# kelaendi/mused

Hardware: AMD Instinct MI355X
Metric: stream rows/sec, d=1024 l=128 window=10k synthetic (SWFD + kNN similarity + eigenstep + labels) (higher is better)
Workload: dtype f64; 1 GPU; synthetic d=1024 l=128 window=10000 k=50 (BASELINE config 2); stream=blob, W=10000, d=1024, l=128, k=50, modalities=1, swfd_levels=14, rccl_ranks=1, lanes_per_gpu=20, padded_window_slots=2

## Files before the change

mused_amd/csrc/eig.hip:

```cpp
#include <stdlib.h>

#include <vector>

#include "internal.h"
#include "wave_ops.h"

namespace mused {

std::recursive_mutex& capture_mutex() {
  static std::recursive_mutex m;
  return m;
}

struct OsjqCtl {
  unsigned head, tail;
  int finished, nmat;
  int all_done, error;
  int dirty;
  int pad;
};

enum class EigDirect {
  None,
  Trd,
  Trdx,
};
enum class EigJacobi {
  Queue,
  WaveGraph,
  RowGraph,
};
struct EigChoice {
  EigDirect direct;
  EigJacobi jacobi;
  int ldn;
  int rps;
  int need;
  bool cert_all;
  bool sort;
  bool adaptive;
};
struct EigEnv {
  bool trd;
  int queue;
  bool graph;
  unsigned long long queue_timeout;
};

struct EigPlan {
  int n = 0, batch = 0, sweeps = 0;
  EigChoice c{};
  double* G = nullptr;
  double* Gc = nullptr;
  double* lam = nullptr;
  const int* rep = nullptr;
  const int* jrep = nullptr;
  int* err_out = nullptr;
  double* trace = nullptr;
  unsigned long long* work = nullptr;
  int* notconv = nullptr;
  unsigned* q = nullptr;
  unsigned qcap = 0;
  OsjqCtl* qctl = nullptr;
  int* qdone = nullptr;
  int* qclean = nullptr;
  unsigned long long q_timeout = 0;
  double* trd_ws = nullptr;
  int* trd_done = nullptr;
  int *trdx_act = nullptr, *trdx_jrep = nullptr;
  int* trdx_nrej = nullptr;
  int* trdx_nrej_host = nullptr;
  hipEvent_t trdx_ev = nullptr;
  bool prof = false;
  int prof_n = 0;
  std::vector<hipEvent_t> ev0, ev1;
  std::vector<hipEvent_t> evm;
  hipGraph_t graph = nullptr;
  hipGraphExec_t exec = nullptr;
  hipStream_t cap_stream = nullptr;
  bool capturing = false;
};

constexpr int OSJ_CB = 32;
constexpr double OSJ_CONV_COS2_WAVE = 1e-10, OSJ_CONV_COS2_ROW = 1e-14;
__device__ __forceinline__ bool osj_pair_active(double pq2, double pp, double qq, double floor2, double cos2) {
  return (pq2 > cos2 * (pp * qq)) & (pp > floor2) & (qq > floor2);
}

__device__ __forceinline__ bool osj_finished(const int* __restrict__ notconv, int fr, int rps, int batch, int m) {
  if (!notconv || fr < rps) return false;
  int any = 0;
  for (int i = 1; i <= rps; ++i) any |= notconv[(long)(fr - i) * batch + m];
  return any == 0;
}

__host__ __device__ constexpr int osj_pair_p(int m2, int step, int k) {
  const int m = m2 - 1;
  const int a = (k == 0) ? m : (step + k) % m;
  const int b = (k == 0) ? (step % m) : ((step - k + m) % m);
  return a < b ? a : b;
}
__host__ __device__ constexpr int osj_pair_q(int m2, int step, int k) {
  const int m = m2 - 1;
  const int a = (k == 0) ? m : (step + k) % m;
  const int b = (k == 0) ? (step % m) : ((step - k + m) % m);
  return a < b ? b : a;
}

template <int N>
__device__ __forceinline__ double wave_treduce(double (&v)[N], int lane, int& idx) {
  static_assert(N == 4 || N == 8 || N == 16 || N == 32 || N == 64, "wave_treduce: N must be 4, 8, 16, 32 or 64");
  if constexpr (N == 4) {
    v[0] = swap32_add(v[0], v[2]);
    v[1] = swap32_add(v[1], v[3]);
    double t4 = swap16_add(v[0], v[1]);
    t4 = t4 + dpp_mov_f64<DPP_ROW_MIRROR>(t4);
    t4 = t4 + dpp_mov_f64<DPP_ROW_HALF_MIRROR>(t4);
    t4 = t4 + dpp_mov_f64<DPP_QUAD_XOR2>(t4);
    t4 = t4 + dpp_mov_f64<DPP_QUAD_XOR1>(t4);
    idx = ((lane >> 5) & 1) * 2 + ((lane >> 4) & 1);
    return t4;
  } else {
#pragma unroll
  for (int i = 0; i < N / 2; ++i) v[i] = swap32_add(v[i], v[i + N / 2]);
#pragma unroll
  for (int i = 0; i < N / 4; ++i) v[i] = swap16_add(v[i], v[i + N / 4]);
  {
    const bool hi = (lane & 8) != 0;
#pragma unroll
    for (int i = 0; i < N / 8; ++i) {
      const double keep = hi ? v[i + N / 8] : v[i];
      const double send = hi ? v[i] : v[i + N / 8];
      v[i] = keep + dpp_mov_f64<DPP_ROW_MIRROR>(send);
    }
  }
  int id = ((lane >> 5) & 1) * 4 + ((lane >> 4) & 1) * 2 + ((lane >> 3) & 1);
  double t;
  if constexpr (N == 8) {
    t = v[0] + dpp_mov_f64<DPP_ROW_HALF_MIRROR>(v[0]);
    t = t + dpp_mov_f64<DPP_QUAD_XOR2>(t);
    t = t + dpp_mov_f64<DPP_QUAD_XOR1>(t);
  } else {
    {
      const bool hi = (lane & 4) != 0;
#pragma unroll
      for (int i = 0; i < N / 16; ++i) {
        const double keep = hi ? v[i + N / 16] : v[i];
        const double send = hi ? v[i] : v[i + N / 16];
        v[i] = keep + dpp_mov_f64<DPP_ROW_HALF_MIRROR>(send);
      }
      id = id * 2 + ((lane >> 2) & 1);
    }
    if constexpr (N == 16) {
      t = v[0] + dpp_mov_f64<DPP_QUAD_XOR2>(v[0]);
      t = t + dpp_mov_f64<DPP_QUAD_XOR1>(t);
    } else {
      {
        const bool hi = (lane & 2) != 0;
#pragma unroll
        for (int i = 0; i < N / 32; ++i) {
          const double keep = hi ? v[i + N / 32] : v[i];
          const double send = hi ? v[i] : v[i + N / 32];
          v[i] = keep + dpp_mov_f64<DPP_QUAD_XOR2>(send);
        }
        id = id * 2 + ((lane >> 1) & 1);
      }
      if constexpr (N == 32) {
        t = v[0] + dpp_mov_f64<DPP_QUAD_XOR1>(v[0]);
      } else {
        const bool hi = (lane & 1) != 0;
        const double keep = hi ? v[1] : v[0];
        const double send = hi ? v[0] : v[1];
        t = keep + dpp_mov_f64<DPP_QUAD_XOR1>(send);
        id = id * 2 + (lane & 1);
      }
    }
  }
  idx = id;
  return t;
  }
}

__device__ __forceinline__ double osj_readlane(double v, int l) {
  const unsigned long long u = (unsigned long long)__double_as_longlong(v);
  const unsigned lo = __builtin_amdgcn_readlane((int)(unsigned)(u & 0xffffffffull), l);
  const unsigned hi = __builtin_amdgcn_readlane((int)(unsigned)(u >> 32), l);
  return __longlong_as_double((long long)(((unsigned long long)hi << 32) | lo));
}

__device__ __forceinline__ double osj_rcp(double y) {
  double r = __builtin_amdgcn_rcp(y);
  r = fma(r, fma(-y, r, 1.0), r);
  r = fma(r, fma(-y, r, 1.0), r);
  return r;
}
__device__ __forceinline__ double osj_rsqrt(double h) {
  double r = __builtin_amdgcn_rsq(h);
  r = r * fma(-0.5 * h, r * r, 1.5);
  r = r * fma(-0.5 * h, r * r, 1.5);
  return r;
}
__device__ __forceinline__ void osj_rotation(double pp, double qq, double pq, double& c, double& s, double& npp,
                                             double& nqq) {
  c = 1.0; s = 0.0; npp = pp; nqq = qq;
  if (pq * pq > 1e-30 * (pp * qq) && pq != 0.0) {
    const double zeta = (qq - pp) * osj_rcp(2.0 * pq);
    const double az = fabs(zeta);
    double t;
// ... 410 lines not shown
      for (int i = 0; i < RP; ++i) osj_st<ST_WT>(&M[(long)colg * ldn + lane + 64 * i], x[c * RP + i] * dd);
    }
  } else {
    const int ca = set_col(ida), cb = set_col(idb);
#pragma unroll
    for (int j = 0; j < SC; ++j) {
      const double da = sh.dsc[wave][j], db = sh.dsc[wave][SC + j];
#pragma unroll
      for (int i = 0; i < RP; ++i) {
        osj_st<ST_WT>(&M[(long)(ca + j) * ldn + lane + 64 * i], x[j * RP + i] * da);
        osj_st<ST_WT>(&M[(long)(cb + j) * ldn + lane + 64 * i], x[(SC + j) * RP + i] * db);
      }
    }
  }
  return active;
}

template <int RP, int SC, bool PREFIX>
__global__ __launch_bounds__(64 * (OSJ_CB / SC), SC == 8 ? 2 : 1) void osjw_kernel(double* __restrict__ Gc, int ldn, int nb,
                                                                                  int round,
                                                                                  int* __restrict__ notconv, int fr, int rps,
                                                                                  const double* __restrict__ trace,
                                                                                  int sortcols,
                                                                                  const int* __restrict__ rep) {
  if (rep && rep[blockIdx.y] != (int)blockIdx.y) return;
  if (osj_finished(notconv, fr, rps, gridDim.y, blockIdx.y)) return;
  double small2 = notconv ? 0.0 : -1.0;
  if (trace) {
    const double tr = trace[blockIdx.y];
    small2 = 1e-24 * tr * tr;
  }
  __shared__ OsjwShared<RP, SC> sh;
  double* M = Gc + (long)blockIdx.y * ldn * ldn;
#ifdef MUSED_OSJ_WT_STORES
  const int active = osjw_unit<RP, SC, PREFIX, false, true>(M, ldn, nb, round, blockIdx.x, small2, sortcols, sh, threadIdx.x);
#else
  const int active = osjw_unit<RP, SC, PREFIX, false>(M, ldn, nb, round, blockIdx.x, small2, sortcols, sh, threadIdx.x);
#endif
  if (notconv && __any(active) && (threadIdx.x & 63) == 0) atomicOr(&notconv[(long)fr * gridDim.y + blockIdx.y], 1);
}

constexpr unsigned OSJQ_EXIT = 0xffffffffu;

__global__ void osjq_init_kernel(OsjqCtl* __restrict__ ctl, unsigned* __restrict__ q, int* __restrict__ qdone,
                                 int* __restrict__ qclean, int batch, int upr, const int* __restrict__ rep,
                                 const int* __restrict__ skip) {
  const int m = blockIdx.x * blockDim.x + threadIdx.x;
  if (m == 0) {
    ctl->head = 0; ctl->finished = 0; ctl->all_done = 0; ctl->error = 0;
  }
  if (m >= batch) return;
  qdone[m] = 0;
  qclean[m] = 0;
  if (rep && rep[m] != m) return;
  if (skip && skip[m]) return;
  const unsigned pos = atomicAdd(&ctl->tail, (unsigned)upr);
  for (int i = 0; i < upr; ++i) q[pos + i] = 1u + (((unsigned)m * 256u + 0u) * 4u + (unsigned)i);
  atomicAdd(&ctl->nmat, 1);
  ctl->dirty = 1;
}

__global__ void osjq_reset_kernel(OsjqCtl* __restrict__ ctl) { ctl->tail = 0; ctl->nmat = 0; ctl->dirty = 0; }
template <int RP>
__global__ __launch_bounds__(256, 2) void osjq_kernel(double* __restrict__ Gc, int ldn, int nb, int batch, int max_sweeps,
                                                     int sort_from, int* __restrict__ notconv,
                                                     const double* __restrict__ trace, unsigned* __restrict__ q,
                                                     unsigned qcap, OsjqCtl* __restrict__ ctl, int* __restrict__ qdone,
                                                     int* __restrict__ qclean, unsigned long long timeout,
                                                     int* __restrict__ err_out) {
  __shared__ OsjwShared<RP, 8> sh;
  __shared__ unsigned s_item;
  const int rounds = nb - 1, upr = nb / 2;
  while (true) {
    if (threadIdx.x == 0) {
      unsigned item = OSJQ_EXIT;
      const bool over = __hip_atomic_load(&ctl->all_done, __ATOMIC_RELAXED, __HIP_MEMORY_SCOPE_AGENT) != 0;
      const unsigned t = over ? qcap : atomicAdd(&ctl->head, 1u);
      if (t < qcap) {
        const unsigned long long t0 = __builtin_amdgcn_s_memrealtime();
        while ((item = __hip_atomic_load(&q[t], __ATOMIC_RELAXED, __HIP_MEMORY_SCOPE_AGENT)) == 0u) {
          if (__hip_atomic_load(&ctl->all_done, __ATOMIC_RELAXED, __HIP_MEMORY_SCOPE_AGENT)) {
            item = OSJQ_EXIT;
            break;
          }
          __builtin_amdgcn_s_sleep(4);
          if (__builtin_amdgcn_s_memrealtime() - t0 > timeout) {
            __hip_atomic_store(&ctl->error, 1, __ATOMIC_RELAXED, __HIP_MEMORY_SCOPE_AGENT);
            __hip_atomic_store(&ctl->all_done, 1, __ATOMIC_RELAXED, __HIP_MEMORY_SCOPE_AGENT);
            if (err_out) atomicOr(err_out, 1);
            item = OSJQ_EXIT;
            break;
          }
        }
      }
      s_item = item;
    }
    __syncthreads();
    const unsigned item = (unsigned)__builtin_amdgcn_readfirstlane((int)s_item);
    __syncthreads();
    if (item == OSJQ_EXIT) return;
    const unsigned v = item - 1u;
    const int k = (int)(v & 3u), R = (int)((v >> 2) & 255u), m = (int)(v >> 10);
    const int sweep = R / rounds, r = R - sweep * rounds;
    double small2 = notconv ? 0.0 : -1.0;
    if (trace) {
      const double tr = trace[m];
      small2 = 1e-24 * tr * tr;
    }
    double* M = Gc + (long)m * ldn * ldn;
    const int so = sweep >= sort_from ? 1 : 0;
    int active;
    int tid = threadIdx.x;
    asm volatile("" : "+v"(tid));
    if (r == 0) active = osjw_unit<RP, 8, true, true>(M, ldn, nb, 0, k, small2, so, sh, tid);
    else active = osjw_unit<RP, 8, false, true>(M, ldn, nb, r, k, small2, so, sh, tid);
    if (notconv && __any(active) && (threadIdx.x & 63) == 0) atomicOr(&notconv[(long)R * batch + m], 1);
    asm volatile("s_waitcnt vmcnt(0)" ::: "memory");
    __syncthreads();
    if (threadIdx.x == 0) {
      const int old = atomicAdd(&qdone[m], 1);
      if (old == upr - 1) {
        __hip_atomic_store(&qdone[m], 0, __ATOMIC_RELAXED, __HIP_MEMORY_SCOPE_AGENT);
        bool fin = (r == rounds - 1) && (sweep + 1 >= max_sweeps);
        if (notconv && !fin) {
          const int flag = __hip_atomic_load(&notconv[(long)R * batch + m], __ATOMIC_RELAXED, __HIP_MEMORY_SCOPE_AGENT);
          const int clean = flag ? 0 : __hip_atomic_load(&qclean[m], __ATOMIC_RELAXED, __HIP_MEMORY_SCOPE_AGENT) + 1;
          __hip_atomic_store(&qclean[m], clean, __ATOMIC_RELAXED, __HIP_MEMORY_SCOPE_AGENT);
          fin = clean >= rounds;
        }
        if (fin) {
          const int f = atomicAdd(&ctl->finished, 1);
          if (f + 1 == ctl->nmat) __hip_atomic_store(&ctl->all_done, 1, __ATOMIC_RELAXED, __HIP_MEMORY_SCOPE_AGENT);
        } else {
          asm volatile("s_waitcnt vmcnt(0)" ::: "memory");
          const unsigned tt = atomicAdd(&ctl->tail, (unsigned)upr);
          for (int i = 0; i < upr; ++i)
            if (tt + i < qcap)
              __hip_atomic_store(&q[tt + i], 1u + (((unsigned)m * 256u + (unsigned)(R + 1)) * 4u + (unsigned)i),
                                 __ATOMIC_RELAXED, __HIP_MEMORY_SCOPE_AGENT);
        }
      }
    }
  }
}

__global__ void osjq_zero_kernel(unsigned* __restrict__ q, unsigned n, const OsjqCtl* __restrict__ ctl) {
  if (!ctl->dirty) return;
  const unsigned i = blockIdx.x * blockDim.x + threadIdx.x;
  if (i < n) q[i] = 0u;
}

__global__ __launch_bounds__(1024) void osjq_prep_direct_kernel(OsjqCtl* __restrict__ ctl, unsigned* __restrict__ q, unsigned qcap,
                                                               int* __restrict__ qdone, int* __restrict__ qclean, int batch,
                                                               int upr, const int* __restrict__ rep, const int* __restrict__ skip,
                                                               const double* __restrict__ Gc, int ldn, int nflag,
                                                               double* __restrict__ trace, int* __restrict__ notconv) {
  __shared__ int s_dirty;
  const int t = threadIdx.x;
  if (t == 0) s_dirty = ctl->dirty;
  __syncthreads();
  if (s_dirty)
    for (unsigned i = t; i < qcap; i += 1024) q[i] = 0u;
  __syncthreads();
  if (t == 0) {
    ctl->head = 0; ctl->tail = 0; ctl->finished = 0; ctl->nmat = 0; ctl->all_done = 0; ctl->error = 0; ctl->dirty = 0;
  }
  __syncthreads();
  for (int m = t; m < batch; m += 1024) {
    qdone[m] = 0;
    qclean[m] = 0;
    if (rep && rep[m] != m) continue;
    if (skip && skip[m]) continue;
    if (trace) {
      const double* M = Gc + (long)m * ldn * ldn;
      double sacc = 0.0;
      for (int i = 0; i < ldn; ++i) sacc += fabs(M[(long)i * ldn + i]);
      trace[m] = sacc;
      for (int f = 0; f < nflag; ++f) notconv[(long)f * batch + m] = 0;
    }
    const unsigned pos = atomicAdd(&ctl->tail, (unsigned)upr);
    for (int i = 0; i < upr; ++i) q[pos + i] = 1u + (((unsigned)m * 256u + 0u) * 4u + (unsigned)i);
    atomicAdd(&ctl->nmat, 1);
    ctl->dirty = 1;
  }
  __syncthreads();
  if (t == 0 && ctl->nmat == 0) ctl->all_done = 1;
}

template <int RP>
static void osjq_launch(EigPlan* p, hipStream_t st) {
  const int ldn = p->c.ldn, nb = ldn / OSJ_CB, upr = nb / 2;
  const bool behind_direct = p->c.direct == EigDirect::Trd;
  if (behind_direct) {
    hipLaunchKernelGGL(osjq_prep_direct_kernel, dim3(1), dim3(1024), 0, st, p->qctl, p->q, p->qcap, p->qdone, p->qclean, p->batch,
                       upr, p->rep, p->trd_done, p->Gc, ldn, p->notconv ? p->sweeps * p->c.rps : 0, p->notconv ? p->trace : nullptr,
                       p->notconv);
  } else {
    hipLaunchKernelGGL(osjq_zero_kernel, dim3(cdiv(p->qcap, 1024)), dim3(1024), 0, st, p->q, p->qcap, p->qctl);
    hipLaunchKernelGGL(osjq_reset_kernel, dim3(1), dim3(1), 0, st, p->qctl);
    hipLaunchKernelGGL(osjq_init_kernel, dim3(cdiv(p->batch, 256)), dim3(256), 0, st, p->qctl, p->q, p->qdone, p->qclean,
                       p->batch, upr, p->rep, (const int*)nullptr);
  }
  long units = (long)p->batch * upr;
  const long cap = behind_direct ? 64 : 512;
  const int grid = (int)(units < cap ? units : cap);
  hipLaunchKernelGGL((osjq_kernel<RP>), dim3(grid), dim3(256), 0, st, p->Gc, ldn, nb, p->batch, p->sweeps,
                     p->c.sort ? 0 : 1 << 30 , p->notconv, p->trace, p->q, p->qcap, p->qctl, p->qdone, p->qclean, p->q_timeout, p->err_out);
}

template <int RP>
static void osjw_launch_sweep(EigPlan* p, int sweep, hipStream_t st) {
  const int ldn = p->c.ldn, nb = ldn / OSJ_CB;
  const int so = p->c.sort ? 1 : 0;
  const int rps = p->c.rps;
  hipLaunchKernelGGL((osjw_kernel<RP, 8, true>), dim3(nb / 2, p->batch), dim3(256), 0, st, p->Gc, ldn, nb, 0,
                     p->notconv, sweep * rps, rps, p->trace, so, p->jrep);
  for (int round = 1; round < nb - 1; ++round)
    hipLaunchKernelGGL((osjw_kernel<RP, 8, false>), dim3(nb / 2, p->batch), dim3(256), 0, st, p->Gc, ldn, nb,
                       round, p->notconv, sweep * rps + round, rps, p->trace, so, p->jrep);
}

__global__ void osj_pack_kernel(const double* __restrict__ G, int n, int ldn, double* __restrict__ Gc) {
  const long gid = (long)blockIdx.x * blockDim.x + threadIdx.x;
  const long per = (long)ldn * ldn;
  if (gid >= per * gridDim.y) return;
  const int b = blockIdx.y;
  const long e = gid;
  if (e >= per) return;
  const int c = (int)(e / ldn), r = (int)(e - (long)c * ldn);
  Gc[b * per + e] = (c < n && r < n) ? G[(long)b * n * n + (long)c * n + r] : 0.0;
}

__global__ void osj_begin_kernel(const double* __restrict__ Gc, int ldn, int nflag, double* __restrict__ trace,
                                 int* __restrict__ notconv) {
  const int b = blockIdx.x, lane = threadIdx.x;
  const double* M = Gc + (long)b * ldn * ldn;
  double s = 0.0;
  for (int i = lane; i < ldn; i += 64) s += fabs(M[(long)i * ldn + i]);
  s = wave_sum(s);
  if (lane == 0) trace[b] = s;
  for (int f = lane; f < nflag; f += 64) notconv[(long)f * gridDim.x + b] = 0;
}

__global__ void osj_count_kernel(const int* __restrict__ notconv, int batch, int nround, int rps,
                                 unsigned long long* __restrict__ acc, const int* __restrict__ rep) {
  int c = 0;
  for (int b = threadIdx.x; b < batch; b += blockDim.x) {
    if (rep && rep[b] != b) continue;
    int clean = 0;
    for (int r = 0; r < nround; ++r) {
      if (r >= rps && clean >= rps) break;
      ++c;
      clean = notconv[(long)r * batch + b] ? 0 : clean + 1;
    }
  }
  c = (int)wave_sum((double)c);
  if ((threadIdx.x & 63) == 0) atomicAdd(acc, (unsigned long long)c);
}

__global__ void osj_norms_kernel(const double* __restrict__ Gc, int ldn, double* __restrict__ lam, const int* __restrict__ skip) {
  const int col = blockIdx.x * (blockDim.x >> 6) + (threadIdx.x >> 6);
  if (col >= ldn) return;
  const int b = blockIdx.y, lane = threadIdx.x & 63;
  if (skip && skip[b]) return;
  const double* c = Gc + ((long)b * ldn + col) * ldn;
  double s = 0.0;
  for (int r = lane; r < ldn; r += 64) s += c[r] * c[r];
  s = wave_sum(s);
  if (lane == 0) lam[(long)b * ldn + col] = sqrt(s);
}

__global__ void osj_extract_kernel(const double* __restrict__ Gc, const double* __restrict__ lam, int n, int ldn,
                                   double* __restrict__ evals, double* __restrict__ V) {
  const int b = blockIdx.y;
  const long gid = (long)blockIdx.x * blockDim.x + threadIdx.x;
  if (gid >= (long)n * n) return;
  const int j = (int)(gid / n), a = (int)(gid - (long)j * n);
  const double l = lam[(long)b * ldn + j];
  if (a == 0) evals[(long)b * n + j] = l;
  if (V) V[(long)b * n * n + (long)a * n + j] = (l > 0.0) ? Gc[((long)b * ldn + j) * ldn + a] / l : 0.0;
}

template <int NT>
static void osjw4_launch_sweep(EigPlan* p, int sweep, hipStream_t st) {
  constexpr int RP = NT / 64;
  const int ldn = p->c.ldn, nb = ldn / OSJ_CB;
  const int rps = p->c.rps;
  const int so = p->c.sort ? 1 : 0;
  hipLaunchKernelGGL((osj_round_kernel<OSJ_CB / 2, NT, 2>), dim3(nb, p->batch), dim3(NT), 0, st, p->Gc, p->n, ldn,
                     2 * nb, 0, p->notconv, sweep * rps, rps, p->trace, so, p->jrep);
  for (int round = 0; round < nb - 1; ++round)
    hipLaunchKernelGGL((osjw_kernel<RP, 4, false>), dim3(nb / 2, p->batch), dim3(512), 0, st, p->Gc, ldn, nb, round,
                       p->notconv, sweep * rps + 1 + round, rps, p->trace, so, p->jrep);
}

template <int NT>
static void osj_launch_sweep(EigPlan* p, int sweep, hipStream_t st) {
  const int ldn = p->c.ldn, nb = ldn / OSJ_CB;
  const int rps = p->c.rps;
  const int so = p->c.sort ? 1 : 0;
  hipLaunchKernelGGL((osj_round_kernel<OSJ_CB / 2, NT, 2>), dim3(nb, p->batch), dim3(NT), 0, st, p->Gc, p->n, ldn,
                     2 * nb, 0, p->notconv, sweep * rps, rps, p->trace, so, p->jrep);
  for (int round = 0; round < nb - 1; ++round)
    hipLaunchKernelGGL((osj_round_kernel<OSJ_CB, NT, 1>), dim3(nb / 2, p->batch), dim3(NT), 0, st, p->Gc, p->n, ldn,
                       nb, round, p->notconv, sweep * rps + 1 + round, rps, p->trace, so, p->jrep);
}

static int osj_enqueue_sweeps(EigPlan* p, hipStream_t st) {
  const int ldn = p->c.ldn;
  switch (p->c.jacobi) {
    case EigJacobi::Queue:
      switch (ldn) {
        case 64: osjq_launch<1>(p, st); break;
        case 128: osjq_launch<2>(p, st); break;
        case 192: osjq_launch<3>(p, st); break;
        default: osjq_launch<4>(p, st); break;
      }
      break;
    case EigJacobi::WaveGraph:
      for (int sw = 0; sw < p->sweeps; ++sw) {
        switch (ldn) {
          case 64: osjw_launch_sweep<1>(p, sw, st); break;
          case 128: osjw_launch_sweep<2>(p, sw, st); break;
          case 192: osjw_launch_sweep<3>(p, sw, st); break;
          case 256: osjw_launch_sweep<4>(p, sw, st); break;
          case 320: osjw4_launch_sweep<320>(p, sw, st); break;
          case 384: osjw4_launch_sweep<384>(p, sw, st); break;
          case 448: osjw4_launch_sweep<448>(p, sw, st); break;
          default: osjw4_launch_sweep<512>(p, sw, st); break;
        }
      }
      break;
    case EigJacobi::RowGraph:
      for (int sw = 0; sw < p->sweeps; ++sw) {
        switch (ldn) {
          case 640: osj_launch_sweep<640>(p, sw, st); break;
          case 768: osj_launch_sweep<768>(p, sw, st); break;
          case 896: osj_launch_sweep<896>(p, sw, st); break;
          default: osj_launch_sweep<1024>(p, sw, st); break;
        }
      }
      break;
  }
  MUSED_LAUNCH_CHECK();
  return MUSED_OK;
}

static int osj_padded_order(int n) {
  if (n <= 512) return ((n + 63) / 64) * 64;
  return ((n + 127) / 128) * 128;
}

static EigEnv eig_read_env() {
  EigEnv e;
  const char* te = getenv("MUSED_EIG_TRD");
  e.trd = !(te && te[0] == '0');
  const char* qe = getenv("MUSED_EIG_QUEUE");
  e.queue = qe ? (qe[0] == '1' ? 1 : 0) : -1;
  const char* ng = getenv("MUSED_NO_GRAPH");
  e.graph = !(ng && ng[0] == '1');
  const char* tq = getenv("MUSED_EIG_QUEUE_TIMEOUT_TICKS");
  e.queue_timeout = tq ? strtoull(tq, nullptr, 10) : 300000000ull;
  return e;
}

static EigChoice eig_choose(int n, int batch, int sweeps, int flags, int need, const EigEnv& env) {
  EigChoice c;
  c.ldn = osj_padded_order(n);
  const int nb = c.ldn / OSJ_CB;
  c.sort = !(flags & EIG_PLAN_NO_SORT);
  c.adaptive = !(flags & EIG_PLAN_FIXED_SWEEPS);
  c.need = (flags & (EIG_PLAN_TOP_NEED | EIG_PLAN_TOP_FD)) ? need : ((flags & EIG_PLAN_TOP_HALF) ? n / 2 : 0);
  c.cert_all = (flags & EIG_PLAN_TOP_NEED) != 0;
  const bool queue_fits = c.ldn <= 256 && sweeps * (nb - 1) <= 255 && batch <= (1 << 21);
  c.direct = EigDirect::None;
  if (env.trd && c.need > 0) {
    if (queue_fits && trd_supports(n, c.ldn, c.need))
      c.direct = EigDirect::Trd;
    else if (trdx_supports(c.ldn, c.need))
      c.direct = EigDirect::Trdx;
  }
  const bool want_queue =
      c.direct == EigDirect::Trd || (env.queue >= 0 ? env.queue == 1 : (long)batch * (nb / 2) <= 224);
  c.jacobi = (queue_fits && want_queue) ? EigJacobi::Queue : (c.ldn <= 512 ? EigJacobi::WaveGraph : EigJacobi::RowGraph);
  c.rps = c.ldn <= 256 ? nb - 1 : nb;
  return c;
}

static int eig_plan_create_impl(EigPlan* p, const EigEnv& env, bool own_graph) {
  const EigChoice& c = p->c;
  const size_t batch = (size_t)p->batch, ldn = (size_t)c.ldn;
  if (p->n != c.ldn) MUSED_CHECK_HIP(hipMalloc(&p->G, sizeof(double) * batch * p->n * p->n));
  MUSED_CHECK_HIP(hipMalloc(&p->Gc, sizeof(double) * batch * ldn * ldn));
  MUSED_CHECK_HIP(hipMalloc(&p->lam, sizeof(double) * batch * ldn));
  if (c.jacobi == EigJacobi::Queue) {
    const int nb = c.ldn / OSJ_CB;
    p->qcap = (unsigned)((long)p->batch * (nb / 2) * (nb - 1) * p->sweeps);
    p->q_timeout = env.queue_timeout;
    MUSED_CHECK_HIP(hipMalloc(&p->q, sizeof(unsigned) * (size_t)p->qcap));
    MUSED_CHECK_HIP(hipMalloc(&p->qctl, sizeof(OsjqCtl)));
    MUSED_CHECK_HIP(hipMalloc(&p->qdone, sizeof(int) * batch));
    MUSED_CHECK_HIP(hipMalloc(&p->qclean, sizeof(int) * batch));
    MUSED_CHECK_HIP(hipMemset(p->qctl, 0, sizeof(OsjqCtl)));
    MUSED_CHECK_HIP(hipMemset(p->q, 0, sizeof(unsigned) * (size_t)p->qcap));
  }
  int rc;
  switch (c.direct) {
    case EigDirect::None: break;
    case EigDirect::Trd:
      if ((rc = trd_prepare())) return rc;
      MUSED_CHECK_HIP(hipMalloc(&p->trd_ws, sizeof(double) * trd_workspace_doubles(p->batch)));
      MUSED_CHECK_HIP(hipMalloc(&p->trd_done, sizeof(int) * batch));
      break;
    case EigDirect::Trdx:
      if ((rc = trdx_prepare(c.ldn))) return rc;
      MUSED_CHECK_HIP(hipMalloc(&p->trd_ws, sizeof(double) * trdx_workspace_doubles(c.ldn, p->batch)));
      MUSED_CHECK_HIP(hipMalloc(&p->trd_done, sizeof(int) * batch));
      MUSED_CHECK_HIP(hipMalloc(&p->trdx_act, sizeof(int) * batch));
      MUSED_CHECK_HIP(hipMalloc(&p->trdx_jrep, sizeof(int) * batch));
      MUSED_CHECK_HIP(hipMalloc(&p->trdx_nrej, sizeof(int)));
      MUSED_CHECK_HIP(hipHostMalloc((void**)&p->trdx_nrej_host, sizeof(int), hipHostMallocDefault));
      MUSED_CHECK_HIP(hipEventCreateWithFlags(&p->trdx_ev, hipEventDisableTiming));
      p->jrep = p->trdx_jrep;
      break;
  }
  if (c.adaptive) {
    MUSED_CHECK_HIP(hipMalloc(&p->trace, sizeof(double) * (batch + 1) + sizeof(int) * batch * p->sweeps * c.rps));
    p->work = (unsigned long long*)(p->trace + batch);
    p->notconv = (int*)(p->trace + batch + 1);
    MUSED_CHECK_HIP(hipMemset(p->work, 0, 8));
  }
  if (own_graph && env.graph) {
    MUSED_CHECK_HIP(hipStreamCreateWithFlags(&p->cap_stream, hipStreamNonBlocking));
    MUSED_CHECK_HIP(hipStreamBeginCapture(p->cap_stream, hipStreamCaptureModeThreadLocal));
    p->capturing = true;
    if ((rc = osj_enqueue_sweeps(p, p->cap_stream))) return rc;
    p->capturing = false;
    MUSED_CHECK_HIP(hipStreamEndCapture(p->cap_stream, &p->graph));
    MUSED_CHECK_HIP(hipGraphInstantiate(&p->exec, p->graph, nullptr, nullptr, 0));
    (void)hipStreamDestroy(p->cap_stream);
    p->cap_stream = nullptr;
  }
  return MUSED_OK;
}

int eig_plan_create(int n, int batch, int sweeps, bool own_graph, EigPlan** out, const int* rep, int flags, int* err_out,
                    int need) {
  MUSED_REQUIRE(n >= 2 && n % 2 == 0 && n <= 1024 && batch >= 1 && sweeps >= 1,
                "eig_plan_create: the order must be even and <= 1024 (n=%d)", n);
  CaptureLock resource_guard(capture_mutex());
  const EigEnv env = eig_read_env();
  EigPlan* p = new EigPlan();
  p->n = n; p->batch = batch; p->sweeps = sweeps;
  p->rep = p->jrep = rep;
  p->err_out = err_out;
  p->c = eig_choose(n, batch, sweeps, flags, need, env);
  const int rc = eig_plan_create_impl(p, env, own_graph);
  if (rc) {
    eig_plan_destroy(p);
    return rc;
  }
  *out = p;
  return MUSED_OK;
}

void eig_plan_destroy(EigPlan* p) {
  if (!p) return;
  CaptureLock resource_guard(capture_mutex());
  if (p->capturing) {
    hipGraph_t g = nullptr;
    (void)hipStreamEndCapture(p->cap_stream, &g);
    if (g) (void)hipGraphDestroy(g);
  }
  if (p->exec) (void)hipGraphExecDestroy(p->exec);
  if (p->graph) (void)hipGraphDestroy(p->graph);
  if (p->cap_stream) (void)hipStreamDestroy(p->cap_stream);
  void* bufs[] = {p->G,      p->Gc,       p->lam,      p->trace,     p->q,        p->qctl, p->qdone,
                  p->qclean, p->trd_ws,   p->trd_done, p->trdx_act,  p->trdx_jrep, p->trdx_nrej};
  for (void* b : bufs)
    if (b) (void)hipFree(b);
  if (p->trdx_nrej_host) (void)hipHostFree(p->trdx_nrej_host);
  if (p->trdx_ev) (void)hipEventDestroy(p->trdx_ev);
  for (auto* v : {&p->ev0, &p->ev1, &p->evm})
    for (hipEvent_t e : *v) (void)hipEventDestroy(e);
  delete p;
}

int eig_plan_profile(EigPlan* p, bool on) {
  if (!p) return MUSED_OK;
  if (on && p->ev0.empty()) {
    for (auto* v : {&p->ev1, &p->evm, &p->ev0}) {
      if (v == &p->evm && p->c.direct == EigDirect::None) continue;
      while (v->size() < 2048) {
        hipEvent_t e;
        MUSED_CHECK_HIP(hipEventCreate(&e));
        v->push_back(e);
      }
    }
  }
  p->prof = on;
  if (on) {
    p->prof_n = 0;
    if (p->work) MUSED_CHECK_HIP(hipMemset(p->work, 0, 8));
  }
  return MUSED_OK;
}

int eig_plan_profile_read(EigPlan* p, double* total_ms, long* launches, double* bytes_per_launch) {
  *total_ms = 0.0; *launches = 0; *bytes_per_launch = 0.0;
  if (!p || p->ev0.empty()) return MUSED_OK;
  for (int i = 0; i < p->prof_n; ++i) {
    MUSED_CHECK_HIP(hipEventSynchronize(p->ev1[i]));
    float ms = 0.f;
    MUSED_CHECK_HIP(hipEventElapsedTime(&ms, p->ev0[i], p->ev1[i]));
    *total_ms += ms;
  }
  *launches = (long)p->prof_n * p->sweeps * p->c.rps;
  double frac = 1.0;
  if (p->work && p->prof_n > 0) {
    unsigned long long w = 0;
    CaptureLock guard(capture_mutex());
    MUSED_CHECK_HIP(hipMemcpy(&w, p->work, 8, hipMemcpyDeviceToHost));
    frac = (double)w / ((double)p->prof_n * p->sweeps * p->c.rps * p->batch);
  }
  *bytes_per_launch = 16.0 * (double)p->batch * p->c.ldn * p->c.ldn * frac;
  return MUSED_OK;
}

int eig_plan_profile_read_direct(EigPlan* p, double* total_ms, long* launches, double* matrices_solved, double* tridiag_ms) {
  *total_ms = 0.0; *launches = 0; *matrices_solved = 0.0;
  if (tridiag_ms) *tridiag_ms = 0.0;
  if (!p || p->c.direct == EigDirect::None || p->ev0.empty()) return MUSED_OK;
  for (int i = 0; i < p->prof_n; ++i) {
    MUSED_CHECK_HIP(hipEventSynchronize(p->ev1[i]));
    float ms = 0.f;
    MUSED_CHECK_HIP(hipEventElapsedTime(&ms, p->ev0[i], p->ev1[i]));
    *total_ms += ms;
    if (tridiag_ms) {
      MUSED_CHECK_HIP(hipEventElapsedTime(&ms, p->ev0[i], p->evm[i]));
      *tridiag_ms += ms;
    }
  }
  *launches = p->prof_n;
  if (p->work) {
    unsigned long long w = 0;
    CaptureLock guard(capture_mutex());
    MUSED_CHECK_HIP(hipMemcpy(&w, p->work, 8, hipMemcpyDeviceToHost));
    *matrices_solved = (double)w;
  }
  return MUSED_OK;
}

EigColumns eig_plan_columns(EigPlan* p) { return {p->Gc, p->lam, p->c.ldn}; }

bool eig_plan_direct_solver(EigPlan* p) { return p && p->c.direct != EigDirect::None; }

double* eig_plan_input(EigPlan* p) { return p->G ? p->G : p->Gc; }

static int eig_run_direct(EigPlan* p, hipStream_t st, bool rec) {
  unsigned long long* work = rec ? p->work : nullptr;
  hipEvent_t after_a = rec ? p->evm[p->prof_n] : nullptr;
  int rc;
  if (p->c.direct == EigDirect::Trd) {
    rc = trd_solve(p->Gc, p->n, p->c.ldn, p->c.need, p->c.cert_all, p->batch, p->rep, p->trd_done, p->trd_ws, st, nullptr, work,
                   after_a, p->lam);
  } else {
    MUSED_CHECK_HIP(hipMemsetAsync(p->trdx_nrej, 0, sizeof(int), st));
    rc = trdx_solve(p->Gc, p->c.ldn, p->c.need, p->c.cert_all, p->batch, p->rep, p->trd_done, p->trdx_act, p->trdx_jrep,
                    p->trdx_nrej, p->trd_ws, st, work, after_a, nullptr, p->lam);
  }
  if (rc) return rc;
  if (rec) {
    MUSED_CHECK_HIP(hipEventRecord(p->ev1[p->prof_n], st));
    ++p->prof_n;
  }
  return MUSED_OK;
}

static int eig_jacobi_needed(EigPlan* p, hipStream_t st, bool* needed) {
  *needed = true;
  if (p->c.direct != EigDirect::Trdx) return MUSED_OK;
  hipStreamCaptureStatus cs = hipStreamCaptureStatusNone;
  (void)hipStreamIsCapturing(st, &cs);
  if (cs != hipStreamCaptureStatusNone) return MUSED_OK;
  MUSED_CHECK_HIP(hipMemcpyAsync(p->trdx_nrej_host, p->trdx_nrej, sizeof(int), hipMemcpyDeviceToHost, st));
  MUSED_CHECK_HIP(hipEventRecord(p->trdx_ev, st));
  MUSED_CHECK_HIP(hipEventSynchronize(p->trdx_ev));
  *needed = *p->trdx_nrej_host != 0;
  return MUSED_OK;
}

int eig_plan_run_inplace(EigPlan* p, double* evals, double* V, hipStream_t st, bool allow_graph) {
  const EigChoice& c = p->c;
  const bool direct = c.direct != EigDirect::None;
  int rc;
  if (p->G) {
    const long per = (long)c.ldn * c.ldn;
    hipLaunchKernelGGL(osj_pack_kernel, dim3(cdiv(per, 256), p->batch), dim3(256), 0, st, p->G, p->n, c.ldn, p->Gc);
  }
  if (p->notconv && c.direct != EigDirect::Trd)
    hipLaunchKernelGGL(osj_begin_kernel, dim3(p->batch), dim3(64), 0, st, p->Gc, c.ldn, p->sweeps * c.rps, p->trace, p->notconv);
  const bool rec = p->prof && p->prof_n < (int)p->ev0.size();
  if (rec) MUSED_CHECK_HIP(hipEventRecord(p->ev0[p->prof_n], st));
  if (direct && (rc = eig_run_direct(p, st, rec))) return rc;
  bool jacobi = true;
  if ((rc = eig_jacobi_needed(p, st, &jacobi))) return rc;
  if (jacobi) {
    if (p->exec && allow_graph)
      MUSED_CHECK_HIP(hipGraphLaunch(p->exec, st));
    else if ((rc = osj_enqueue_sweeps(p, st)))
      return rc;
  }
  if (rec && !direct) {
    MUSED_CHECK_HIP(hipEventRecord(p->ev1[p->prof_n], st));
    ++p->prof_n;
    if (p->notconv)
      hipLaunchKernelGGL(osj_count_kernel, dim3(1), dim3(256), 0, st, p->notconv, p->batch, p->sweeps * c.rps, c.rps, p->work,
                         p->rep);
  }
  hipLaunchKernelGGL(osj_norms_kernel, dim3(cdiv(c.ldn, 4), p->batch), dim3(256), 0, st, p->Gc, c.ldn, p->lam,
                     (const int*)p->trd_done);
  if (evals)
    hipLaunchKernelGGL(osj_extract_kernel, dim3(cdiv((long)p->n * p->n, 256), p->batch), dim3(256), 0, st, p->Gc, p->lam, p->n,
                       c.ldn, evals, V);
  MUSED_LAUNCH_CHECK();
  return MUSED_OK;
}

int eig_plan_run(EigPlan* p, const double* G, double* evals, double* V, hipStream_t st) {
  const size_t bytes = sizeof(double) * (size_t)p->batch * p->n * p->n;
  MUSED_CHECK_HIP(hipMemcpyAsync(eig_plan_input(p), G, bytes, hipMemcpyDeviceToDevice, st));
  return eig_plan_run_inplace(p, evals, V, st, true);
}

static int eig_time(EigPlan* p, hipEvent_t& e0, hipEvent_t& e1, const double* G, int reps, double* evals, double* V,
                    double* out_ms, int* out_err, hipStream_t st) {
  MUSED_CHECK_HIP(hipEventCreate(&e0));
  MUSED_CHECK_HIP(hipEventCreate(&e1));
  int rc = eig_plan_run(p, G, evals, V, st);
  MUSED_CHECK_HIP(hipStreamSynchronize(st));
  MUSED_CHECK_HIP(hipEventRecord(e0, st));
  for (int i = 0; i < reps && !rc; ++i) rc = eig_plan_run(p, G, evals, V, st);
  MUSED_CHECK_HIP(hipEventRecord(e1, st));
  MUSED_CHECK_HIP(hipEventSynchronize(e1));
  float ms = 0.f;
  MUSED_CHECK_HIP(hipEventElapsedTime(&ms, e0, e1));
  *out_ms = ms / (reps > 0 ? reps : 1);
  if (out_err) {
    *out_err = 0;
    if (p->c.jacobi == EigJacobi::Queue) {
      OsjqCtl c;
      MUSED_CHECK_HIP(hipMemcpy(&c, p->qctl, sizeof(c), hipMemcpyDeviceToHost));
      *out_err = c.error ? -1 : (int)c.tail;
    }
  }
  return rc;
}

}

using namespace mused;

extern "C" {

int mused_debug_eig_choice(int n, int batch, int sweeps, int flags, int need, int* out) {
  MUSED_REQUIRE(out && n >= 2 && n % 2 == 0 && n <= 1024 && batch >= 1 && sweeps >= 1,
                "mused_debug_eig_choice: the order must be even and <= 1024 (n=%d)", n);
  const EigChoice c = eig_choose(n, batch, sweeps, flags, need, eig_read_env());
  const int v[8] = {(int)c.direct, (int)c.jacobi, c.ldn, c.rps, c.need, c.cert_all, c.sort, c.adaptive};
  memcpy(out, v, sizeof(v));
  return MUSED_OK;
}

int mused_debug_eig_time(const double* G, int n, int batch, int sweeps, int reps, double* evals, double* V, double* out_ms,
                         int* out_err, void* stream) {
  EigPlan* p = nullptr;
  int rc = eig_plan_create(n, batch, sweeps, true, &p);
  if (rc) return rc;
  hipEvent_t e0 = nullptr, e1 = nullptr;
  rc = eig_time(p, e0, e1, G, reps, evals, V, out_ms, out_err, (hipStream_t)stream);
  if (e0) (void)hipEventDestroy(e0);
  if (e1) (void)hipEventDestroy(e1);
  eig_plan_destroy(p);
  return rc;
}

int mused_syevj_batched(const double* G, int n, int batch, int sweeps, double* evals, double* V, void* stream) {
  MUSED_REQUIRE(G && evals && V, "mused_syevj_batched: null pointer");
  EigPlan* p = nullptr;
  int rc = eig_plan_create(n, batch, sweeps, true, &p);
  if (rc) return rc;
  rc = eig_plan_run(p, G, evals, V, (hipStream_t)stream);
  hipError_t e = hipStreamSynchronize((hipStream_t)stream);
  eig_plan_destroy(p);
  if (rc) return rc;
  MUSED_CHECK_HIP(e);
  return MUSED_OK;
}

}
```

mused_amd/csrc/gemm_f64.h:

```cpp
#pragma once
#include <mutex>
#include "common.h"

namespace mused {

typedef double v4f64 __attribute__((ext_vector_type(4)));

constexpr int GEMM_BM = 128;
constexpr int GEMM_BN = 128;
constexpr int GEMM_BK = 16;
constexpr int GEMM_LD = 144;
constexpr int GEMM_THREADS = 256;
constexpr int GEMM_LDS_BYTES = 2  * 2  * GEMM_BK * GEMM_LD * 8;

struct GemmArgs {
  const void* A;
  const void* B;
  long lda, ldb;
  long strideA, strideB;
  int M, N, K;
  int kchunk;
  int splitk;
  int bsplit;
  int tiles_m, tiles_n;
  const int* rep;
  int sym;
};

template <typename TIn, bool VEC>
__device__ __forceinline__ void stage_load_kc(const TIn* __restrict__ src, long ld, int r0, int nrows, int k0,
                                              int kend, TIn (&r)[8]) {
  const int m = threadIdx.x & 127;
  const int kh = threadIdx.x >> 7;
  const int row = r0 + m;
  const int k = k0 + kh * 8;
  if (row < nrows) {
    const TIn* p = src + (long)row * ld + k;
    if (VEC && k + 8 <= kend) {
      if (sizeof(TIn) == 4) {
        const float4 a = *reinterpret_cast<const float4*>(p);
        const float4 b = *reinterpret_cast<const float4*>(p + 4);
        r[0] = a.x; r[1] = a.y; r[2] = a.z; r[3] = a.w;
        r[4] = b.x; r[5] = b.y; r[6] = b.z; r[7] = b.w;
      } else {
        const double2* q = reinterpret_cast<const double2*>(p);
#pragma unroll
        for (int j = 0; j < 4; ++j) {
          const double2 v = q[j];
          r[2 * j] = v.x;
          r[2 * j + 1] = v.y;
        }
      }
    } else {
#pragma unroll
      for (int j = 0; j < 8; ++j) r[j] = (k + j < kend) ? p[j] : (TIn)0;
    }
  } else {
#pragma unroll
    for (int j = 0; j < 8; ++j) r[j] = (TIn)0;
  }
}

template <typename TIn>
__device__ __forceinline__ void stage_store_kc(double* __restrict__ lds, const TIn (&r)[8]) {
  const int m = threadIdx.x & 127;
  const int kh = threadIdx.x >> 7;
#pragma unroll
  for (int j = 0; j < 8; ++j) lds[(kh * 8 + j) * GEMM_LD + m] = (double)r[j];
}

template <typename TIn, bool VEC>
__device__ __forceinline__ void stage_load_mc(const TIn* __restrict__ src, long ld, int c0, int ncols, int k0,
                                              int kend, TIn (&r)[8]) {
  const int kk = threadIdx.x >> 4;
  const int c = c0 + (threadIdx.x & 15) * 8;
  const int k = k0 + kk;
  if (k < kend) {
    const TIn* p = src + (long)k * ld + c;
    if (VEC && c + 8 <= ncols) {
      if (sizeof(TIn) == 4) {
        const float4 a = *reinterpret_cast<const float4*>(p);
        const float4 b = *reinterpret_cast<const float4*>(p + 4);
        r[0] = a.x; r[1] = a.y; r[2] = a.z; r[3] = a.w;
        r[4] = b.x; r[5] = b.y; r[6] = b.z; r[7] = b.w;
      } else {
        const double2* q = reinterpret_cast<const double2*>(p);
#pragma unroll
        for (int j = 0; j < 4; ++j) {
          const double2 v = q[j];
          r[2 * j] = v.x;
          r[2 * j + 1] = v.y;
        }
      }
    } else {
#pragma unroll
      for (int j = 0; j < 8; ++j) r[j] = (c + j < ncols) ? p[j] : (TIn)0;
    }
  } else {
#pragma unroll
    for (int j = 0; j < 8; ++j) r[j] = (TIn)0;
  }
}

template <typename TIn>
__device__ __forceinline__ void stage_store_mc(double* __restrict__ lds, const TIn (&r)[8]) {
  const int kk = threadIdx.x >> 4;
  const int c = (threadIdx.x & 15) * 8;
  double* p = lds + kk * GEMM_LD + c;
#pragma unroll
  for (int j = 0; j < 8; ++j) p[j] = (double)r[j];
}

template <typename TIn>
__device__ __forceinline__ void stage_load8(const TIn* __restrict__ p, TIn (&r)[8]) {
  if (sizeof(TIn) == 4) {
    const float4 a = *reinterpret_cast<const float4*>(p);
    const float4 b = *reinterpret_cast<const float4*>(p + 4);
    r[0] = a.x; r[1] = a.y; r[2] = a.z; r[3] = a.w;
    r[4] = b.x; r[5] = b.y; r[6] = b.z; r[7] = b.w;
  } else {
    const double2* q = reinterpret_cast<const double2*>(p);
#pragma unroll
    for (int j = 0; j < 4; ++j) {
      const double2 v = q[j];
      r[2 * j] = v.x;
      r[2 * j + 1] = v.y;
    }
  }
}
template <typename TIn>
__device__ __forceinline__ void stage_load_kc_full(const TIn* __restrict__ src, long ld, int r0, int k0, TIn (&r)[8]) {
  stage_load8(src + (long)(r0 + (threadIdx.x & 127)) * ld + k0 + (threadIdx.x >> 7) * 8, r);
}
template <typename TIn>
__device__ __forceinline__ void stage_load_mc_full(const TIn* __restrict__ src, long ld, int c0, int k0, TIn (&r)[8]) {
  stage_load8(src + (long)(k0 + (threadIdx.x >> 4)) * ld + c0 + (threadIdx.x & 15) * 8, r);
}

__device__ __forceinline__ int xcd_remap(int pid, int nwg) {
  const int q = nwg >> 3, r = nwg & 7, xcd = pid & 7;
  const int base = (xcd < r) ? xcd * (q + 1) : r * (q + 1) + (xcd - r) * q;
  return base + (pid >> 3);
}

template <typename TA, typename TB, bool A_KC, bool B_KC, bool VEC>
__device__ __forceinline__ void gemm_tile_mainloop(const GemmArgs& g, const TA* __restrict__ A, const TB* __restrict__ B,
                                                   int m0, int n0, int k_lo, int k_hi, double* smem,
                                                   v4f64 (&acc)[4][4]) {
  double* As = smem;
  double* Bs = smem + 2 * GEMM_BK * GEMM_LD;
  const int lane = threadIdx.x & 63;
  const int wave = threadIdx.x >> 6;
  const int wr = wave >> 1, wc = wave & 1;
  const int kq = lane >> 4, li = lane & 15;
#pragma unroll
  for (int i = 0; i < 4; ++i)
#pragma unroll
    for (int j = 0; j < 4; ++j) acc[i][j] = (v4f64){0.0, 0.0, 0.0, 0.0};

  TA ra[8];
  TB rb[8];
  const int nkt = (k_hi - k_lo + GEMM_BK - 1) / GEMM_BK;

  const bool full_mn = VEC && m0 + GEMM_BM <= g.M && n0 + GEMM_BN <= g.N;
  auto load_tile = [&](int kt) {
    const int k0 = k_lo + kt * GEMM_BK;
    if (full_mn && k0 + GEMM_BK <= k_hi) {
      if (A_KC) stage_load_kc_full<TA>(A, g.lda, m0, k0, ra); else stage_load_mc_full<TA>(A, g.lda, m0, k0, ra);
      if (B_KC) stage_load_kc_full<TB>(B, g.ldb, n0, k0, rb); else stage_load_mc_full<TB>(B, g.ldb, n0, k0, rb);
      return;
    }
    if (A_KC) stage_load_kc<TA, VEC>(A, g.lda, m0, g.M, k0, k_hi, ra);
    else      stage_load_mc<TA, VEC>(A, g.lda, m0, g.M, k0, k_hi, ra);
    if (B_KC) stage_load_kc<TB, VEC>(B, g.ldb, n0, g.N, k0, k_hi, rb);
    else      stage_load_mc<TB, VEC>(B, g.ldb, n0, g.N, k0, k_hi, rb);
  };
  auto store_tile = [&](int buf) {
    double* a = As + buf * GEMM_BK * GEMM_LD;
    double* b = Bs + buf * GEMM_BK * GEMM_LD;
    if (A_KC) stage_store_kc(a, ra); else stage_store_mc(a, ra);
    if (B_KC) stage_store_kc(b, rb); else stage_store_mc(b, rb);
  };

  if (nkt > 0) {
    load_tile(0);
    store_tile(0);
  }
  __syncthreads();

  int cur = 0;
  for (int kt = 0; kt < nkt; ++kt) {
    const bool more = (kt + 1 < nkt);
    if (more) load_tile(kt + 1);
    const double* a = As + cur * GEMM_BK * GEMM_LD + wr * 64 + li;
    const double* b = Bs + cur * GEMM_BK * GEMM_LD + wc * 64 + li;
#pragma unroll
    for (int kk = 0; kk < GEMM_BK / 4; ++kk) {
      double fa[4], fb[4];
#pragma unroll
      for (int i = 0; i < 4; ++i) fa[i] = a[(kk * 4 + kq) * GEMM_LD + i * 16];
#pragma unroll
      for (int j = 0; j < 4; ++j) fb[j] = b[(kk * 4 + kq) * GEMM_LD + j * 16];
#pragma unroll
      for (int i = 0; i < 4; ++i)
#pragma unroll
        for (int j = 0; j < 4; ++j)
          acc[i][j] = __builtin_amdgcn_mfma_f64_16x16x4f64(fa[i], fb[j], acc[i][j], 0, 0, 0);
    }
    if (more) store_tile(cur ^ 1);
    __syncthreads();
    cur ^= 1;
  }
}

template <typename TA, typename TB, bool A_KC, bool B_KC, bool VEC, typename Epi>
__global__ __launch_bounds__(GEMM_THREADS, 2) void gemm_f64_kernel(GemmArgs g, Epi epi) {
  extern __shared__ __attribute__((aligned(16))) double smem[];

  const int z = blockIdx.z;
  const int zb = g.bsplit ? z / g.bsplit : z;
  if (g.rep && g.rep[zb] != zb) return;
  int tm, tn;
  if (g.sym) {
    const int t = g.tiles_n, nwg = t * (t + 1) / 2;
    const int e = xcd_remap(blockIdx.x, nwg);
    int r = (int)((2.0 * t + 1.0 - sqrt((2.0 * t + 1.0) * (2.0 * t + 1.0) - 8.0 * e)) * 0.5);
    r = r < 0 ? 0 : (r > t - 1 ? t - 1 : r);
    while (r > 0 && r * t - r * (r - 1) / 2 > e) --r;
    while (r + 1 < t && (r + 1) * t - (r + 1) * r / 2 <= e) ++r;
    tm = r;
    tn = r + (e - (r * t - r * (r - 1) / 2));
  } else {
    const int nwg = g.tiles_m * g.tiles_n;
    const int wg = xcd_remap(blockIdx.x, nwg);
    constexpr int GROUP_M = 8;
    const int per_group = GROUP_M * g.tiles_n;
    const int group_id = wg / per_group;
    const int first_m = group_id * GROUP_M;
    const int group_size = min(g.tiles_m - first_m, GROUP_M);
    tm = first_m + (wg % group_size);
    tn = (wg % per_group) / group_size;
  }
  const int m0 = tm * GEMM_BM, n0 = tn * GEMM_BN;
  const bool mirror = g.sym && tm != tn;

  int k_lo = 0, k_hi = g.K;
  const TA* A = reinterpret_cast<const TA*>(g.A);
  const TB* B = reinterpret_cast<const TB*>(g.B);
  if (g.splitk) {
    k_lo = z * g.kchunk;
    k_hi = min(g.K, k_lo + g.kchunk);
  } else {
    A += (long)zb * g.strideA;
    B += (long)zb * g.strideB;
    if (g.bsplit) {
      k_lo = (z - zb * g.bsplit) * g.kchunk;
      k_hi = min(g.K, k_lo + g.kchunk);
    }
  }

  const int lane = threadIdx.x & 63;
  const int wave = threadIdx.x >> 6;
  const int wr = wave >> 1, wc = wave & 1;
  const int kq = lane >> 4, li = lane & 15;

  v4f64 acc[4][4];
  gemm_tile_mainloop<TA, TB, A_KC, B_KC, VEC>(g, A, B, m0, n0, k_lo, k_hi, smem, acc);

#pragma unroll
  for (int i = 0; i < 4; ++i) {
#pragma unroll
    for (int j = 0; j < 4; ++j) {
      const int col = n0 + wc * 64 + j * 16 + li;
#pragma unroll
      for (int r = 0; r < 4; ++r) {
        const int row = m0 + wr * 64 + i * 16 + kq + 4 * r;
        if (row < g.M && col < g.N) epi(z, row, col, acc[i][j][r]);
      }
    }
  }
  if (mirror) {
    __syncthreads();
    double* patch = smem + wave * (32 * 65);
#pragma unroll
    for (int half = 0; half < 2; ++half) {
#pragma unroll
      for (int i = 0; i < 4; ++i)
#pragma unroll
        for (int jj = 0; jj < 2; ++jj) {
          const int j = half * 2 + jj;
          const int col = n0 + wc * 64 + j * 16 + li;
#pragma unroll
          for (int r = 0; r < 4; ++r) {
            const int rl = i * 16 + kq + 4 * r;
            const int rg = m0 + wr * 64 + rl;
            patch[(jj * 16 + li) * 65 + rl] = (rg < g.M && col < g.N) ? epi.value(col, rg, acc[i][j][r]) : 0.0;
          }
        }
      const int rowm = m0 + wr * 64 + lane;
#pragma unroll 8
      for (int c = 0; c < 32; ++c) {
        const int colm = n0 + wc * 64 + half * 32 + c;
        if (colm < g.N && rowm < g.M) epi.put(z, colm, rowm, patch[c * 65 + lane]);
      }
    }
  }
}

struct EpiStore {
  double* C;
  long ldc;
  long strideC;
  double alpha;
  __device__ __forceinline__ void operator()(int z, int row, int col, double v) const {
    C[(long)z * strideC + (long)row * ldc + col] = alpha * v;
  }
  __device__ __forceinline__ double value(int, int, double v) const { return alpha * v; }
  __device__ __forceinline__ void put(int z, int row, int col, double val) const {
    C[(long)z * strideC + (long)row * ldc + col] = val;
  }
};

template <typename TA, typename TB, bool A_KC, bool B_KC, bool VEC, typename Epi>
int gemm_f64_prepare_t() {
  static std::once_flag once;
  static hipError_t err = hipSuccess;
  std::call_once(once, [] {
    auto k = gemm_f64_kernel<TA, TB, A_KC, B_KC, VEC, Epi>;
    err = hipFuncSetAttribute(reinterpret_cast<const void*>(k), hipFuncAttributeMaxDynamicSharedMemorySize,
                              GEMM_LDS_BYTES);
  });
  MUSED_CHECK_HIP(err);
  return MUSED_OK;
}

template <typename TA, typename TB, bool A_KC, bool B_KC, typename Epi>
int gemm_f64_launch_t(GemmArgs g, int batch, Epi epi, bool vec, hipStream_t stream) {
  g.tiles_m = cdiv(g.M, GEMM_BM);
  g.tiles_n = cdiv(g.N, GEMM_BN);
  if (g.M <= 0 || g.N <= 0 || batch <= 0) return MUSED_OK;
  dim3 grid(g.sym ? g.tiles_n * (g.tiles_n + 1) / 2 : g.tiles_m * g.tiles_n, 1, batch);
  int rc;
  if (vec) {
    if ((rc = gemm_f64_prepare_t<TA, TB, A_KC, B_KC, true, Epi>())) return rc;
    hipLaunchKernelGGL((gemm_f64_kernel<TA, TB, A_KC, B_KC, true, Epi>), grid, dim3(GEMM_THREADS), GEMM_LDS_BYTES,
                       stream, g, epi);
  } else {
    if ((rc = gemm_f64_prepare_t<TA, TB, A_KC, B_KC, false, Epi>())) return rc;
    hipLaunchKernelGGL((gemm_f64_kernel<TA, TB, A_KC, B_KC, false, Epi>), grid, dim3(GEMM_THREADS), GEMM_LDS_BYTES,
                       stream, g, epi);
  }
  MUSED_LAUNCH_CHECK();
  return MUSED_OK;
}

template <typename T>
static inline bool vec_ok(const void* p, long ld, long stride) {
  const long e = 16 / (long)sizeof(T);
  return ((uintptr_t)p % 16 == 0) && (ld % e == 0) && (stride % e == 0);
}

}
```

mused_amd/csrc/gemm_f64.hip:

```cpp
#include <stdarg.h>

#include "gemm_f64.h"
#include "internal.h"

namespace mused {

static thread_local char g_err[512] = "";

void set_error(const char* fmt, ...) {
  va_list ap;
  va_start(ap, fmt);
  vsnprintf(g_err, sizeof(g_err), fmt, ap);
  va_end(ap);
}

const char* last_error() { return g_err; }

int gemm_f64_prepare_all() {
  int rc = 0;
#define PREP(a, b, v) rc |= gemm_f64_prepare_t<double, double, a, b, v, EpiStore>()
  PREP(true, true, true); PREP(true, true, false); PREP(true, false, true); PREP(true, false, false);
  PREP(false, true, true); PREP(false, true, false); PREP(false, false, true); PREP(false, false, false);
#undef PREP
  return rc ? MUSED_ERR_HIP : MUSED_OK;
}

int gemm_f64(bool a_kc, bool b_kc, const double* A, long lda, long strideA, const double* B, long ldb,
             long strideB, double* C, long ldc, long strideC, int M, int N, int K, int batch, double alpha,
             hipStream_t stream, const int* rep) {
  GemmArgs g;
  memset(&g, 0, sizeof(g));
  g.A = A; g.B = B; g.lda = lda; g.ldb = ldb; g.strideA = strideA; g.strideB = strideB;
  g.M = M; g.N = N; g.K = K; g.splitk = 0; g.kchunk = 0;
  g.rep = rep;
  g.sym = (A == B && a_kc == b_kc && lda == ldb && strideA == strideB && M == N) ? 1 : 0;
  EpiStore epi{C, ldc, strideC, alpha};
  const bool vec = vec_ok<double>(A, lda, strideA) && vec_ok<double>(B, ldb, strideB);
  if (a_kc && b_kc) return gemm_f64_launch_t<double, double, true, true>(g, batch, epi, vec, stream);
  if (a_kc && !b_kc) return gemm_f64_launch_t<double, double, true, false>(g, batch, epi, vec, stream);
  if (!a_kc && b_kc) return gemm_f64_launch_t<double, double, false, true>(g, batch, epi, vec, stream);
  return gemm_f64_launch_t<double, double, false, false>(g, batch, epi, vec, stream);
}

int gemm_f64_splitk(bool a_kc, bool b_kc, const double* A, long lda, const double* B, long ldb, double* partial,
                    int M, int N, int K, int kchunk, int nsplit, hipStream_t stream) {
  MUSED_REQUIRE(kchunk > 0 && kchunk % GEMM_BK == 0 && nsplit >= 1 && (long)kchunk * nsplit >= K,
                "gemm_f64_splitk: bad kchunk %d x %d for K=%d", kchunk, nsplit, K);
  GemmArgs g;
  memset(&g, 0, sizeof(g));
  g.A = A; g.B = B; g.lda = lda; g.ldb = ldb;
  g.M = M; g.N = N; g.K = K; g.splitk = 1; g.kchunk = kchunk;
  EpiStore epi{partial, (long)N, (long)M * N, 1.0};
  const bool vec = vec_ok<double>(A, lda, 0) && vec_ok<double>(B, ldb, 0);
  if (a_kc && b_kc) return gemm_f64_launch_t<double, double, true, true>(g, nsplit, epi, vec, stream);
  if (a_kc && !b_kc) return gemm_f64_launch_t<double, double, true, false>(g, nsplit, epi, vec, stream);
  if (!a_kc && b_kc) return gemm_f64_launch_t<double, double, false, true>(g, nsplit, epi, vec, stream);
  return gemm_f64_launch_t<double, double, false, false>(g, nsplit, epi, vec, stream);
}

__global__ void splitk_reduce_kernel(const double* __restrict__ partial, int nsplit, long count,
                                     double* __restrict__ out) {
  const long i = (long)blockIdx.x * blockDim.x + threadIdx.x;
  if (i >= count) return;
  double s = 0.0;
  for (int z = 0; z < nsplit; ++z) s += partial[(long)z * count + i];
  out[i] = s;
}

int gemm_f64_batched_splitk(bool a_kc, bool b_kc, const double* A, long lda, long strideA, const double* B, long ldb, long strideB,
                            double* partial, int M, int N, int K, int batch, int kchunk, int nsplit, hipStream_t stream,
                            const int* rep) {
  MUSED_REQUIRE(kchunk > 0 && kchunk % GEMM_BK == 0 && nsplit >= 1 && (long)kchunk * nsplit >= K,
                "gemm_f64_batched_splitk: bad kchunk %d x %d for K=%d", kchunk, nsplit, K);
  GemmArgs g;
  memset(&g, 0, sizeof(g));
  g.A = A; g.B = B; g.lda = lda; g.ldb = ldb; g.strideA = strideA; g.strideB = strideB;
  g.M = M; g.N = N; g.K = K; g.splitk = 0; g.kchunk = kchunk; g.bsplit = nsplit;
  g.rep = rep;
  g.sym = (A == B && a_kc == b_kc && lda == ldb && strideA == strideB && M == N) ? 1 : 0;
  EpiStore epi{partial, (long)N, (long)M * N, 1.0};
  const bool vec = vec_ok<double>(A, lda, strideA) && vec_ok<double>(B, ldb, strideB);
  if (a_kc && b_kc) return gemm_f64_launch_t<double, double, true, true>(g, batch * nsplit, epi, vec, stream);
  if (a_kc && !b_kc) return gemm_f64_launch_t<double, double, true, false>(g, batch * nsplit, epi, vec, stream);
  if (!a_kc && b_kc) return gemm_f64_launch_t<double, double, false, true>(g, batch * nsplit, epi, vec, stream);
  return gemm_f64_launch_t<double, double, false, false>(g, batch * nsplit, epi, vec, stream);
}

__global__ void batched_splitk_reduce_kernel(const double* __restrict__ partial, int nsplit, long count, double* __restrict__ out,
                                             const int* __restrict__ rep) {
  const int z = blockIdx.y;
  if (rep && rep[z] != z) return;
  const long i = (long)blockIdx.x * blockDim.x + threadIdx.x;
  if (i >= count) return;
  const double* p = partial + (long)z * nsplit * count + i;
  double s = 0.0;
  for (int sp = 0; sp < nsplit; ++sp) s += p[(long)sp * count];
  out[(long)z * count + i] = s;
}

int gemm_batched_splitk_reduce(const double* partial, int nsplit, long count, double* out, int batch, const int* rep,
                               hipStream_t stream) {
  hipLaunchKernelGGL(batched_splitk_reduce_kernel, dim3(cdiv(count, 256), batch), dim3(256), 0, stream, partial, nsplit, count, out,
                     rep);
  MUSED_LAUNCH_CHECK();
  return MUSED_OK;
}

int gemm_splitk_reduce(const double* partial, int nsplit, long count, double* out, hipStream_t stream) {
  hipLaunchKernelGGL(splitk_reduce_kernel, dim3(cdiv(count, 256)), dim3(256), 0, stream, partial, nsplit, count,
                     out);
  MUSED_LAUNCH_CHECK();
  return MUSED_OK;
}

}

extern "C" {

const char* mused_last_error(void) { return mused::last_error(); }

int mused_version(void) { return 100; }

int mused_memcpy_d2d(void* dst, const void* src, long bytes, void* stream) {
  MUSED_REQUIRE(dst && src && bytes >= 0, "mused_memcpy_d2d: bad arguments");
  MUSED_CHECK_HIP(hipMemcpyAsync(dst, src, (size_t)bytes, hipMemcpyDeviceToDevice, (hipStream_t)stream));
  return MUSED_OK;
}

int mused_gemm_f64(int a_kc, int b_kc, const double* A, long lda, const double* B, long ldb, double* C, long ldc,
                   int M, int N, int K, double alpha, void* stream) {
  return mused::gemm_f64(a_kc != 0, b_kc != 0, A, lda, 0, B, ldb, 0, C, ldc, 0, M, N, K, 1, alpha,
                         (hipStream_t)stream);
}

int mused_gemm_f64_batched(int a_kc, int b_kc, const double* A, long lda, long strideA, const double* B, long ldb,
                           long strideB, double* C, long ldc, long strideC, int M, int N, int K, int batch,
                           double alpha, void* stream) {
  return mused::gemm_f64(a_kc != 0, b_kc != 0, A, lda, strideA, B, ldb, strideB, C, ldc, strideC, M, N, K, batch,
                         alpha, (hipStream_t)stream);
}

int mused_gemm_f64_batched_rep(int a_kc, int b_kc, const double* A, long lda, long strideA, const double* B, long ldb,
                               long strideB, double* C, long ldc, long strideC, int M, int N, int K, int batch,
                               double alpha, const int* rep, void* stream) {
  return mused::gemm_f64(a_kc != 0, b_kc != 0, A, lda, strideA, B, ldb, strideB, C, ldc, strideC, M, N, K, batch,
                         alpha, (hipStream_t)stream, rep);
}

int mused_gemm_f64_splitk(int a_kc, int b_kc, const double* A, long lda, const double* B, long ldb, double* partial,
                          double* C, int M, int N, int K, int kchunk, int nsplit, void* stream) {
  MUSED_REQUIRE(A && B && partial && C && M >= 0 && N >= 0 && K >= 0, "mused_gemm_f64_splitk: bad arguments");
  int rc = mused::gemm_f64_splitk(a_kc != 0, b_kc != 0, A, lda, B, ldb, partial, M, N, K, kchunk, nsplit,
                                  (hipStream_t)stream);
  if (rc != MUSED_OK || M == 0 || N == 0) return rc;
  return mused::gemm_splitk_reduce(partial, nsplit, (long)M * N, C, (hipStream_t)stream);
}

int mused_gemm_f64_batched_splitk(int a_kc, int b_kc, const double* A, long lda, long strideA, const double* B, long ldb,
                                  long strideB, double* partial, double* C, int M, int N, int K, int batch, int kchunk,
                                  int nsplit, const int* rep, void* stream) {
  MUSED_REQUIRE(A && B && partial && C && M >= 0 && N >= 0 && K >= 0 && batch >= 1,
                "mused_gemm_f64_batched_splitk: bad arguments");
  int rc = mused::gemm_f64_batched_splitk(a_kc != 0, b_kc != 0, A, lda, strideA, B, ldb, strideB, partial, M, N, K, batch,
                                          kchunk, nsplit, (hipStream_t)stream, rep);
  if (rc != MUSED_OK || M == 0 || N == 0) return rc;
  return mused::gemm_batched_splitk_reduce(partial, nsplit, (long)M * N, C, batch, rep, (hipStream_t)stream);
}

}
```

mused_amd/csrc/internal.h:

```cpp
#pragma once
#include "common.h"

#include <mutex>

namespace mused {

int select_from_records(const double* rec, int n, int kind, int k, int* out_idx, unsigned long long* out_mask,
                        int mask_words, hipStream_t stream);
int select_from_tag_sets(const int* rowptr, const int* tags, const int* postptr, const int* postrow, int n, int k,
                         int* out_idx, unsigned long long* out_mask, int mask_words, hipStream_t stream);
int select_max_fused_rows(bool tag_sets);
int select_window_records(const double* rec, const int* vrank, int s, int e, int kind, int k, unsigned long long* out_mask,
                          int mask_words, hipStream_t stream);
int select_window_tag_sets(const int* rowptr, const int* tags, const int* postptr, const int* postrow, const int* vrank, int s,
                           int e, int k, unsigned long long* out_mask, int mask_words, hipStream_t stream);

std::recursive_mutex& capture_mutex();
using CaptureLock = std::lock_guard<std::recursive_mutex>;


int gemm_f64(bool a_kc, bool b_kc, const double* A, long lda, long strideA, const double* B, long ldb,
             long strideB, double* C, long ldc, long strideC, int M, int N, int K, int batch, double alpha,
             hipStream_t stream, const int* rep = nullptr);

int gemm_f64_batched_splitk(bool a_kc, bool b_kc, const double* A, long lda, long strideA, const double* B, long ldb, long strideB,
                            double* partial, int M, int N, int K, int batch, int kchunk, int nsplit, hipStream_t stream,
                            const int* rep = nullptr);
int gemm_batched_splitk_reduce(const double* partial, int nsplit, long count, double* out, int batch, const int* rep,
                               hipStream_t stream);
int gemm_f64_prepare_all();

int gemm_f64_splitk(bool a_kc, bool b_kc, const double* A, long lda, const double* B, long ldb, double* partial,
                    int M, int N, int K, int kchunk, int nsplit, hipStream_t stream);
int gemm_splitk_reduce(const double* partial, int nsplit, long count, double* out, hipStream_t stream);

int lu_permute_l(double* Y, int n, int r, long ld, int* pivstep, double* prow, long ws_f64_len, hipStream_t st);
int qr_economic(double* Y, int n, int r, long ldy, double* Q, long ldq, double* tau, double* wpart, hipStream_t st,
                const int* run_if = nullptr);
int spmm_binary(const int* rowptr, const int* colidx, int n, const double* Q, long ldq, int r, double* Y, long ldy,
                hipStream_t stream);

int adj_csr_from_mask(const unsigned long long* mask, int n, int words, int* deg, int* rowptr, int* colidx,
                      int* stats, long cap, int* overflow, hipStream_t st);
int zero_ints(int* p, long n, hipStream_t st);
int adj_transpose(const unsigned long long* mask, int n, int words, unsigned long long* out, hipStream_t st);

struct EigPlan;
constexpr int EIG_PLAN_FIXED_SWEEPS = 1;
constexpr int EIG_PLAN_NO_SORT = 2;
constexpr int EIG_PLAN_TOP_HALF = 4;
constexpr int EIG_PLAN_TOP_NEED = 8;
constexpr int EIG_PLAN_TOP_FD = 16;
int eig_plan_create(int n, int batch, int sweeps, bool own_graph, EigPlan** out, const int* rep = nullptr, int flags = 0,
                    int* err_out = nullptr, int need = 0);
void eig_plan_destroy(EigPlan* p);
double* eig_plan_input(EigPlan* p);
int eig_plan_run_inplace(EigPlan* p, double* evals, double* V, hipStream_t stream, bool allow_graph);
int eig_plan_run(EigPlan* p, const double* G, double* evals, double* V, hipStream_t stream);
struct EigColumns {
  const double *cols, *lam;
  int ld;
};
EigColumns eig_plan_columns(EigPlan* p);
bool eig_plan_direct_solver(EigPlan* p);
int eig_plan_profile(EigPlan* p, bool on);
int eig_plan_profile_read(EigPlan* p, double* total_ms, long* launches, double* bytes_per_launch);
int eig_plan_profile_read_direct(EigPlan* p, double* total_ms, long* launches, double* matrices_solved,
                                 double* tridiag_ms = nullptr);

size_t trd_workspace_doubles(int batch);
int trd_prepare();
bool trd_supports(int n, int ldn, int need);
long trd_tail_ws_per();
long trd_tail_off_hs();
long trd_tail_off_tg();
int trd_tail_launch(const double* G, const int* rep, double* ws, int batch, hipStream_t st);
int trd_solve(double* Gc, int n, int ldn, int need, bool cert_all, int batch, const int* rep, int* done, double* ws,
              hipStream_t st, long long* dbg_clk = nullptr, unsigned long long* work = nullptr, hipEvent_t after_a = nullptr,
              double* lam_out = nullptr);

bool trdx_supports(int ldn, int need);
size_t trdx_workspace_doubles(int ldn, int batch);
int trdx_prepare(int ldn);
int trdx_solve(double* Gc, int ldn, int need, bool cert_all, int batch, const int* rep, int* done, int* act, int* jrep,
               int* nrej, double* ws, hipStream_t st, unsigned long long* work = nullptr, hipEvent_t after_a = nullptr,
               long long* prof = nullptr,
               double* lam_out = nullptr);

}
```

mused_amd/csrc/swfd.hip:

```cpp
#include <vector>

#include "internal.h"

namespace mused {

struct Swfd {
  int N, d, ell, L, S, cap, n2, n4, n3;
  int lanes;
  double R;
  long i;
  int pend;
  long restart_mark;
  int skip_dead;
  bool twin;
  int sweeps;
  double* buf;
  double* queue;
  long long* qt;
  int* meta;
  int* rep;
  long long* dropped;
  double* theta;
  double *T, *Wc;
  int gram_split;
  double* gpart;
  int* plan;
  int* keep_src;
  long long* now_dev;
  int* status;
  int* status_host;
  EigPlan* eig;
  double *stack, *Wq, *Bout, *sig_out, *qinfo;
  int* qsel;
  EigPlan* eigq;
  EigPlan* eigq3;
  int pre_chunk;
  double *pre_in, *pre_out, *pre_gram;
  EigPlan* eigp;
};

static inline int sk_index(const Swfd* h, int lane, int level, int kind) { return lane * 2 * h->L + kind * h->L + level; }

struct BitWord { unsigned long long w; };
template <typename T>
__device__ __forceinline__ double row_elem(const T* row, int c) { return (double)row[c]; }
template <>
__device__ __forceinline__ double row_elem<BitWord>(const BitWord* row, int c) {
  return (double)((row[c >> 6].w >> (c & 63)) & 1ull);
}

template <typename T>
__global__ void swfd_append_kernel(const T* __restrict__ X, long ldx, long lane_stride, int per_lane, int m, int d,
                                   int n2, int pend, const int* __restrict__ meta, double* __restrict__ buf) {
  const int r = blockIdx.x, s = blockIdx.y;
  X += (long)(s / per_lane) * lane_stride;
  const int row = meta[s * 4 + 0] + pend + r;
  if (row >= n2) return;
  double* dst = buf + ((long)s * n2 + row) * d;
  const T* src = X + (long)r * ldx;
  for (int c = threadIdx.x; c < d; c += blockDim.x) dst[c] = row_elem<T>(src, c);
}

__global__ void swfd_restart_kernel(double* __restrict__ buf, double* __restrict__ queue, long long* __restrict__ qt,
                                    int* __restrict__ meta, long long* __restrict__ dropped, int L, long buf_elems,
                                    long queue_elems, int cap) {
  const int lane = blockIdx.y / L, j = blockIdx.y - lane * L;
  const int sm = lane * 2 * L + j, sa = sm + L;
  const long gid = (long)blockIdx.x * blockDim.x + threadIdx.x;
  if (gid < buf_elems) {
    buf[sm * buf_elems + gid] = buf[sa * buf_elems + gid];
    buf[sa * buf_elems + gid] = 0.0;
  }
  if (gid < queue_elems) queue[sm * queue_elems + gid] = queue[sa * queue_elems + gid];
  if (gid < cap) qt[sm * cap + gid] = qt[sa * cap + gid];
  if (gid == 0) {
    for (int k = 0; k < 4; ++k) {
      meta[sm * 4 + k] = meta[sa * 4 + k];
      meta[sa * 4 + k] = 0;
    }
    dropped[sm] = dropped[sa];
    dropped[sa] = 0;
  }
}

__global__ void swfd_set_now_kernel(long long* now, long long v) { *now = v; }

__global__ void swfd_rep_kernel(const int* __restrict__ meta, int L, int nchains, int* __restrict__ rep, int twin,
                                const long long* __restrict__ dropped, long long epoch_start, int skip_dead,
                                long long* __restrict__ now_dev, long long now) {
  const int c = blockIdx.x * blockDim.x + threadIdx.x;
  if (c == 0) *now_dev = now;
  if (c >= nchains) return;
  const int base = ((twin && (c & 1)) ? c - 1 : c) * L;
  if (twin && (c & 1)) {
    int r = base + L - 1;
    rep[c * L + L - 1] = r;
    for (int j = L - 2; j >= 0; --j) {
      if (meta[(base + j) * 4 + 3] != 0) r = base + j;
      rep[c * L + j] = r;
    }
    return;
  }
  int r = base + L - 1;
  rep[r] = r;
  for (int j = L - 2; j >= 0; --j) {
    if (meta[(base + j) * 4 + 3] != 0) r = base + j;
    rep[base + j] = r;
  }
  if (skip_dead && !twin && (c & 1) == 0)
    for (int j = 0; j < L - 1; ++j)
      if (dropped[base + j] > epoch_start) rep[base + j] = -1;
}

__global__ __launch_bounds__(1024) void swfd_decide_kernel(const double* __restrict__ evals,
                                                          const double* __restrict__ U, int ldu, int n2,
                                                          int ell, int cap,
                                                          int N, const long long* __restrict__ now_p,
                                                          const double* __restrict__ theta, int* __restrict__ meta,
                                                          long long* __restrict__ qt, long long* __restrict__ dropped,
                                                          int* __restrict__ plan, int* __restrict__ keep_src,
                                                          double* __restrict__ Wc, const int* __restrict__ rep) {
  __shared__ double lam[1024];
  __shared__ int order[1024];
  __shared__ double scale[512];
  const int s = blockIdx.x, t = threadIdx.x;
  const long long now = *now_p;
  const int sr = rep ? rep[s] : s;
  if (sr < 0) return;
  const double* ev = evals + (long)sr * ldu;
  const double* Us = U + (long)sr * ldu * ldu;
  if (t < n2) lam[t] = ev[t];
  __syncthreads();
  if (t < n2) {
    const double mine = lam[t];
    int rank = 0;
    for (int j = 0; j < n2; ++j) {
      const double o = lam[j];
      rank += (o > mine) || (o == mine && j < t);
    }
    order[rank] = t;
  }
  __syncthreads();
  __shared__ int s_part[16];
  __shared__ int s_wcnt[3][4];
  const int head0 = meta[s * 4 + 1], cnt0 = meta[s * 4 + 2];
  long long* q = qt + (long)s * cap;
  const int wv = t >> 6, ln = t & 63;
  int expired = 0;
  for (int k = t; k < cnt0; k += 1024) expired += (q[(head0 + k) % cap] + N <= now) ? 1 : 0;
#pragma unroll
  for (int o = 32; o > 0; o >>= 1) expired += __shfl_xor(expired, o);
  if (ln == 0) s_part[wv] = expired;
  __syncthreads();
  int nexp = 0;
#pragma unroll
  for (int ww = 0; ww < 16; ++ww) nexp += s_part[ww];
  const int head1 = (head0 + nexp) % cap, cnt1 = cnt0 - nexp;
  const double l0 = lam[order[0]];
  const double delta = lam[order[ell - 1]] > 0.0 ? lam[order[ell - 1]] : 0.0;
  const double tol = 1e-10 * (l0 > 0.0 ? l0 : 0.0);
  const double th = theta[s];
  int kind = 0, near = 0;
  double sc = 0.0;
  if (t < ell) {
    const double l = lam[order[t]];
    double s2 = l - delta;
    s2 = s2 > 0.0 ? s2 : 0.0;
    if (s2 > tol) {
      sc = sqrt(s2 / l) / l;
      kind = (s2 >= th) ? 2 : 1;
      near = (kind == 2 && s2 < 2.0 * th) ? 1 : 0;
    }
    scale[t] = sc;
  }
  const unsigned long long mk = __ballot(kind == 1), md = __ballot(kind == 2), mn = __ballot(near != 0);
  const unsigned long long below = (ln == 0) ? 0ull : (~0ull >> (64 - ln));
  if (ln == 0 && wv < 4) {
    s_wcnt[0][wv] = __popcll(mk);
    s_wcnt[1][wv] = __popcll(md);
    s_wcnt[2][wv] = __popcll(mn);
  }
  __syncthreads();
  int kpos = __popcll(mk & below), dpos = __popcll(md & below);
  int nk = 0, nd = 0, nnear = 0;
#pragma unroll
  for (int ww = 0; ww < 4; ++ww) {
    if (ww < wv) {
      kpos += s_wcnt[0][ww];
      dpos += s_wcnt[1][ww];
    }
    nk += s_wcnt[0][ww];
    nd += s_wcnt[1][ww];
    nnear += s_wcnt[2][ww];
  }
  const int nevict = (cnt1 + nd > cap) ? (cnt1 + nd - cap) : 0;
  if (t == 0) {
    long long drop = dropped[s];
    if (nevict > 0) {
      const long long ts = q[(head1 + nevict - 1) % cap];
      drop = ts > drop ? ts : drop;
    }
    dropped[s] = drop;
  }
  __syncthreads();
  if (t < ell) {
    int pos = 0;
    if (kind == 1) {
      pos = kpos;
      keep_src[s * ell + kpos] = t;
    } else if (kind == 2) {
      pos = (head1 + cnt1 + dpos) % cap;
      q[pos] = now;
    }
    plan[(s * ell + t) * 2 + 0] = kind;
    plan[(s * ell + t) * 2 + 1] = pos;
  }
  if (t == 0) {
    meta[s * 4 + 0] = nk;
    meta[s * 4 + 1] = (head1 + nevict) % cap;
    meta[s * 4 + 2] = cnt1 + nd - nevict;
    meta[s * 4 + 3] += nnear;
  }
  __syncthreads();
  if (sr != s) return;
  double* W = Wc + (long)s * ell * n2;
  for (int e = t; e < ell * n2; e += 1024) {
    const int i = e / n2, a = e - i * n2;
    const double sc = scale[i];
    W[e] = (sc != 0.0) ? sc * Us[(long)order[i] * ldu + a] : 0.0;
  }
}

__global__ void swfd_scatter_kernel(const double* __restrict__ T, const int* __restrict__ plan,
                                    const int* __restrict__ keep_src, const int* __restrict__ meta,
                                    double* __restrict__ buf, double* __restrict__ queue, int n2, int ell, int cap,
                                    int d, const int* __restrict__ rep) {
  const int rho = blockIdx.x, s = blockIdx.y;
  if (rep && rep[s] < 0) return;
  const double* Ts = T + (long)(rep ? rep[s] : s) * ell * d;
  if (rho < ell && plan[(s * ell + rho) * 2] == 2) {
    const int slot = plan[(s * ell + rho) * 2 + 1];
    double* dst = queue + ((long)s * cap + slot) * d;
    const double* src = Ts + (long)rho * d;
    for (int c = threadIdx.x; c < d; c += blockDim.x) dst[c] = src[c];
  }
  const int nk = meta[s * 4 + 0];
  double* dst = buf + ((long)s * n2 + rho) * d;
  if (rho < nk) {
    const double* src = Ts + (long)keep_src[s * ell + rho] * d;
    for (int c = threadIdx.x; c < d; c += blockDim.x) dst[c] = src[c];
  } else {
    for (int c = threadIdx.x; c < d; c += blockDim.x) dst[c] = 0.0;
  }
}

static int swfd_rotate_all(Swfd* h, hipStream_t st) {
  const int S = h->S, n2 = h->n2, d = h->d, ell = h->ell;
  int rc;
  if (h->rep)
    hipLaunchKernelGGL(swfd_rep_kernel, dim3(cdiv(2 * h->lanes, 64)), dim3(64), 0, st, h->meta, h->L, 2 * h->lanes, h->rep,
                       h->twin ? 1 : 0, h->dropped, (long long)(((h->i - 1) / h->N) * h->N), h->skip_dead, h->now_dev,
                       (long long)h->i);
  else
    hipLaunchKernelGGL(swfd_set_now_kernel, dim3(1), dim3(1), 0, st, h->now_dev, (long long)h->i);
  if (h->gram_split > 1) {
    const int kchunk = ((d + h->gram_split - 1) / h->gram_split + 15) / 16 * 16;
    if ((rc = gemm_f64_batched_splitk(true, true, h->buf, d, (long)n2 * d, h->buf, d, (long)n2 * d, h->gpart, n2, n2, d, S, kchunk,
                                      h->gram_split, st, h->rep)))
      return rc;
    if ((rc = gemm_batched_splitk_reduce(h->gpart, h->gram_split, (long)n2 * n2, eig_plan_input(h->eig), S, h->rep, st))) return rc;
  } else if ((rc = gemm_f64(true, true, h->buf, d, (long)n2 * d, h->buf, d, (long)n2 * d, eig_plan_input(h->eig), n2,
                            (long)n2 * n2, n2, n2, d, S, 1.0, st, h->rep)))
    return rc;
  if ((rc = eig_plan_run_inplace(h->eig, nullptr, nullptr, st, true))) return rc;
  const EigColumns e = eig_plan_columns(h->eig);
  hipLaunchKernelGGL(swfd_decide_kernel, dim3(S), dim3(1024), 0, st, e.lam, e.cols, e.ld, n2, ell, h->cap, h->N, h->now_dev,
                     h->theta, h->meta, h->qt, h->dropped, h->plan, h->keep_src, h->Wc, h->rep);
  if ((rc = gemm_f64(true, false, h->Wc, n2, (long)ell * n2, h->buf, d, (long)n2 * d, h->T, d, (long)ell * d, ell, d,
                     n2, S, 1.0, st, h->rep)))
    return rc;
  hipLaunchKernelGGL(swfd_scatter_kernel, dim3(n2, S), dim3(256), 0, st, h->T, h->plan, h->keep_src, h->meta, h->buf,
                     h->queue, n2, ell, h->cap, d, h->rep);
  MUSED_LAUNCH_CHECK();
  h->pend = 0;
  return MUSED_OK;
}

static int swfd_restart(Swfd* h, hipStream_t st) {
  const long be = (long)h->n2 * h->d, qe = (long)h->cap * h->d;
  const long m = be > qe ? be : qe;
  hipLaunchKernelGGL(swfd_restart_kernel, dim3(cdiv(m, 256), h->L * h->lanes), dim3(256), 0, st, h->buf, h->queue, h->qt,
                     h->meta, h->dropped, h->L, be, qe, h->cap);
  MUSED_LAUNCH_CHECK();
  return MUSED_OK;
}

constexpr int SWFD_PRE_MAX = 96;
struct PreBlocks {
  int row0[SWFD_PRE_MAX];
  int rows[SWFD_PRE_MAX];
};

template <typename T>
__global__ void swfd_pre_load_kernel(const T* __restrict__ X, long ldx, long lane_stride, int lanes, int ell, int d,
                                     PreBlocks pb, double* __restrict__ out) {
  const int row = blockIdx.x, z = blockIdx.y;
  const int blk = z / lanes, lane = z - blk * lanes;
  double* dst = out + ((long)z * ell + row) * d;
  if (row < pb.rows[blk]) {
    const T* src = X + (long)lane * lane_stride + (long)(pb.row0[blk] + row) * ldx;
    for (int c = threadIdx.x; c < d; c += blockDim.x) dst[c] = row_elem<T>(src, c);
  } else {
    for (int c = threadIdx.x; c < d; c += blockDim.x) dst[c] = 0.0;
  }
}

__global__ void swfd_pre_pack_kernel(const double* __restrict__ gram, int ell, double* __restrict__ Gc) {
  const int n2 = 2 * ell;
  const long z = blockIdx.y;
  const long e = (long)blockIdx.x * blockDim.x + threadIdx.x;
  if (e >= (long)n2 * n2) return;
  const int col = (int)(e / n2), row = (int)(e - (long)col * n2);
  double v = 0.0;
  if (col < ell) v = (row < ell) ? gram[z * ell * ell + (long)col * ell + row] : ((row - ell == col) ? 1.0 : 0.0);
  Gc[z * n2 * n2 + e] = v;
}

template <typename T>
static int swfd_prerotate(Swfd* h, const T* X, long ldx, long lane_stride, const PreBlocks& pb, int nblk, hipStream_t st) {
  const int ell = h->ell, d = h->d, B = h->lanes, n2 = h->n2;
  int rc;
  const int Z = nblk * B;
  hipLaunchKernelGGL(swfd_pre_load_kernel<T>, dim3(ell, Z), dim3(256), 0, st, X, ldx, lane_stride, B, ell, d, pb,
                     h->pre_in);
  if ((rc = gemm_f64(true, true, h->pre_in, d, (long)ell * d, h->pre_in, d, (long)ell * d, h->pre_gram, ell,
                     (long)ell * ell, ell, ell, d, Z, 1.0, st)))
    return rc;
  hipLaunchKernelGGL(swfd_pre_pack_kernel, dim3(cdiv((long)n2 * n2, 256), Z), dim3(256), 0, st, h->pre_gram, ell,
                     eig_plan_input(h->eigp));
  if ((rc = eig_plan_run_inplace(h->eigp, nullptr, nullptr, st, true))) return rc;
  const double* cols = eig_plan_columns(h->eigp).cols;
  const int ld = eig_plan_columns(h->eigp).ld;
  if ((rc = gemm_f64(true, false, cols + ell, ld, (long)ld * ld, h->pre_in, d, (long)ell * d, h->pre_out, d, (long)ell * d,
                     ell, d, ell, Z, 1.0, st)))
    return rc;
  MUSED_LAUNCH_CHECK();
  return MUSED_OK;
}

template <typename T>
static int swfd_append_t(Swfd* h, const T* X, long ldx, long lane_stride, long m, hipStream_t st) {
  long r = 0;
  int rc;
  PreBlocks pb;
  int pre_n = 0, pre_next = 0;
  while (r < m) {
    if (h->i > 0 && h->i % h->N == 0 && h->restart_mark != h->i) {
      if ((rc = swfd_restart(h, st))) return rc;
      h->restart_mark = h->i;
      h->twin = false;
    }
    const long in_epoch = h->i % h->N;
    long until = h->ell - (in_epoch % h->ell);
    if (h->N - in_epoch < until) until = h->N - in_epoch;
    const long take = (m - r) < until ? (m - r) : until;
    bool from_pre = false;
    if (h->pre_chunk > 0 && h->pend == 0 && take == until) {
      if (pre_next >= pre_n) {
        pre_n = pre_next = 0;
        long rr = r, ii = h->i;
        while (pre_n < h->pre_chunk && rr < m) {
          const long ie = ii % h->N;
          long u = h->ell - (ie % h->ell);
          if (h->N - ie < u) u = h->N - ie;
          if (m - rr < u) break;
          pb.row0[pre_n] = (int)rr;
          pb.rows[pre_n] = (int)u;
          ++pre_n;
          rr += u;
          ii += u;
        }
        if ((rc = swfd_prerotate<T>(h, X, ldx, lane_stride, pb, pre_n, st))) return rc;
      }
      from_pre = true;
    }
    if (from_pre) {
      const double* src = h->pre_out + (long)pre_next * h->lanes * h->ell * h->d;
      hipLaunchKernelGGL(swfd_append_kernel<double>, dim3((int)take, h->S), dim3(256), 0, st, src, (long)h->d,
                         (long)h->ell * h->d, 2 * h->L, (int)take, h->d, h->n2, h->pend, h->meta, h->buf);
      ++pre_next;
    } else {
      hipLaunchKernelGGL(swfd_append_kernel<T>, dim3((int)take, h->S), dim3(256), 0, st, X + r * ldx, ldx, lane_stride,
                         2 * h->L, (int)take, h->d, h->n2, h->pend, h->meta, h->buf);
    }
    MUSED_LAUNCH_CHECK();
    h->pend += (int)take;
    h->i += take;
    r += take;
    if (take == until) {
      if ((rc = swfd_rotate_all(h, st))) return rc;
    }
  }
  return MUSED_OK;
}

__global__ void swfd_select_kernel(const int* __restrict__ meta, const long long* __restrict__ qt,
                                   const long long* __restrict__ dropped, int L, int cap, int N, long long now,
                                   int* __restrict__ qsel_all) {
  if (threadIdx.x != 0) return;
  const int lane = blockIdx.x;
  const int base = lane * 2 * L;
  int* qsel = qsel_all + (long)lane * (4 + cap);
  int lvl = L - 1;
  for (int j = 0; j < L; ++j) {
    const long long dr = dropped[base + j];
    if (dr == 0 || dr + N <= now) { lvl = j; break; }
  }
  const int sk = base + lvl;
  const int head = meta[sk * 4 + 1], cnt = meta[sk * 4 + 2];
  int ns = 0;
  for (int q = 0; q < cnt; ++q) {
    const int slot = (head + q) % cap;
    if (qt[(long)sk * cap + slot] + N > now) qsel[4 + ns++] = slot;
  }
  qsel[0] = lvl;
  qsel[1] = ns;
  qsel[2] = meta[sk * 4 + 0];
  qsel[3] = sk;
}

__global__ void swfd_stack_kernel(const int* __restrict__ qsel_all, const double* __restrict__ buf,
                                  const double* __restrict__ queue, int n2, int n4, int cap, int d, int pend,
// ... 12 lines not shown
                                                                const double* __restrict__ U_all, int ldu, int n4, int ell,
                                                                int cap, const int* __restrict__ qsel_all,
                                                                double* __restrict__ Wq_all,
                                                                double* __restrict__ qinfo_all) {
  __shared__ double lam[1024];
  __shared__ int order[1024];
  __shared__ double scale[512];
  const int t = threadIdx.x, lane = blockIdx.x;
  const double* evals = evals_all + (long)lane * ldu;
  const double* U = U_all + (long)lane * ldu * ldu;
  const int* qsel = qsel_all + (long)lane * (4 + cap);
  double* Wq = Wq_all + (long)lane * ell * n4;
  double* qinfo = qinfo_all + (long)lane * 2;
  if (t < n4) lam[t] = evals[t];
  __syncthreads();
  if (t < n4) {
    const double mine = lam[t];
    int rank = 0;
    for (int j = 0; j < n4; ++j) {
      const double o = lam[j];
      rank += (o > mine) || (o == mine && j < t);
    }
    order[rank] = t;
  }
  __syncthreads();
  const double l0 = lam[order[0]];
  const double delta = lam[order[ell - 1]] > 0.0 ? lam[order[ell - 1]] : 0.0;
  const double tol = 1e-10 * (l0 > 0.0 ? l0 : 0.0);
  if (t < ell) {
    const double l = lam[order[t]];
    double s2 = l - delta;
    s2 = s2 > 0.0 ? s2 : 0.0;
    scale[t] = (s2 > tol) ? sqrt(s2 / l) / l : 0.0;
  }
  if (t == 0) {
    qinfo[0] = (double)qsel[0];
    qinfo[1] = delta;
  }
  __syncthreads();
  for (int e = t; e < ell * n4; e += 1024) {
    const int i = e / n4, a = e - i * n4;
    const double sc = scale[i];
    Wq[e] = (sc != 0.0) ? sc * U[(long)order[i] * ldu + a] : 0.0;
  }
}

__global__ __launch_bounds__(256) void swfd_finish_rows_kernel(double* __restrict__ B, int d, double* __restrict__ sig) {
  __shared__ double sv[4];
  __shared__ int si[4];
  __shared__ double ss[4];
  __shared__ double s_sign;
  const long rowid = (long)blockIdx.y * gridDim.x + blockIdx.x;
  double* row = B + rowid * d;
  double best = -1.0, sq = 0.0;
  int bi = 0x7fffffff;
  for (int c = threadIdx.x; c < d; c += 256) {
    const double v = row[c];
    const double a = fabs(v);
    sq += v * v;
    if (a > best || (a == best && c < bi)) { best = a; bi = c; }
  }
#pragma unroll
  for (int o = 32; o > 0; o >>= 1) {
    const double ob = __shfl_xor(best, o);
    const int oi = __shfl_xor(bi, o);
    sq += __shfl_xor(sq, o);
    if (ob > best || (ob == best && oi < bi)) { best = ob; bi = oi; }
  }
  if ((threadIdx.x & 63) == 0) { sv[threadIdx.x >> 6] = best; si[threadIdx.x >> 6] = bi; ss[threadIdx.x >> 6] = sq; }
  __syncthreads();
  if (threadIdx.x == 0) {
    for (int w = 1; w < 4; ++w)
      if (sv[w] > best || (sv[w] == best && si[w] < bi)) { best = sv[w]; bi = si[w]; }
    s_sign = (row[bi] < 0.0) ? -1.0 : 1.0;
    sig[rowid] = sqrt(ss[0] + ss[1] + ss[2] + ss[3]);
  }
  __syncthreads();
  if (s_sign < 0.0)
    for (int c = threadIdx.x; c < d; c += 256) row[c] = -row[c];
}

static int swfd_query(Swfd* h, double* outB, double* outSigma, double* outInfo, hipStream_t st) {
  const bool small = (h->pend == 0) && h->eigq3;
  EigPlan* const eq = small ? h->eigq3 : h->eigq;
  const int n4 = small ? h->n3 : h->n4, d = h->d, ell = h->ell, B = h->lanes;
  int rc;
  hipLaunchKernelGGL(swfd_select_kernel, dim3(B), dim3(64), 0, st, h->meta, h->qt, h->dropped, h->L, h->cap, h->N,
                     (long long)h->i, h->qsel);
  hipLaunchKernelGGL(swfd_stack_kernel, dim3(n4, B), dim3(256), 0, st, h->qsel, h->buf, h->queue, h->n2, n4, h->cap, d,
                     h->pend, h->stack);
  if ((rc = gemm_f64(true, true, h->stack, d, (long)n4 * d, h->stack, d, (long)n4 * d, eig_plan_input(eq), n4,
                     (long)n4 * n4, n4, n4, d, B, 1.0, st)))
    return rc;
  if ((rc = eig_plan_run_inplace(eq, nullptr, nullptr, st, true))) return rc;
  const EigColumns e = eig_plan_columns(eq);
  hipLaunchKernelGGL(swfd_decide_query_kernel, dim3(B), dim3(1024), 0, st, e.lam, e.cols, e.ld, n4, ell, h->cap, h->qsel, h->Wq,
                     h->qinfo);
  if ((rc = gemm_f64(true, false, h->Wq, n4, (long)ell * n4, h->stack, d, (long)n4 * d, h->Bout, d, (long)ell * d, ell,
                     d, n4, B, 1.0, st)))
    return rc;
  hipLaunchKernelGGL(swfd_finish_rows_kernel, dim3(ell, B), dim3(256), 0, st, h->Bout, d, h->sig_out);
  MUSED_LAUNCH_CHECK();
  MUSED_CHECK_HIP(hipMemcpyAsync(outB, h->Bout, sizeof(double) * (size_t)B * ell * d, hipMemcpyDeviceToDevice, st));
  if (outSigma)
    MUSED_CHECK_HIP(hipMemcpyAsync(outSigma, h->sig_out, sizeof(double) * (size_t)B * ell, hipMemcpyDeviceToDevice, st));
  if (outInfo) MUSED_CHECK_HIP(hipMemcpyAsync(outInfo, h->qinfo, sizeof(double) * 2 * B, hipMemcpyDeviceToDevice, st));
  return MUSED_OK;
}

static size_t swfd_half_bytes(const Swfd* h) {
  const size_t L = h->L;
  return L * ((size_t)h->n2 * h->d * 8 + (size_t)h->cap * h->d * 8 + (size_t)h->cap * 8 + 4 * 4 + 8);
}

}

using namespace mused;

extern "C" {

int mused_swfd_create_lanes(long N, double R, int d, int ell, int sweeps, int lanes, void** out);
int mused_swfd_destroy(void* handle);

int mused_swfd_create(long N, double R, int d, int ell, int sweeps, void** out) {
  return mused_swfd_create_lanes(N, R, d, ell, sweeps, 1, out);
}

static int swfd_create_impl(Swfd* h, long N, double R, int d, int ell, int sweeps, int lanes);

int mused_swfd_create_lanes(long N, double R, int d, int ell, int sweeps, int lanes, void** out) {
  MUSED_REQUIRE(out && N >= 1 && d >= 1 && ell >= 1 && ell <= 256, "mused_swfd_create: need N, d >= 1 and 1 <= sketch_dim <= 256");
  MUSED_REQUIRE(lanes >= 1 && lanes <= 64, "mused_swfd_create_lanes: 1 <= lanes <= 64");
  MUSED_REQUIRE(N < (1l << 31), "mused_swfd_create: N too large");
  CaptureLock resource_guard(capture_mutex());
  Swfd* h = new Swfd();
  memset(h, 0, sizeof(*h));
  const int rc = swfd_create_impl(h, N, R, d, ell, sweeps, lanes);
  if (rc) {
    (void)mused_swfd_destroy(h);
    return rc;
  }
  *out = h;
  return MUSED_OK;
}

static int swfd_create_impl(Swfd* h, long N, double R, int d, int ell, int sweeps, int lanes) {
  h->N = (int)N; h->R = R; h->d = d; h->ell = ell;
  double r1 = R > 1.0 ? R : 1.0;
  int lg = 0;
  while ((double)(1ull << lg) < r1 && lg < 62) ++lg;
  h->L = lg + 1;
  h->lanes = lanes;
  h->S = 2 * h->L * lanes;
  h->cap = 2 * ell;
  h->n2 = 2 * ell;
  h->n4 = 4 * ell;
  h->n3 = (3 * ell + 1) & ~1;
  h->sweeps = sweeps > 0 ? sweeps : 24;
  h->restart_mark = -1;
  h->twin = true;
  const size_t S = h->S, n2 = h->n2, n4 = h->n4, cap = h->cap, dd = d, l = ell;
#define ALLOC(p, bytes) MUSED_CHECK_HIP(hipMalloc((void**)&(p), (bytes)))
#define ZALLOC(p, bytes) do { ALLOC(p, bytes); MUSED_CHECK_HIP(hipMemset((p), 0, (bytes))); } while (0)
  ZALLOC(h->buf, 8 * S * n2 * dd);
  ZALLOC(h->queue, 8 * S * cap * dd);
  ZALLOC(h->qt, 8 * S * cap);
  ZALLOC(h->meta, 4 * S * 4);
  {
    const char* dd = getenv("MUSED_SWFD_DEDUPE");
    if (!(dd && dd[0] == '0')) ALLOC(h->rep, 4 * S);
    const char* sd = getenv("MUSED_SWFD_SKIP_DEAD");
    h->skip_dead = (sd && sd[0] == '0') ? 0 : 1;
  }
  ZALLOC(h->dropped, 8 * S);
  ZALLOC(h->status, 4);
  MUSED_CHECK_HIP(hipHostMalloc((void**)&h->status_host, sizeof(int), hipHostMallocDefault));
  ALLOC(h->theta, 8 * S);
  ALLOC(h->T, 8 * S * l * dd); ALLOC(h->Wc, 8 * S * l * n2);
  ALLOC(h->plan, 4 * S * l * 2); ALLOC(h->keep_src, 4 * S * l); ALLOC(h->now_dev, 8);
  {
    const char* gs = getenv("MUSED_SWFD_GRAM_SPLIT");
    h->gram_split = gs ? atoi(gs) : (d >= 8192 ? 8 : 1);
    if (h->gram_split < 1 || h->gram_split > 16) h->gram_split = 1;
    if (h->gram_split > 1) ALLOC(h->gpart, 8 * S * (size_t)h->gram_split * n2 * n2);
  }
  const size_t Bn = lanes;
  ALLOC(h->stack, 8 * Bn * n4 * dd);
  ALLOC(h->Wq, 8 * Bn * l * n4); ALLOC(h->Bout, 8 * Bn * l * dd); ALLOC(h->sig_out, 8 * Bn * l);
  ALLOC(h->qinfo, 8 * 2 * Bn); ALLOC(h->qsel, 4 * Bn * (4 + cap));
#undef ZALLOC
#undef ALLOC
  std::vector<double> th(S);
  for (int lane = 0; lane < lanes; ++lane)
    for (int kind = 0; kind < 2; ++kind)
      for (int j = 0; j < h->L; ++j) th[sk_index(h, lane, j, kind)] = ldexp((double)h->N / ell, j);
  MUSED_CHECK_HIP(hipMemcpy(h->theta, th.data(), 8 * S, hipMemcpyHostToDevice));
  int rc;
  if ((rc = gemm_f64_prepare_all())) return rc;
  if ((rc = eig_plan_create(h->n2, h->S, h->sweeps, true, &h->eig, h->rep, EIG_PLAN_TOP_HALF, h->status))) return rc;
  if ((rc = eig_plan_create(h->n4, lanes, h->sweeps + 2, true, &h->eigq, nullptr, EIG_PLAN_TOP_FD, h->status, ell))) return rc;
  if (h->n3 < h->n4 &&
      (rc = eig_plan_create(h->n3, lanes, h->sweeps + 2, true, &h->eigq3, nullptr, EIG_PLAN_TOP_FD, h->status, ell)))
    return rc;
  {
    const char* pr = getenv("MUSED_SWFD_PREROT");
    const bool want_pre = pr ? (pr[0] != '0') : !eig_plan_direct_solver(h->eig);
    if (want_pre) {
      const size_t per_block = (size_t)lanes * ell * dd * 8;
      size_t c = ((size_t)256 << 20) / per_block;
      c = c < 1 ? 1 : (c > (size_t)SWFD_PRE_MAX ? (size_t)SWFD_PRE_MAX : c);
      h->pre_chunk = (int)c;
      MUSED_CHECK_HIP(hipMalloc((void**)&h->pre_in, c * per_block));
      MUSED_CHECK_HIP(hipMalloc((void**)&h->pre_out, c * per_block));
      MUSED_CHECK_HIP(hipMalloc((void**)&h->pre_gram, 8 * c * lanes * l * l));
      const char* ps = getenv("MUSED_SWFD_PREROT_SWEEPS");
      const int psw = ps ? atoi(ps) : 5;
      if ((rc = eig_plan_create(h->n2, (int)c * lanes, psw > 0 ? psw : 5, true, &h->eigp, nullptr,
                                EIG_PLAN_FIXED_SWEEPS | EIG_PLAN_NO_SORT, h->status)))
        return rc;
    }
  }
  return MUSED_OK;
}

int mused_swfd_destroy(void* handle) {
  Swfd* h = (Swfd*)handle;
  if (!h) return MUSED_OK;
  CaptureLock resource_guard(capture_mutex());
  eig_plan_destroy(h->eig);
  eig_plan_destroy(h->eigq);
  if (h->eigq3) eig_plan_destroy(h->eigq3);
  if (h->eigp) eig_plan_destroy(h->eigp);
  void* bufs[] = {h->buf, h->queue, h->qt, h->meta, h->dropped, h->theta, h->T, h->Wc, h->plan,
                  h->keep_src, h->now_dev, h->stack, h->Wq, h->Bout, h->sig_out, h->qinfo, h->qsel,
                  h->rep, h->pre_in, h->pre_out, h->pre_gram, h->status, h->gpart};
  for (void* b : bufs) (void)hipFree(b);
  if (h->status_host) (void)hipHostFree(h->status_host);
  delete h;
  return MUSED_OK;
}

int mused_swfd_levels(void* handle) { return handle ? ((Swfd*)handle)->L : -1; }

int mused_swfd_profile(void* handle, int on) {
  Swfd* h = (Swfd*)handle;
  MUSED_REQUIRE(h, "mused_swfd_profile: null handle");
  return eig_plan_profile(h->eig, on != 0);
}

int mused_swfd_profile_read(void* handle, double* total_ms, long* launches, double* bytes_per_launch) {
  Swfd* h = (Swfd*)handle;
  MUSED_REQUIRE(h && total_ms && launches && bytes_per_launch, "mused_swfd_profile_read: null pointer");
  return eig_plan_profile_read(h->eig, total_ms, launches, bytes_per_launch);
}

extern "C" int mused_swfd_profile_read_direct(void* handle, double* total_ms, long* launches, double* matrices_solved,
                                              int* direct, double* tridiag_ms) {
  Swfd* h = (Swfd*)handle;
  MUSED_REQUIRE(h && total_ms && launches && matrices_solved && direct, "mused_swfd_profile_read_direct: null pointer");
  *direct = eig_plan_direct_solver(h->eig) ? 1 : 0;
  return eig_plan_profile_read_direct(h->eig, total_ms, launches, matrices_solved, tridiag_ms);
}

int mused_swfd_append_lanes(void* handle, const void* rows, int dtype, long n_rows, long ld, long lane_stride,
                            void* stream);

int mused_swfd_append(void* handle, const void* rows, int dtype, long n_rows, long ld, void* stream) {
  Swfd* h = (Swfd*)handle;
  MUSED_REQUIRE(h && h->lanes == 1, "mused_swfd_append: this handle has %d lanes, use mused_swfd_append_lanes", h ? h->lanes : 0);
  return mused_swfd_append_lanes(handle, rows, dtype, n_rows, ld, 0, stream);
}

int mused_swfd_append_lanes(void* handle, const void* rows, int dtype, long n_rows, long ld, long lane_stride,
                            void* stream) {
  Swfd* h = (Swfd*)handle;
  MUSED_REQUIRE(h && (rows || n_rows == 0) && n_rows >= 0, "mused_swfd_append: bad arguments");
  hipStream_t st = (hipStream_t)stream;
  if (dtype == MUSED_BITS) {
    MUSED_REQUIRE(ld >= (h->d + 63) / 64, "mused_swfd_append: bit rows need a pitch of at least ceil(d / 64) words");
    return swfd_append_t<BitWord>(h, (const BitWord*)rows, ld, lane_stride, n_rows, st);
  }
  MUSED_REQUIRE(ld >= h->d, "mused_swfd_append: row pitch smaller than d");
  if (dtype == MUSED_F32) return swfd_append_t<float>(h, (const float*)rows, ld, lane_stride, n_rows, st);
  if (dtype == MUSED_F64) return swfd_append_t<double>(h, (const double*)rows, ld, lane_stride, n_rows, st);
  if (dtype == MUSED_I64) return swfd_append_t<long long>(h, (const long long*)rows, ld, lane_stride, n_rows, st);
  set_error("mused_swfd_append: unsupported dtype %d", dtype);
  return MUSED_ERR_UNSUPPORTED;
}

int mused_swfd_lanes(void* handle) { return handle ? ((Swfd*)handle)->lanes : -1; }

int mused_swfd_debug_state(void* handle, int* rep_out, int* meta_out) {
  Swfd* h = (Swfd*)handle;
  if (!h) return MUSED_ERR_ARG;
  MUSED_CHECK_HIP(hipDeviceSynchronize());
  if (h->rep && rep_out) MUSED_CHECK_HIP(hipMemcpy(rep_out, h->rep, 4 * (size_t)h->S, hipMemcpyDeviceToHost));
  if (meta_out) MUSED_CHECK_HIP(hipMemcpy(meta_out, h->meta, 16 * (size_t)h->S, hipMemcpyDeviceToHost));
  return h->rep ? 1 : 0;
}

int mused_swfd_query(void* handle, double* out_sketch, double* out_sigma, double* out_info, void* stream) {
  Swfd* h = (Swfd*)handle;
  MUSED_REQUIRE(h && out_sketch, "mused_swfd_query: null pointer");
  return swfd_query(h, out_sketch, out_sigma, out_info, (hipStream_t)stream);
}

int mused_swfd_status(void* handle, int* status_out, void* stream) {
  Swfd* h = (Swfd*)handle;
  MUSED_REQUIRE(h && status_out, "mused_swfd_status: null pointer");
  MUSED_CHECK_HIP(hipMemcpyAsync(h->status_host, h->status, sizeof(int), hipMemcpyDeviceToHost, (hipStream_t)stream));
  MUSED_CHECK_HIP(hipStreamSynchronize((hipStream_t)stream));
  *status_out = *h->status_host;
  return MUSED_OK;
}

int mused_swfd_counters(void* handle, long* rows_seen, int* pending) {
  Swfd* h = (Swfd*)handle;
  MUSED_REQUIRE(h && rows_seen && pending, "mused_swfd_counters: null pointer");
  *rows_seen = h->i;
  *pending = h->pend;
  return MUSED_OK;
}

long mused_swfd_half_bytes(void* handle) { return handle ? (long)swfd_half_bytes((Swfd*)handle) : -1; }

static int half_copy(Swfd* h, int kind, char* blob, bool to_blob, hipStream_t st) {
  const size_t L = h->L;
  const size_t o = (size_t)kind * L;
  struct Part { char* dev; size_t bytes; };
  Part parts[5] = {
      {(char*)(h->buf + o * h->n2 * h->d), L * h->n2 * h->d * 8},
      {(char*)(h->queue + o * h->cap * h->d), L * (size_t)h->cap * h->d * 8},
      {(char*)(h->qt + o * h->cap), L * (size_t)h->cap * 8},
      {(char*)(h->meta + o * 4), L * 16},
      {(char*)(h->dropped + o), L * 8},
  };
  size_t off = 0;
  for (const Part& p : parts) {
    if (to_blob) MUSED_CHECK_HIP(hipMemcpyAsync(blob + off, p.dev, p.bytes, hipMemcpyDeviceToDevice, st));
    else MUSED_CHECK_HIP(hipMemcpyAsync(p.dev, blob + off, p.bytes, hipMemcpyDeviceToDevice, st));
    off += p.bytes;
  }
  return MUSED_OK;
}

int mused_swfd_export_half(void* handle, int kind, void* dst, void* stream) {
  Swfd* h = (Swfd*)handle;
  MUSED_REQUIRE(h && dst && (kind == 0 || kind == 1), "mused_swfd_export_half: bad arguments");
  MUSED_REQUIRE(h->lanes == 1, "mused_swfd_export_half: single-lane handles only");
  return half_copy(h, kind, (char*)dst, true, (hipStream_t)stream);
}

int mused_swfd_import_half(void* handle, int kind, const void* src, void* stream) {
  Swfd* h = (Swfd*)handle;
  MUSED_REQUIRE(h && src && (kind == 0 || kind == 1), "mused_swfd_import_half: bad arguments");
  MUSED_REQUIRE(h->lanes == 1, "mused_swfd_import_half: single-lane handles only");
  h->twin = false;
  return half_copy(h, kind, (char*)src, false, (hipStream_t)stream);
}

int mused_swfd_begin_epoch(void* handle, long rows_seen, const void* main_half, void* stream) {
  Swfd* h = (Swfd*)handle;
  MUSED_REQUIRE(h && rows_seen >= 0 && rows_seen % h->N == 0, "mused_swfd_begin_epoch: rows_seen must be a multiple of N");
  hipStream_t st = (hipStream_t)stream;
  const size_t S = h->S, L = h->L;
  MUSED_CHECK_HIP(hipMemsetAsync(h->buf, 0, 8 * S * (size_t)h->n2 * h->d, st));
  MUSED_CHECK_HIP(hipMemsetAsync(h->meta, 0, 4 * S * 4, st));
  MUSED_CHECK_HIP(hipMemsetAsync(h->dropped, 0, 8 * S, st));
  MUSED_CHECK_HIP(hipMemsetAsync(h->qt, 0, 8 * S * h->cap, st));
  (void)L;
  if (main_half) {
    MUSED_REQUIRE(h->lanes == 1, "mused_swfd_begin_epoch: a state blob can only be imported into a single-lane handle");
    int rc = half_copy(h, 0, (char*)main_half, false, st);
    if (rc) return rc;
  }
  h->i = rows_seen;
  h->pend = 0;
  h->restart_mark = rows_seen;
  h->twin = (main_half == nullptr);
  return MUSED_OK;
}

}

extern "C" int mused_fd_rotate(double* buf, int ell, int d, double* sigma_out, int sweeps, void* stream) {
  MUSED_REQUIRE(buf && sigma_out && ell >= 1 && d >= 1, "mused_fd_rotate: bad arguments");
  void* hv = nullptr;
  int rc = mused_swfd_create(1l << 30, 1.0, d, ell, sweeps, &hv);
  if (rc) return rc;
  mused::Swfd* h = (mused::Swfd*)hv;
  hipStream_t st = (hipStream_t)stream;
  const size_t bytes = sizeof(double) * (size_t)2 * ell * d;
  hipError_t e = hipMemcpyAsync(h->buf, buf, bytes, hipMemcpyDeviceToDevice, st);
  h->i = 2 * ell;
  if (e == hipSuccess) rc = mused::swfd_rotate_all(h, st);
  if (e == hipSuccess && !rc) e = hipMemcpyAsync(buf, h->buf, bytes, hipMemcpyDeviceToDevice, st);
  if (e == hipSuccess && !rc) {
    hipLaunchKernelGGL(mused::swfd_finish_rows_kernel, dim3(ell), dim3(256), 0, st, buf, d, sigma_out);
    e = hipStreamSynchronize(st);
  }
  mused_swfd_destroy(hv);
  if (rc) return rc;
  MUSED_CHECK_HIP(e);
  return MUSED_OK;
}
```

mused_amd/csrc/trd.hip:

```cpp
#include <stdlib.h>

#include "trd_common.h"

namespace mused {

constexpr int TN = 256, TM = 128, TNT = 512;
constexpr int L_D = 0, L_E = 256, L_LAM = 1024, L_ZS = 1152, L_TAU = 1280, L_MISC = 1536, L_S = 1728;
constexpr int A_XS = 0 , A_VS = 256, A_WS = 512, A_RP = 768 , A_CP = 1792 , A_RED = 2304 , A_SQ = 2312 ;

__host__ __device__ constexpr int tidx(int a, int b) { return a * (a + 1) / 2 + b; }

#ifdef TRD_STEP_PROFILE
#define TRD_TICK(i) do { const long long now_ = clock64(); prof[i] += now_ - last_; last_ = now_; } while (0)
#else
#define TRD_TICK(i) do { } while (0)
#endif
template <int K>
__device__ __forceinline__ void trd_step(double (&A)[2][36], const int k, double* __restrict__ sm, const int t, const int p,
                                         const int q, const int wp, const int wq, double* __restrict__ Hs, long long* prof) {
  const int kk = k & 31, l = t & 63;
#ifdef TRD_STEP_PROFILE
  long long last_ = clock64();
#endif
  double* S = sm + L_S;
// ... 33 lines not shown
    tau = (beta - x0) * trd_rcp(beta);
    scale = trd_rcp(x0 - beta);
  }
  if (t < TN) {
    const double v = (tau != 0.0) ? (t > k + 1 ? xs[t] * scale : (t == k + 1 ? 1.0 : 0.0)) : 0.0;
    vs[t] = v;
    Hs[(long)k * TN + t] = v;
    if (t == 0) {
      sm[L_E + k] = beta;
      sm[L_TAU + k] = tau;
    }
  }
  lds_barrier();
  TRD_TICK(1);
  if (tau == 0.0) return;
  {
    double r[16];
#pragma unroll
    for (int e = 0; e < 16; ++e) r[e] = 0.0;
#pragma unroll
    for (int b = K; b < 8; ++b) {
      const double vj = vs[q + 32 * b];
#pragma unroll
      for (int a = b; a < 8; ++a) {
        r[2 * a] = fma(A[0][tidx(a, b)], vj, r[2 * a]);
        r[2 * a + 1] = fma(A[1][tidx(a, b)], vj, r[2 * a + 1]);
      }
    }
    double c[8];
#pragma unroll
    for (int b = 0; b < 8; ++b) c[b] = 0.0;
    double dpart = 0.0;
#pragma unroll
    for (int u = 0; u < 2; ++u)
#pragma unroll
      for (int a = K; a < 8; ++a) {
        const double vi = vs[p + 16 * u + 32 * a];
        dpart = fma(vi, r[2 * a + u], dpart);
#pragma unroll
        for (int b = K; b <= a; ++b) c[b] = fma(A[u][tidx(a, b)], vi, c[b]);
      }
    const bool h5 = (l & 32) != 0, h4 = (l & 16) != 0, h3 = (l & 8) != 0;
    const bool h2 = (l & 4) != 0, h1 = (l & 2) != 0, h0 = (l & 1) != 0;
    double* rp = S + A_RP + wq * 256;
    double* cpw = S + A_CP + wp * 256;
    if constexpr (K < 4) {
#pragma unroll
      for (int e = 0; e < 8; ++e) r[e] = swap32_add(r[e], r[e + 8]);
#pragma unroll
      for (int e = 0; e < 4; ++e) r[e] = swap16_add(r[e], r[e + 4]);
#pragma unroll
      for (int e = 0; e < 2; ++e) {
        const double keep = h3 ? r[e + 2] : r[e], send = h3 ? r[e] : r[e + 2];
        r[e] = keep + dpp_mov_f64<DPP_ROW_ROR8>(send);
      }
      const int e0 = (h5 ? 8 : 0) + (h4 ? 4 : 0) + (h3 ? 2 : 0);
      rp[p + 16 * e0] = r[0];
      rp[p + 16 * (e0 + 1)] = r[1];
#pragma unroll
      for (int b = 0; b < 4; ++b) {
        const double keep = h2 ? c[b + 4] : c[b], send = h2 ? c[b] : c[b + 4];
        c[b] = keep + dpp_mov_f64<DPP_ROW_HALF_MIRROR>(send);
      }
#pragma unroll
      for (int b = 0; b < 2; ++b) {
        const double keep = h0 ? c[b + 2] : c[b], send = h0 ? c[b] : c[b + 2];
        c[b] = keep + dpp_mov_f64<DPP_QUAD_XOR1>(send);
      }
      {
        const double keep = h1 ? c[1] : c[0], send = h1 ? c[0] : c[1];
        c[0] = keep + dpp_mov_f64<DPP_QUAD_XOR2>(send);
      }
      const int b0 = (h2 ? 4 : 0) + (h0 ? 2 : 0) + (h1 ? 1 : 0);
      cpw[q + 32 * b0] = c[0];
    } else {
#pragma unroll
      for (int e = 0; e < 4; ++e) r[e] = swap32_add(r[8 + e], r[12 + e]);
#pragma unroll
      for (int e = 0; e < 2; ++e) r[e] = swap16_add(r[e], r[e + 2]);
      {
        const double keep = h3 ? r[1] : r[0], send = h3 ? r[0] : r[1];
        r[0] = keep + dpp_mov_f64<DPP_ROW_ROR8>(send);
      }
      rp[p + 16 * (8 + (h5 ? 4 : 0) + (h4 ? 2 : 0) + (h3 ? 1 : 0))] = r[0];
#pragma unroll
      for (int b = 0; b < 2; ++b) {
        const double keep = h2 ? c[6 + b] : c[4 + b], send = h2 ? c[4 + b] : c[6 + b];
        c[b] = keep + dpp_mov_f64<DPP_ROW_HALF_MIRROR>(send);
      }
      {
        const double keep = h0 ? c[1] : c[0], send = h0 ? c[0] : c[1];
        c[0] = keep + dpp_mov_f64<DPP_QUAD_XOR1>(send);
      }
      c[0] = c[0] + dpp_mov_f64<DPP_QUAD_XOR2>(c[0]);
      if (!h1) cpw[q + 32 * (4 + (h2 ? 2 : 0) + (h0 ? 1 : 0))] = c[0];
    }
    dpart = wave_allsum(dpart);
    if (l == 0) S[A_RED + (t >> 6)] = dpart;
  }
  TRD_TICK(2);
  lds_barrier();
  TRD_TICK(3);
  if (t < TN) {
    const double* rp = S + A_RP;
    const double* cp = S + A_CP;
    const double* red = S + A_RED;
    const double y = ((rp[t] + rp[256 + t]) + (rp[512 + t] + rp[768 + t])) + (cp[t] + cp[256 + t]);
    const double dot = 2.0 * (((red[0] + red[1]) + (red[2] + red[3])) + ((red[4] + red[5]) + (red[6] + red[7])));
    const double alpha = -0.5 * tau * tau * dot;
    ws[t] = t > k ? fma(tau, y, alpha * vs[t]) : 0.0;
  }
  lds_barrier();
  TRD_TICK(4);
#pragma unroll
  for (int u = 0; u < 2; ++u) {
    double vi[8], wi[8];
#pragma unroll
    for (int a = K; a < 8; ++a) {
      vi[a] = vs[p + 16 * u + 32 * a];
      wi[a] = ws[p + 16 * u + 32 * a];
    }
#pragma unroll
    for (int b = K; b < 8; ++b) {
      const double vj = vs[q + 32 * b], wj = ws[q + 32 * b];
      const double vjh = 0.5 * vj, wjh = 0.5 * wj;
#pragma unroll
      for (int a = b; a < 8; ++a)
        A[u][tidx(a, b)] = fma(-vi[a], (a == b) ? wjh : wj, fma(-wi[a], (a == b) ? vjh : vj, A[u][tidx(a, b)]));
    }
  }
  TRD_TICK(5);
}

struct L256 {
  static constexpr int TNX = TN, TMX = TM;
  static constexpr long W_HS = 0;
  static constexpr long W_ZG = W_HS + (long)TN * TN;
  static constexpr long W_TG = W_ZG + (long)TN * TM;
  static constexpr long W_LG = W_TG + 3 * TN;
  static constexpr long W_MI = W_LG + 3 * TM;
  static constexpr long W_TM = W_MI + 16;
  static constexpr long W_PER = W_TM + 16 * 256;
};
constexpr long W_HS = L256::W_HS, W_ZG = L256::W_ZG, W_TG = L256::W_TG, W_LG = L256::W_LG, W_MI = L256::W_MI, W_TM = L256::W_TM,
               W_PER = L256::W_PER;

struct TrdDebug {
  long long* clk;
  unsigned long long* work;
};

template <bool EMB>
__global__ __launch_bounds__(TNT, 1) void trd_a_kernel(const double* __restrict__ Gc, const int* __restrict__ rep,
                                                       double* __restrict__ ws, TrdDebug dbg, const TrdShape sh) {
  extern __shared__ __attribute__((aligned(16))) double sm[];
  const int bm = blockIdx.x;
  if (rep && rep[bm] != bm) return;
  const int t = threadIdx.x, w = t >> 6, l = t & 63;
  const int wp = w >> 2, wq = w & 3, lp = l & 7, lq = l >> 3;
  const int p = wp * 8 + lp, q = wq * 8 + lq;
  const int off = EMB ? sh.off : 0, ldn = EMB ? sh.ldn : TN;
  const double* G = Gc + (long)bm * ldn * ldn;
  double* wsm = ws + (long)bm * W_PER;
  double* Hs = wsm + W_HS;
  double* S = sm + L_S;
  double A[2][36];
  const double* Gsrc = G;
  if constexpr (EMB) {
    for (int e = t; e < TN * TN; e += TNT) {
      const int j = e >> 8, i = e & 255;
      Hs[e] = (j >= off && i >= off) ? G[(long)(j - off) * ldn + (i - off)] : 0.0;
    }
    __syncthreads();
    Gsrc = Hs;
  }
#pragma unroll
  for (int u = 0; u < 2; ++u)
#pragma unroll
    for (int a = 0; a < 8; ++a)
#pragma unroll
      for (int b = 0; b <= a; ++b) {
        const int i = p + 16 * u + 32 * a, j = q + 32 * b;
        A[u][tidx(a, b)] = Gsrc[(long)j * TN + i] * (a == b ? 0.5 : 1.0);
      }
  for (int i = t; i < 768; i += TNT) S[A_XS + i] = 0.0;
  if (EMB) {
    __syncthreads();
    if (t < off) {
      sm[L_D + t] = 0.0;
      sm[L_E + t] = 0.0;
      sm[L_TAU + t] = 0.0;
    }
    for (int i = t; i < (off & 15) * TN; i += TNT) Hs[(long)(off & ~15) * TN + i] = 0.0;
  }
  __syncthreads();
  long long prof[6] = {0, 0, 0, 0, 0, 0};
#define TRD_RUN(KV)                                                                           \
  for (int k_ = (EMB && off > 32 * (KV)) ? off : 32 * (KV); k_ < 32 * (KV) + 32 && k_ <= TN - 2; ++k_) \
    trd_step<KV>(A, k_, sm, t, p, q, wp, wq, Hs, prof);
  TRD_RUN(0) TRD_RUN(1) TRD_RUN(2) TRD_RUN(3) TRD_RUN(4) TRD_RUN(5) TRD_RUN(6) TRD_RUN(7)
#undef TRD_RUN
#ifdef TRD_STEP_PROFILE
  if (dbg.clk && t == 0)
    for (int i = 0; i < 6; ++i) dbg.clk[(long)bm * 16 + 8 + i] = prof[i];
#endif
  (void)prof;
  if (p == 15 && q == 31) sm[L_D + TN - 1] = 2.0 * A[1][tidx(7, 7)];
  if (t == 0) { sm[L_E + TN - 1] = 0.0; sm[L_TAU + TN - 1] = 0.0; }
  __syncthreads();
  if (t < TN) {
    wsm[W_TG + t] = sm[L_D + t];
    wsm[W_TG + TN + t] = sm[L_E + t];
    wsm[W_TG + 2 * TN + t] = sm[L_TAU + t];
  }
}

__global__ __launch_bounds__(64) void trd_t_kernel(const int* __restrict__ rep, double* __restrict__ ws, const TrdShape sh) {
  __shared__ double Gs[16][17];
  __shared__ double Ts[16][17];
  const int bm = blockIdx.x >> 4, kb = blockIdx.x & 15;
  if (rep && rep[bm] != bm) return;
  if (16 * kb + 15 < sh.off) return;
  double* wsm = ws + (long)bm * W_PER;
  const double* Hs = wsm + W_HS;
  const int l = threadIdx.x, kq = l >> 4, li = l & 15;
  const int kr = 16 * kb + li;
  const double* vrow = Hs + (long)(kr <= TN - 3 ? kr : 0) * TN;
  const bool okr = kr <= TN - 3;
  v4f64 Ga = {0.0, 0.0, 0.0, 0.0}, Gb = {0.0, 0.0, 0.0, 0.0};
  const int s_lo = (16 * kb) >> 2;
  for (int s4 = s_lo; s4 < TN / 4; s4 += 2) {
    const double a0 = okr ? vrow[4 * s4 + kq] : 0.0;
    const double a1 = okr ? vrow[4 * s4 + 4 + kq] : 0.0;
    Ga = __builtin_amdgcn_mfma_f64_16x16x4f64(a0, a0, Ga, 0, 0, 0);
    Gb = __builtin_amdgcn_mfma_f64_16x16x4f64(a1, a1, Gb, 0, 0, 0);
  }
  Ga += Gb;
#pragma unroll
  for (int r = 0; r < 4; ++r) {
    Gs[kq + 4 * r][li] = Ga[r];
    Ts[kq + 4 * r][li] = 0.0;
  }
  __syncthreads();
  if (l < 16) {
    for (int c = 0; c < 16; ++c) {
      const int kc = 16 * kb + c;
      const double tau = kc <= TN - 3 ? wsm[W_TG + 2 * TN + kc] : 0.0;
      double v = 0.0;
      if (l == c) v = tau;
      else if (l < c) {
        double acc = 0.0;
        for (int b2 = l; b2 < c; ++b2) acc = fma(Ts[l][b2], Gs[b2][c], acc);
        v = -tau * acc;
      }
      Ts[l][c] = v;
    }
  }
  __syncthreads();
#pragma unroll
  for (int r = 0; r < 4; ++r) wsm[W_TM + kb * 256 + (kq + 4 * r) * 16 + li] = Ts[kq + 4 * r][li];
}

constexpr int DM_VA = 0;
constexpr int DM_VB = 4096;
constexpr int DM_TM = DM_VB + 16 * 272;
constexpr int DM_TOTAL = DM_TM + 256;
__global__ __launch_bounds__(TNT, 1) void trd_d_kernel(double* __restrict__ Gc, const int* __restrict__ rep,
                                                       int* __restrict__ done, double* __restrict__ ws, TrdDebug dbg,
                                                       const TrdShape sh, double* __restrict__ lam_out) {
  extern __shared__ __attribute__((aligned(16))) double sm[];
  const int bm = blockIdx.x;
  if (rep && rep[bm] != bm) {
    if (threadIdx.x == 0) done[bm] = 1;
    return;
  }
  const int t = threadIdx.x, w = t >> 6, l = t & 63;
  const int kq = l >> 4, li = l & 15;
  const int off = sh.off, ldn = sh.ldn, n = sh.n;
  double* G = Gc + (long)bm * ldn * ldn;
  double* wsm = ws + (long)bm * W_PER;
  const double* Hs = wsm + W_HS;
  const double* Zg = wsm + W_ZG;
  double* S = sm + L_S;
  int* badflag = reinterpret_cast<int*>(sm + L_MISC + 8);
  if (t < TM) {
    sm[L_LAM + t] = wsm[W_LG + t];
    sm[L_ZS + t] = wsm[W_LG + TM + t];
    sm[L_D + t] = wsm[W_LG + 2 * TM + t];
  }
  if (t == 0) *badflag = reinterpret_cast<const int*>(wsm + W_MI + 2)[0];
  __syncthreads();
  const double lam0 = sm[L_LAM], lamcut = sm[L_LAM + sh.need - 1];
  auto significant = [&](int c) -> bool { return c < sh.nvec && trd_significant(sm[L_LAM + c], c, lam0, lamcut, sh); };
  if (t < 64) {
    double rmax = fmax(significant(t) ? sm[L_D + t] : 0.0, significant(t + 64) ? sm[L_D + t + 64] : 0.0);
#pragma unroll
    for (int o = 32; o > 0; o >>= 1) rmax = fmax(rmax, __shfl_xor(rmax, o));
    if (t == 0) sm[L_MISC + 10] = rmax;
  }
  const int col = 16 * w + li;
  const bool wact = 16 * w < sh.nvec;
  v4f64 Zt[16];
  {
    const double zs = wact ? sm[L_ZS + col] : 0.0;
#pragma unroll
    for (int T = 0; T < 16; ++T)
#pragma unroll
      for (int r = 0; r < 4; ++r) Zt[T][r] = wact ? Zg[(long)(16 * T + kq + 4 * r) * TM + col] * zs : 0.0;
  }
  const int kb_lo = off >> 4;
  auto fetch = [&](int kb, double (&nx)[8], double& tx) {
#pragma unroll
    for (int m = 0; m < 8; ++m) {
      const int idx = t + TNT * m, kr = 16 * kb + (idx >> 8);
      nx[m] = (kb >= kb_lo && kr <= TN - 3) ? Hs[(long)kr * TN + (idx & 255)] : 0.0;
    }
    tx = (kb >= kb_lo && t < 256) ? wsm[W_TM + kb * 256 + t] : 0.0;
  };
  auto store = [&](double* __restrict__ buf, const double (&nx)[8], double tx) {
#pragma unroll
    for (int m = 0; m < 8; ++m) {
      const int idx = t + TNT * m, rr = idx >> 8, row = idx & 255;
      buf[DM_VA + row * 16 + rr] = nx[m];
      buf[DM_VB + rr * 272 + row] = nx[m];
    }
    if (t < 256) buf[DM_TM + t] = tx;
  };
  double nx[8], tx;
  const int kb_top = (TN - 3) >> 4;
  fetch(kb_top, nx, tx);
  {
    double* bnd = S;
    if (li < 4) {
#pragma unroll
      for (int T = 0; T < 16; ++T)
#pragma unroll
        for (int r = 0; r < 4; ++r) bnd[w * 1024 + li * 256 + 16 * T + kq + 4 * r] = Zt[T][r];
    }
    __syncthreads();
    const double* xb = bnd + (w < 7 ? w + 1 : w) * 1024 + (li & 3) * 256;
    double dot[4] = {0.0, 0.0, 0.0, 0.0};
#pragma unroll
    for (int T = 0; T < 16; ++T) {
      if (16 * T + 15 >= off) {
#pragma unroll
        for (int r = 0; r < 4; ++r) {
          const int row = 16 * T + kq + 4 * r;
          const double z = row >= off ? Zt[T][r] : 0.0;
          const double x = row >= off ? xb[row] : 0.0;
#pragma unroll
          for (int dl = 1; dl <= 4; ++dl) {
            const double y = li < dl ? x : z;
            dot[dl - 1] = fma(z, __shfl(y, (l & 48) | ((li + dl) & 15)), dot[dl - 1]);
          }
        }
      }
    }
#pragma unroll
    for (int dl = 1; dl <= 4; ++dl) {
      double dv = dot[dl - 1];
      dv += __shfl_xor(dv, 16);
      dv += __shfl_xor(dv, 32);
      const int c2 = col + dl;
      if (kq == 0 && c2 < TM && significant(col) && significant(c2) && !(fabs(dv) <= TRD_COS_MAX)) atomicOr(badflag, 2);
    }
    const int c = t >> 2;
    if ((t & 3) == 0 && c + 5 < TM && significant(c) && significant(c + 5)) {
      const double width = fmax(1e-7 * lam0, TRD_GAP_PER_RES * sm[L_MISC + 10] * wsm[W_MI]);
      if ((sm[L_LAM + c] - sm[L_LAM + c + 5]) <= width) atomicOr(badflag, 4);
    }
  }
  __syncthreads();
  if (*badflag) {
    if (t == 0) done[bm] = 0;
    return;
  }
  store(S, nx, tx);
  __syncthreads();
  int cur = 0;
  for (int kb = kb_top; kb >= kb_lo; --kb) {
    fetch(kb - 1, nx, tx);
    const double* vA = S + cur * DM_TOTAL + DM_VA;
    const double* vB = S + cur * DM_TOTAL + DM_VB;
    const double* tm = S + cur * DM_TOTAL + DM_TM;
    const int Tlo = wact ? (16 * kb + 1) >> 4 : 16;
    v4f64 Sa = {0.0, 0.0, 0.0, 0.0}, Sb = {0.0, 0.0, 0.0, 0.0};
#pragma unroll
    for (int T = 0; T < 16; ++T) {
      if (T >= Tlo) {
#pragma unroll
        for (int r = 0; r < 4; ++r) {
          const double a = vA[(16 * T + 4 * r + kq) * 16 + li];
          if (T & 1) Sb = __builtin_amdgcn_mfma_f64_16x16x4f64(a, Zt[T][r], Sb, 0, 0, 0);
          else Sa = __builtin_amdgcn_mfma_f64_16x16x4f64(a, Zt[T][r], Sa, 0, 0, 0);
        }
      }
    }
    v4f64 Sw = Sa + Sb;
    v4f64 Cw = {0.0, 0.0, 0.0, 0.0};
#pragma unroll
    for (int s4 = 0; s4 < 4; ++s4) Cw = __builtin_amdgcn_mfma_f64_16x16x4f64(tm[li * 16 + 4 * s4 + kq], Sw[s4], Cw, 0, 0, 0);
    Cw = -Cw;
#pragma unroll
    for (int T = 0; T < 16; ++T) {
      if (T >= Tlo) {
#pragma unroll
        for (int s4 = 0; s4 < 4; ++s4)
          Zt[T] = __builtin_amdgcn_mfma_f64_16x16x4f64(vB[(4 * s4 + kq) * 272 + 16 * T + li], Cw[s4], Zt[T], 0, 0, 0);
      }
    }
    store(S + (cur ^ 1) * DM_TOTAL, nx, tx);
    __syncthreads();
    cur ^= 1;
  }
  {
    const int ncol = n < sh.nvec ? n : sh.nvec;
    const bool cval = col < ncol;
    const double lc = cval ? sm[L_LAM + col] : 0.0;
    const double f = lc > 0.0 ? lc : 0.0;
    double* tr = S + w * (16 * 132 + 64);
#pragma unroll
    for (int h = 0; h < 2; ++h) {
#pragma unroll
      for (int T = 0; T < 8; ++T)
#pragma unroll
        for (int r = 0; r < 4; ++r) tr[li * 132 + 16 * T + kq + 4 * r] = cval ? f * Zt[8 * h + T][r] : 0.0;
      __syncthreads();
      for (int c = 0; c < 16; ++c) {
        const int cc = 16 * w + c;
        if (cc < ldn) {
#pragma unroll
          for (int g = 0; g < 2; ++g) {
            const int i = 128 * h + 64 * g + l - off;
            if (i >= 0) G[(long)cc * ldn + i] = tr[c * 132 + 64 * g + l];
          }
        }
      }
      __syncthreads();
    }
    if (ldn > TM) {
      double* Z0 = G + (long)TM * ldn;
      const int nz = (ldn - TM) * ldn;
      if ((ldn & 1) == 0 && (reinterpret_cast<unsigned long long>(Z0) & 15ull) == 0ull) {
        double2* Z2 = reinterpret_cast<double2*>(Z0);
        for (int idx = t; idx < nz / 2; idx += TNT) Z2[idx] = make_double2(0.0, 0.0);
      } else {
        for (int idx = t; idx < nz; idx += TNT) Z0[idx] = 0.0;
      }
    }
    if (lam_out && t < ldn) {
      const double lv = t < ncol ? sm[L_LAM + t] : 0.0;
      lam_out[(long)bm * ldn + t] = (lv > 0.0 && lv * lv > 0.0) ? lv : 0.0;
    }
    const int npad = ldn - n;
    for (int idx = t; idx < npad * (ldn < TM ? ldn : TM); idx += TNT) {
      const int c = idx / npad;
      G[(long)c * ldn + n + (idx - c * npad)] = 0.0;
    }
  }
  if (t == 0) {
    done[bm] = 1;
    if (dbg.work) atomicAdd(dbg.work, 1ull);
  }
}

}

namespace mused {

size_t trd_workspace_doubles(int batch) { return (size_t)batch * (size_t)W_PER; }

constexpr int L_A_TOTAL = L_S + 2314;
constexpr int L_DM_TOTAL = L_S + 2 * DM_TOTAL;
constexpr int C_LDS = trd_c_lds_doubles<L256, 32>();

int trd_prepare() {
  static std::once_flag once;
  static hipError_t rc = hipSuccess;
  std::call_once(once, [] {
    rc = hipFuncSetAttribute((const void*)trd_d_kernel, hipFuncAttributeMaxDynamicSharedMemorySize, (int)(sizeof(double) * L_DM_TOTAL));
    if (rc == hipSuccess)
      rc = hipFuncSetAttribute((const void*)trd_c_kernel<L256, 32>, hipFuncAttributeMaxDynamicSharedMemorySize, (int)(sizeof(double) * C_LDS));
  });
  MUSED_CHECK_HIP(rc);
  return MUSED_OK;
}

long trd_tail_ws_per() { return W_PER; }
long trd_tail_off_hs() { return W_HS; }
long trd_tail_off_tg() { return W_TG; }
int trd_tail_launch(const double* G, const int* rep, double* ws, int batch, hipStream_t st) {
  TrdDebug dbg{nullptr, nullptr};
  TrdShape sh;
  sh.n = TN; sh.ldn = TN; sh.off = 0; sh.nvec = TM; sh.need = TM; sh.cert_all = 0;
  hipLaunchKernelGGL(trd_a_kernel<false>, dim3(batch), dim3(TNT), sizeof(double) * L_A_TOTAL, st, G, rep, ws, dbg, sh);
  MUSED_LAUNCH_CHECK();
  return MUSED_OK;
}

bool trd_supports(int n, int ldn, int need) { return n >= 2 && n <= TN && ldn >= n && ldn <= TN && need >= 1 && need <= TM && need <= n; }

int trd_solve(double* Gc, int n, int ldn, int need, bool cert_all, int batch, const int* rep, int* done, double* ws,
              hipStream_t st, long long* dbg_clk, unsigned long long* work, hipEvent_t after_a, double* lam_out) {
  MUSED_REQUIRE(trd_supports(n, ldn, need), "trd_solve: unsupported shape (n=%d, ld=%d, need=%d)", n, ldn, need);
  TrdDebug dbg{dbg_clk, work};
  TrdShape sh;
  sh.n = n; sh.ldn = ldn; sh.off = TN - n;
  sh.nvec = ((need + 31) / 32) * 32;
  sh.need = need;
  sh.cert_all = cert_all ? 1 : 0;
  const int nch = sh.nvec / 32;
  if (n == TN && ldn == TN) hipLaunchKernelGGL(trd_a_kernel<false>, dim3(batch), dim3(TNT), sizeof(double) * L_A_TOTAL, st, Gc, rep, ws, dbg, sh);
  else hipLaunchKernelGGL(trd_a_kernel<true>, dim3(batch), dim3(TNT), sizeof(double) * L_A_TOTAL, st, Gc, rep, ws, dbg, sh);
  if (after_a) MUSED_CHECK_HIP(hipEventRecord(after_a, st));
  if (batch <= 64) hipLaunchKernelGGL((trd_b_kernel<128, L256>), dim3(nch * batch), dim3(128), 0, st, rep, ws, sh);
  else hipLaunchKernelGGL((trd_b_kernel<512, L256>), dim3(batch), dim3(512), 0, st, rep, ws, sh);
  hipLaunchKernelGGL((trd_c_kernel<L256, 32>), dim3(nch * batch), dim3(128), sizeof(double) * C_LDS, st, rep, ws, sh);
  hipLaunchKernelGGL(trd_t_kernel, dim3(16 * batch), dim3(64), 0, st, rep, ws, sh);
  hipLaunchKernelGGL(trd_d_kernel, dim3(batch), dim3(TNT), sizeof(double) * L_DM_TOTAL, st, Gc, rep, done, ws, dbg, sh, lam_out);
  MUSED_LAUNCH_CHECK();
  return MUSED_OK;
}

__global__ void trd_export_kernel(const double* __restrict__ ws, double* __restrict__ d, double* __restrict__ e,
                                  double* __restrict__ lam, double* __restrict__ res) {
  const int bm = blockIdx.x, t = threadIdx.x;
  const double* wsm = ws + (long)bm * W_PER;
  if (d) d[(long)bm * TN + t] = wsm[W_TG + t];
  if (e) e[(long)bm * TN + t] = wsm[W_TG + TN + t];
  if (t < TM) {
    if (lam) lam[(long)bm * TM + t] = wsm[W_LG + t];
    if (res) res[(long)bm * TM + t] = wsm[W_LG + 2 * TM + t];
  }
}

}

using namespace mused;

extern "C" int mused_debug_trd_n(double* G, int n, int need, int cert_all, int batch, double* out_d, double* out_e,
                                 double* out_lam, double* out_res, int* out_done, void* stream) {
  MUSED_REQUIRE(G && batch >= 1 && out_done, "mused_debug_trd: bad arguments");
  int rc = trd_prepare();
  if (rc) return rc;
  hipStream_t st = (hipStream_t)stream;
  double* ws = nullptr;
  MUSED_CHECK_HIP(hipMalloc((void**)&ws, sizeof(double) * trd_workspace_doubles(batch)));
  rc = trd_solve(G, n, n, need, cert_all != 0, batch, nullptr, out_done, ws, st);
  if (!rc) hipLaunchKernelGGL(trd_export_kernel, dim3(batch), dim3(TN), 0, st, ws, out_d, out_e, out_lam, out_res);
  hipError_t e = hipStreamSynchronize(st);
  (void)hipFree(ws);
  if (rc) return rc;
  MUSED_CHECK_HIP(e);
  return MUSED_OK;
}

extern "C" int mused_debug_trd(double* G, int batch, double* out_d, double* out_e, double* out_lam, double* out_res,
                               int* out_done, void* stream) {
  return mused_debug_trd_n(G, TN, TM, 0, batch, out_d, out_e, out_lam, out_res, out_done, stream);
}

extern "C" int mused_debug_trd_time_n(const double* G, int n, int need, int batch, int reps, double* out_ms, int* out_done,
                                      long long* out_clk, void* stream) {
  MUSED_REQUIRE(G && batch >= 1 && reps >= 1 && out_ms, "mused_debug_trd_time: bad arguments");
  hipStream_t st = (hipStream_t)stream;
  int rc = trd_prepare();
  if (rc) return rc;
  double *ws = nullptr, *work = nullptr;
  int* done = nullptr;
  const size_t bytes = sizeof(double) * (size_t)batch * n * n;
  MUSED_CHECK_HIP(hipMalloc((void**)&ws, sizeof(double) * trd_workspace_doubles(batch)));
  MUSED_CHECK_HIP(hipMalloc((void**)&work, bytes));
  MUSED_CHECK_HIP(hipMalloc((void**)&done, sizeof(int) * (size_t)batch));
  hipEvent_t e0, e1;
  MUSED_CHECK_HIP(hipEventCreate(&e0));
  MUSED_CHECK_HIP(hipEventCreate(&e1));
  double total = 0.0;
  for (int i = 0; i <= reps && !rc; ++i) {
    MUSED_CHECK_HIP(hipMemcpyAsync(work, G, bytes, hipMemcpyDeviceToDevice, st));
    MUSED_CHECK_HIP(hipEventRecord(e0, st));
    rc = trd_solve(work, n, n, need, false, batch, nullptr, done, ws, st, out_clk);
    MUSED_CHECK_HIP(hipEventRecord(e1, st));
    MUSED_CHECK_HIP(hipEventSynchronize(e1));
    float ms = 0.f;
    MUSED_CHECK_HIP(hipEventElapsedTime(&ms, e0, e1));
    if (i > 0) total += ms;
  }
  *out_ms = total / reps;
  if (out_done) MUSED_CHECK_HIP(hipMemcpy(out_done, done, sizeof(int) * (size_t)batch, hipMemcpyDeviceToHost));
  (void)hipEventDestroy(e0);
  (void)hipEventDestroy(e1);
  (void)hipFree(ws); (void)hipFree(work); (void)hipFree(done);
  return rc;
}

extern "C" int mused_debug_trd_time(const double* G, int batch, int reps, double* out_ms, int* out_done, long long* out_clk,
                                    void* stream) {
  return mused_debug_trd_time_n(G, TN, TM, batch, reps, out_ms, out_done, out_clk, stream);
}
```

mused_amd/csrc/trd_common.h:

```cpp
#pragma once
#include <math.h>

#include <type_traits>

#include "internal.h"
#include "wave_ops.h"

namespace mused {

typedef double v4f64 __attribute__((ext_vector_type(4)));

constexpr double TRD_RES_MAX = 1e-13, TRD_COS_MAX = 1e-8, TRD_GAP_PER_RES = 2e8, TRD_COS_REORTH = 1e-10;

__device__ __forceinline__ void lds_barrier() { asm volatile("s_waitcnt lgkmcnt(0)\n\ts_barrier" ::: "memory"); }

__device__ __forceinline__ double trd_rcp(double y) {
  double r = __builtin_amdgcn_rcp(y);
  r = fma(fma(-y, r, 1.0), r, r);
  r = fma(fma(-y, r, 1.0), r, r);
  return r;
}

struct TrdShape {
  int n, ldn, off;
  int nvec;
  int need;
  int cert_all;
};

__device__ __forceinline__ bool trd_significant(double lc, int c, double lam0, double lamcut, const TrdShape& sh) {
  if (c >= sh.need || !(lc > 0.0)) return false;
  const double l0 = lam0 > 0.0 ? lam0 : 0.0;
  return sh.cert_all ? (lc > 1e-24 * l0) : ((lc - lamcut) > 1e-10 * l0);
}


template <int TNX>
__device__ __forceinline__ int trd_sturm(const double2* __restrict__ dd2, double x) {
  static_assert(TNX % 8 == 0 && TNX >= 24, "trd_sturm: the order must be a multiple of 8");
  double p0 = 1.0, p1 = dd2[0].x - x;
  unsigned bits = (unsigned)__double2hiint(p1) >> 31;
  int cnt = (int)bits;
  auto row = [&](const double2 de) {
    const double p2 = fma(de.x - x, p1, -(de.y * p0));
    bits = __builtin_amdgcn_alignbit(bits, (unsigned)__double2hiint(p2), 31);
    p0 = p1;
    p1 = p2;
  };
  auto rescale = [&]() {
    const unsigned e1 = __builtin_amdgcn_ubfe((unsigned)__double2hiint(p1), 20, 11), e0 = __builtin_amdgcn_ubfe((unsigned)__double2hiint(p0), 20, 11);
    const double f = __hiloint2double((int)((2046u - max(e1, e0)) << 20), 0);
    p1 *= f;
    p0 *= f;
  };
  auto flush = [&](unsigned mask) {
    cnt += __builtin_popcount((bits ^ (bits >> 1)) & mask);
    bits &= 1u;
  };
  constexpr int NBLK = TNX / 8 - 1, NLOOP = NBLK - 1;
  constexpr int PENDING = (NLOOP % 3) * 8 + 15;
  double2 cur[8];
#pragma unroll
  for (int j = 0; j < 8; ++j) cur[j] = dd2[1 + j];
#pragma unroll 3
  for (int b = 0; b < NLOOP; ++b) {
    double2 nxt[8];
#pragma unroll
    for (int j = 0; j < 8; ++j) nxt[j] = dd2[9 + 8 * b + j];
#pragma unroll
    for (int j = 0; j < 8; ++j) row(cur[j]);
    rescale();
#pragma unroll
    for (int j = 0; j < 8; ++j) cur[j] = nxt[j];
    if (b % 3 == 2) flush(0x00ffffffu);
  }
  {
    double2 nxt[8];
#pragma unroll
    for (int j = 0; j < 8; ++j) nxt[j] = dd2[TNX - 7 + j];
#pragma unroll
    for (int j = 0; j < 8; ++j) row(cur[j]);
    rescale();
#pragma unroll
    for (int j = 0; j < 7; ++j) row(nxt[j]);
  }
  flush((PENDING >= 32) ? 0xffffffffu : ((1u << PENDING) - 1u));
  return cnt;
}

template <int NTB, typename LY>
__global__ __launch_bounds__(NTB) void trd_b_kernel(const int* __restrict__ rep, double* __restrict__ ws, const TrdShape sh) {
  constexpr int TNX = LY::TNX, NWV = NTB / 64;
  const int NCH = NTB == 512 ? 1 : sh.nvec / (NTB / 4);
  constexpr int PASSES = 19, NPT = 512;
  __shared__ __attribute__((aligned(16))) double2 dd2[TNX + 8];
  __shared__ double part[3 * NWV];
  __shared__ double scal[4];
  __shared__ int cnts[NPT];
  const int bm = blockIdx.x / NCH, cq = blockIdx.x % NCH;
  if (rep && rep[bm] != bm) return;
  const int t = threadIdx.x, w = t >> 6, l = t & 63;
  double* wsm = ws + (long)bm * LY::W_PER;
  const double* dg = wsm + LY::W_TG;
  const double* eg = wsm + LY::W_TG + TNX;
  double lo = 1.7976931348623157e308, hi = -1.7976931348623157e308, e2m = 0.0;
  for (int i = t; i < TNX; i += NTB) {
    const double di = dg[i], em = i > 0 ? eg[i - 1] : 0.0, ep = eg[i];
    const double rad = fabs(em) + fabs(ep);
    lo = fmin(lo, di - rad);
    hi = fmax(hi, di + rad);
    e2m = fmax(e2m, ep * ep);
  }
#pragma unroll
  for (int o = 32; o > 0; o >>= 1) {
    lo = fmin(lo, __shfl_xor(lo, o));
    hi = fmax(hi, __shfl_xor(hi, o));
    e2m = fmax(e2m, __shfl_xor(e2m, o));
  }
  if (l == 0) { part[3 * w] = lo; part[3 * w + 1] = hi; part[3 * w + 2] = e2m; }
  __syncthreads();
  if (t == 0) {
    for (int ww = 1; ww < NWV; ++ww) { lo = fmin(lo, part[3 * ww]); hi = fmax(hi, part[3 * ww + 1]); e2m = fmax(e2m, part[3 * ww + 2]); }
    const double tn = fmax(fabs(lo), fabs(hi));
    const double piv = 2.2250738585072014e-308 * fmax(1.0, e2m);
    int ks = (tn > 0.0 && tn < 1.7976931348623157e308) ? __builtin_amdgcn_frexp_exp(tn) : 0;
    ks = ks > 1000 ? 1000 : (ks < -1000 ? -1000 : ks);
    const double sc = __builtin_amdgcn_ldexp(1.0, -ks);
    scal[0] = (lo - 2.0 * tn * 2.220446049250313e-16 * TNX - 2.0 * piv) * sc;
    scal[1] = (hi + 2.0 * tn * 2.220446049250313e-16 * TNX + 2.0 * piv) * sc;
    scal[2] = sc;
    scal[3] = __builtin_amdgcn_ldexp(1.0, ks);
    if (cq == 0) {
      wsm[LY::W_MI] = tn;
      wsm[LY::W_MI + 1] = piv;
      reinterpret_cast<int*>(wsm + LY::W_MI + 2)[0] = 0;
    }
  }
  __syncthreads();
  const double gl = scal[0], gu = scal[1], sc = scal[2], unsc = scal[3];
  for (int i = t; i < TNX; i += NTB) {
    const double es_ = (i > 0 ? eg[i - 1] : 0.0) * sc;
    dd2[i] = make_double2(dg[i] * sc, fmax(es_ * es_, 7.52316384526264e-37));
  }
  if (t < 8) dd2[TNX + t] = make_double2(0.0, 0.0);
  __syncthreads();
  const double h0 = (gu - gl) * (1.0 / (double)(NPT + 1));
  for (int i = t; i < NPT; i += NTB) cnts[i] = trd_sturm<TNX>(dd2, fma(h0, (double)(i + 1), gl));
  __syncthreads();
  const int r = cq * (NTB / 4) + (t >> 2), s = t & 3, jidx = TNX - 1 - r;
  if (r >= sh.nvec) return;
  int first = 0;
  for (int step = NPT / 2; step > 0; step >>= 1)
    if (first + step <= NPT && cnts[first + step - 1] <= jidx) first += step;
  if (first < NPT && cnts[first] <= jidx) first += 1;
  lo = first == 0 ? gl : fma(h0, (double)first, gl);
  hi = first >= NPT ? gu : fma(h0, (double)(first + 1), gl);
  for (int it = 0; it < PASSES; ++it) {
    const double h = (hi - lo) * 0.2;
    const double x = fma(h, (double)(s + 1), lo);
    const int above = trd_sturm<TNX>(dd2, x) > jidx ? 0 : 1;
    int nf = above;
    nf += __builtin_amdgcn_mov_dpp(nf, DPP_QUAD_XOR1, 0xf, 0xf, false);
    nf += __builtin_amdgcn_mov_dpp(nf, DPP_QUAD_XOR2, 0xf, 0xf, false);
    const double nlo = fma(h, (double)nf, lo);
    hi = (nf == 4) ? hi : fma(h, (double)(nf + 1), lo);
    lo = nlo;
  }
  if (s == 0) wsm[LY::W_LG + r] = 0.5 * (lo + hi) * unsc;
}

template <typename LY, int VPW>
constexpr int trd_c_lds_doubles() { return 2 * LY::TNX + LY::TNX + 4 * VPW + 2 * LY::TNX * VPW; }

template <typename LY, int VPW>
__global__ __launch_bounds__(128) void trd_c_kernel(const int* __restrict__ rep, double* __restrict__ ws, const TrdShape sh) {
  constexpr int TNX = LY::TNX, TMX = LY::TMX;
  static_assert(TNX % 32 == 0 && (VPW == 8 || VPW == 16 || VPW == 32), "trd_c_kernel: unsupported shape");
  extern __shared__ __attribute__((aligned(16))) double smc[];
  double2* dd2 = reinterpret_cast<double2*>(smc);
  double* es = smc + 2 * TNX;
  double* xch = es + TNX;
  double* qp = xch + 4 * VPW;
  double* qm = qp + TNX * VPW;
  const int nch = sh.nvec / VPW;
  const int bm = blockIdx.x / nch, cq = blockIdx.x - bm * nch;
  if (rep && rep[bm] != bm) return;
  const int t = threadIdx.x, role = t >> 6, l = t & 63;
  double* wsm = ws + (long)bm * LY::W_PER;
  double* Zg = wsm + LY::W_ZG;
  for (int i = t; i < TNX; i += 128) {
    const double em = i > 0 ? wsm[LY::W_TG + TNX + i - 1] : 0.0;
    dd2[i] = make_double2(wsm[LY::W_TG + i], em * em);
    es[i] = wsm[LY::W_TG + TNX + i];
  }
  __syncthreads();
  const double tnorm = wsm[LY::W_MI], pivmin = wsm[LY::W_MI + 1];
  const double lam0 = wsm[LY::W_LG], lamcut = wsm[LY::W_LG + sh.need - 1];
  const bool act = l < VPW;
  const int cl = l & (VPW - 1), c = cq * VPW + cl;
  const double lam = wsm[LY::W_LG + c];
  auto guard = [&](double v) -> double { return fabs(v) < pivmin ? -pivmin : v; };
  if (act) {
    if (role == 0) {
      double qv = dd2[0].x - lam;
      qp[cl] = qv;
      auto stretch = [&](const int i0, auto cnt) {
        constexpr int CNT = decltype(cnt)::value;
        double2 de[CNT];
#pragma unroll
        for (int j = 0; j < CNT; ++j) de[j] = dd2[i0 + j];
#pragma unroll
        for (int j = 0; j < CNT; ++j) {
          qv = fma(-de[j].y, trd_rcp(guard(qv)), de[j].x - lam);
          qp[(i0 + j) * VPW + cl] = qv;
        }
      };
      for (int i0 = 1; i0 + 8 <= TNX; i0 += 8) stretch(i0, std::integral_constant<int, 8>());
      stretch(TNX - 7, std::integral_constant<int, 7>());
    } else {
      double qv = dd2[TNX - 1].x - lam;
      qm[(TNX - 1) * VPW + cl] = qv;
      auto stretch = [&](const int i0, auto cnt) {
        constexpr int CNT = decltype(cnt)::value;
        double dx[CNT], e2[CNT];
#pragma unroll
        for (int j = 0; j < CNT; ++j) {
          dx[j] = dd2[i0 - j].x - lam;
          e2[j] = dd2[i0 - j + 1].y;
        }
#pragma unroll
        for (int j = 0; j < CNT; ++j) {
          qv = fma(-e2[j], trd_rcp(guard(qv)), dx[j]);
          qm[(i0 - j) * VPW + cl] = qv;
        }
      };
      for (int i0 = TNX - 2; i0 >= 7; i0 -= 8) stretch(i0, std::integral_constant<int, 8>());
      stretch(6, std::integral_constant<int, 7>());
    }
  }
  __syncthreads();
  if (act) {
    const int i0 = role * (TNX / 2);
    double best = 1.7976931348623157e308;
    int kt = i0;
    for (int ib = i0; ib < i0 + TNX / 2; ib += 16) {
      double a[16], b[16];
#pragma unroll
      for (int j = 0; j < 16; ++j) {
        a[j] = qp[(ib + j) * VPW + cl];
        b[j] = qm[(ib + j) * VPW + cl];
      }
#pragma unroll
      for (int j = 0; j < 16; ++j) {
        const double g = fabs((a[j] + b[j]) - (dd2[ib + j].x - lam));
        if (g < best) { best = g; kt = ib + j; }
      }
    }
    xch[cl * 4 + role] = best;
    xch[cl * 4 + 2 + role] = (double)kt;
  }
  __syncthreads();
  int kt = 0;
  double gbest = 0.0;
  if (act) {
    const double b0 = xch[cl * 4], b1 = xch[cl * 4 + 1];
    const bool up = !(b1 < b0);
    gbest = up ? b0 : b1;
    kt = (int)(up ? xch[cl * 4 + 2] : xch[cl * 4 + 3]);
  }
  __syncthreads();
  if (act) {
    double ss = 0.0, zc = 1.0;
    if (role == 0) {
      Zg[(long)kt * TMX + c] = 1.0;
      for (int ib = kt - 1; ib >= 0; ib -= 8) {
        double qq[8], ee[8];
#pragma unroll
        for (int j = 0; j < 8; ++j) {
          const int i = ib - j;
          qq[j] = i >= 0 ? qp[i * VPW + cl] : 1.0;
          ee[j] = i >= 0 ? es[i] : 0.0;
        }
#pragma unroll
        for (int j = 0; j < 8; ++j) {
          zc = -ee[j] * zc * trd_rcp(guard(qq[j]));
          if (ib - j >= 0) Zg[(long)(ib - j) * TMX + c] = zc;
          ss = fma(zc, zc, ss);
        }
      }
    } else {
      for (int ib = kt + 1; ib < TNX; ib += 8) {
        double qq[8], ee[8];
#pragma unroll
        for (int j = 0; j < 8; ++j) {
          const int i = ib + j;
          qq[j] = i < TNX ? qm[i * VPW + cl] : 1.0;
          ee[j] = i < TNX ? es[i - 1] : 0.0;
        }
#pragma unroll
        for (int j = 0; j < 8; ++j) {
          zc = -ee[j] * zc * trd_rcp(guard(qq[j]));
          if (ib + j < TNX) Zg[(long)(ib + j) * TMX + c] = zc;
          ss = fma(zc, zc, ss);
        }
      }
    }
    xch[cl * 4 + role] = ss;
  }
  __syncthreads();
  if (cq == 0 && t == 0 && !(fabs(lam0) <= 1.7976931348623157e308 && tnorm <= 1.7976931348623157e308))
    atomicOr(reinterpret_cast<int*>(wsm + LY::W_MI + 2), 1);
  if (act && role == 0) {
    const double ss = 1.0 + xch[cl * 4] + xch[cl * 4 + 1];
    const double zs = 1.0 / sqrt(ss);
    wsm[LY::W_LG + TMX + c] = zs;
    const double res = gbest * zs / (tnorm > 0.0 ? tnorm : 1.0);
    wsm[LY::W_LG + 2 * TMX + c] = res;
    if (trd_significant(lam, c, lam0, lamcut, sh) && !(ss < 1e300 && res <= TRD_RES_MAX))
      atomicOr(reinterpret_cast<int*>(wsm + LY::W_MI + 2), 1);
  }
}

}
```

mused_amd/csrc/trdx.hip:

```cpp
#include <stdlib.h>

#include "trd_common.h"

namespace mused {

constexpr int XRB = 64;
constexpr int XTAIL = 256;

template <int NX>
struct LX {
  static constexpr int TNX = NX, TMX = NX / 2, NBLK = NX / XRB;
  static constexpr long W_A = 0;
  static constexpr long W_HS = W_A + (long)NX * NX;
  static constexpr long W_ZG = W_HS + (long)NX * NX;
  static constexpr long W_ZB = W_ZG + (long)NX * TMX;
  static constexpr long W_TG = W_ZB + (long)NX * TMX;
  static constexpr long W_LG = W_TG + 3 * NX;
  static constexpr long W_MI = W_LG + 3 * TMX;
  static constexpr long W_TF = W_MI + 16;
  static constexpr long W_PER = W_TF + (long)NBLK * XRB * XRB;
  static_assert(W_PER % 2 == 0 && NX % 64 == 0, "layout");
};

__device__ __forceinline__ double wave_treduce32(double (&r)[32], const int l, int& idx) {
// ... 618 lines not shown
      if (tt >= kb) {
        __syncthreads();
        vchunk_store(Vs, VP, t, stg);
        __syncthreads();
        if (tt + 1 < TPW) vchunk_load(Hs, NX, kb, tt + 1, t, stg);
#pragma unroll
        for (int s = 0; s < 4; ++s) {
          double a[4];
#pragma unroll
          for (int mi = 0; mi < 4; ++mi) a[mi] = Vs[(16 * mi + li) * VP + 16 * w + kq + 4 * s];
#pragma unroll
          for (int mi = 0; mi < 4; ++mi)
#pragma unroll
            for (int ct = 0; ct < CT; ++ct)
              sp[mi][ct] = __builtin_amdgcn_mfma_f64_16x16x4f64(a[mi], z[tt][ct][s], sp[mi][ct], 0, 0, 0);
        }
      }
    }
    for (int ww = 0; ww < 4; ++ww) {
      if (w == ww) {
#pragma unroll
        for (int mi = 0; mi < 4; ++mi)
#pragma unroll
          for (int ct = 0; ct < CT; ++ct)
#pragma unroll
            for (int r = 0; r < 4; ++r) {
              double* ps = Ss + (16 * mi + kq + 4 * r) * SP + 16 * ct + li;
              *ps = (ww == 0) ? sp[mi][ct][r] : *ps + sp[mi][ct][r];
            }
      }
      __syncthreads();
    }
    {
      v4f64 cc[CT];
#pragma unroll
      for (int ct = 0; ct < CT; ++ct) cc[ct] = (v4f64){0.0, 0.0, 0.0, 0.0};
#pragma unroll
      for (int s = 0; s < 16; ++s)
#pragma unroll
        for (int ct = 0; ct < CT; ++ct)
          cc[ct] = __builtin_amdgcn_mfma_f64_16x16x4f64(tf[s], Ss[K::kmap(s, kq) * SP + 16 * ct + li], cc[ct], 0, 0, 0);
#pragma unroll
      for (int ct = 0; ct < CT; ++ct)
#pragma unroll
        for (int r = 0; r < 4; ++r) Cs[(16 * w + kq + 4 * r) * SP + 16 * ct + li] = cc[ct][r];
    }
    vchunk_load(Hs, NX, kb, kb, t, stg);
#pragma unroll
    for (int tt = 0; tt < TPW; ++tt) {
      if (tt >= kb) {
        __syncthreads();
        vchunk_store(Vs, VP, t, stg);
        __syncthreads();
        if (tt + 1 < TPW) vchunk_load(Hs, NX, kb, tt + 1, t, stg);
#pragma unroll
        for (int s = 0; s < 16; ++s) {
          const int kr = K::kmap(s, kq);
          const double a = -Vs[kr * VP + 16 * w + li];
#pragma unroll
          for (int ct = 0; ct < CT; ++ct)
            z[tt][ct] = __builtin_amdgcn_mfma_f64_16x16x4f64(a, Cs[kr * SP + 16 * ct + li], z[tt][ct], 0, 0, 0);
        }
      }
    }
    __syncthreads();
  }
#pragma unroll
  for (int ct = 0; ct < CT; ++ct) {
    const int col = c0 + 16 * ct + li;
#pragma unroll
    for (int tt = 0; tt < TPW; ++tt)
#pragma unroll
      for (int r = 0; r < 4; ++r) wsm[LY::W_ZB + (long)(64 * tt + 16 * w + kq + 4 * r) * TMX + col] = z[tt][ct][r];
  }
}

template <typename LY>
__global__ __launch_bounds__(256) void trdx_store_kernel(const int* __restrict__ act, const double* __restrict__ ws,
                                                         double* __restrict__ Gc, const TrdShape sh, double* __restrict__ lam_out) {
  constexpr int TNX = LY::TNX, TMX = LY::TMX, NT = TNX / 64;
  __shared__ double tile[64][65];
  const int bm = blockIdx.y;
  if (act[bm] != bm) return;
  const int ti = blockIdx.x / NT, tc = blockIdx.x % NT;
  const double* wsm = ws + (long)bm * LY::W_PER;
  const double* Zb = wsm + LY::W_ZB;
  double* G = Gc + (long)bm * TNX * TNX;
  if (lam_out && blockIdx.x == 0)
    for (int cc = threadIdx.x; cc < TNX; cc += 256) {
      const double lv = cc < sh.nvec ? wsm[LY::W_LG + cc] : 0.0;
      lam_out[(long)bm * TNX + cc] = (lv > 0.0 && lv * lv > 0.0) ? lv : 0.0;
    }
  const int tx = threadIdx.x & 63, ty = threadIdx.x >> 6;
  const int c = 64 * tc + tx;
  const double lc = c < sh.nvec ? wsm[LY::W_LG + c] : 0.0;
  const double f = lc > 0.0 ? lc : 0.0;
  for (int r = ty; r < 64; r += 4) tile[r][tx] = (c < sh.nvec) ? f * Zb[(long)(64 * ti + r) * TMX + c] : 0.0;
  __syncthreads();
  for (int cc = ty; cc < 64; cc += 4) G[(long)(64 * tc + cc) * TNX + 64 * ti + tx] = tile[tx][cc];
}

template <typename LY>
__global__ void trdx_export_kernel(const double* __restrict__ ws, double* __restrict__ d, double* __restrict__ e,
                                   double* __restrict__ lam, double* __restrict__ res, int nvec) {
  const int bm = blockIdx.x, t = threadIdx.x;
  const double* wsm = ws + (long)bm * LY::W_PER;
  if (d) d[(long)bm * LY::TNX + t] = wsm[LY::W_TG + t];
  if (e) e[(long)bm * LY::TNX + t] = wsm[LY::W_TG + LY::TNX + t];
  if (t < nvec) {
    if (lam) lam[(long)bm * LY::TMX + t] = wsm[LY::W_LG + t];
    if (res) res[(long)bm * LY::TMX + t] = wsm[LY::W_LG + 2 * LY::TMX + t];
  }
}

template <int NX>
static int trdx_prepare_t() {
  using LY = LX<NX>;
  static std::once_flag once;
  static hipError_t rc = hipSuccess;
  std::call_once(once, [] {
    rc = hipFuncSetAttribute((const void*)trdx_a_kernel<NX>, hipFuncAttributeMaxDynamicSharedMemorySize,
                             (int)(sizeof(double) * trdx_a_lds_doubles<NX>()));
    if (rc == hipSuccess)
      rc = hipFuncSetAttribute((const void*)trd_c_kernel<LY, XA<NX>::VPW>, hipFuncAttributeMaxDynamicSharedMemorySize,
                               (int)(sizeof(double) * trd_c_lds_doubles<LY, XA<NX>::VPW>()));
    if (rc == hipSuccess)
      rc = hipFuncSetAttribute((const void*)trdx_tfac_kernel<NX>, hipFuncAttributeMaxDynamicSharedMemorySize,
                               (int)(sizeof(double) * TF_LDS_DOUBLES));
    if (rc == hipSuccess)
      rc = hipFuncSetAttribute((const void*)trdx_back_kernel<NX>, hipFuncAttributeMaxDynamicSharedMemorySize,
                               (int)(sizeof(double) * XZ<NX>::LDS_DOUBLES));
  });
  MUSED_CHECK_HIP(rc);
  return trd_prepare();
}

template <int NX>
static int trdx_solve_t(double* Gc, const TrdShape& sh, int batch, const int* rep, int* done, int* act, int* jrep, int* nrej,
                        double* ws, hipStream_t st, unsigned long long* work, hipEvent_t after_a, long long* prof, double* lam_out) {
  using LY = LX<NX>;
  constexpr int VPW = XA<NX>::VPW;
  const int nvec = sh.nvec, nch32 = nvec / 32, nchc = nvec / VPW;
  double* g22 = ws + (size_t)batch * LY::W_PER;
  double* wst = g22 + (size_t)batch * XTAIL * XTAIL;
  hipLaunchKernelGGL(trdx_a_kernel<NX>, dim3(batch), dim3(XA<NX>::NT), sizeof(double) * trdx_a_lds_doubles<NX>(), st, Gc, rep, ws, prof,
                     g22);
  if (after_a) MUSED_CHECK_HIP(hipEventRecord(after_a, st));
  {
    const int rc_t = trd_tail_launch(g22, rep, wst, batch, st);
    if (rc_t) return rc_t;
  }
  hipLaunchKernelGGL(trdx_tail_merge_kernel<NX>, dim3(XTAIL, batch), dim3(256), 0, st, rep, ws, wst, trd_tail_ws_per(), trd_tail_off_hs(),
                     trd_tail_off_tg());
  hipLaunchKernelGGL((trd_b_kernel<128, LY>), dim3(nch32 * batch), dim3(128), 0, st, rep, ws, sh);
  constexpr size_t c_lds = sizeof(double) * trd_c_lds_doubles<LY, VPW>();
  hipLaunchKernelGGL((trd_c_kernel<LY, VPW>), dim3(nchc * batch), dim3(128), c_lds, st, rep, ws, sh);
  hipLaunchKernelGGL(trdx_cert_kernel<LY>, dim3(batch), dim3(256), 0, st, rep, ws, done, act, jrep, nrej, work, sh);
  MUSED_LAUNCH_CHECK();
  hipLaunchKernelGGL(trdx_tfac_kernel<NX>, dim3(LY::NBLK, batch), dim3(256), sizeof(double) * TF_LDS_DOUBLES, st, act, ws);
  hipLaunchKernelGGL(trdx_back_kernel<NX>, dim3(nvec / XZ<NX>::NC, batch), dim3(256), sizeof(double) * XZ<NX>::LDS_DOUBLES, st, act,
                     ws, sh);
  hipLaunchKernelGGL(trdx_store_kernel<LY>, dim3((NX / 64) * (NX / 64), batch), dim3(256), 0, st, act, ws, Gc, sh, lam_out);
  MUSED_LAUNCH_CHECK();
  return MUSED_OK;
}

bool trdx_supports(int ldn, int need) {
  const bool order = (ldn >= 320 && ldn <= 512 && ldn % 64 == 0) || (ldn >= 640 && ldn <= 1024 && ldn % 128 == 0);
  return order && need >= 1 && ((need + 31) / 32) * 32 <= ldn / 2;
}

#define TRDX_DISPATCH(ldn, EXPR) \
  switch (ldn) {                 \
    case 320: EXPR(320); break;  \
    case 384: EXPR(384); break;  \
    case 448: EXPR(448); break;  \
    case 512: EXPR(512); break;  \
    case 640: EXPR(640); break;  \
    case 768: EXPR(768); break;  \
    case 896: EXPR(896); break;  \
    default: EXPR(1024); break;  \
  }

size_t trdx_workspace_doubles(int ldn, int batch) {
#define TRDX_WS(NX) return (size_t)batch * ((size_t)LX<NX>::W_PER + (size_t)XTAIL * XTAIL + (size_t)trd_tail_ws_per())
  TRDX_DISPATCH(ldn, TRDX_WS)
  return 0;
}

int trdx_prepare(int ldn) {
  MUSED_REQUIRE(trdx_supports(ldn, 1), "trdx_prepare: unsupported order %d", ldn);
#define TRDX_PREP(NX) return trdx_prepare_t<NX>()
  TRDX_DISPATCH(ldn, TRDX_PREP)
  return MUSED_OK;
}

int trdx_solve(double* Gc, int ldn, int need, bool cert_all, int batch, const int* rep, int* done, int* act, int* jrep,
               int* nrej, double* ws, hipStream_t st, unsigned long long* work, hipEvent_t after_a, long long* prof,
               double* lam_out) {
  MUSED_REQUIRE(trdx_supports(ldn, need), "trdx_solve: unsupported shape (order %d, need %d)", ldn, need);
  TrdShape sh;
  sh.n = ldn; sh.ldn = ldn; sh.off = 0;
  sh.nvec = ((need + 31) / 32) * 32;
  sh.need = need;
  sh.cert_all = cert_all ? 1 : 0;
#define TRDX_SOLVE(NX) return trdx_solve_t<NX>(Gc, sh, batch, rep, done, act, jrep, nrej, ws, st, work, after_a, prof, lam_out)
  TRDX_DISPATCH(ldn, TRDX_SOLVE)
  return MUSED_OK;
}

}

using namespace mused;

extern "C" int mused_debug_trdx(double* G, int n, int need, int cert_all, int batch, double* out_d, double* out_e,
                                double* out_lam, double* out_res, int* out_done, void* stream) {
  MUSED_REQUIRE(G && batch >= 1 && out_done && trdx_supports(n, need), "mused_debug_trdx: bad arguments");
  int rc = trdx_prepare(n);
  if (rc) return rc;
  hipStream_t st = (hipStream_t)stream;
  double* ws = nullptr;
  int* ib = nullptr;
  MUSED_CHECK_HIP(hipMalloc((void**)&ws, sizeof(double) * trdx_workspace_doubles(n, batch)));
  MUSED_CHECK_HIP(hipMalloc((void**)&ib, sizeof(int) * (2 * (size_t)batch + 1)));
  MUSED_CHECK_HIP(hipMemsetAsync(ib + 2 * batch, 0, sizeof(int), st));
  rc = trdx_solve(G, n, need, cert_all != 0, batch, nullptr, out_done, ib, ib + batch, ib + 2 * batch, ws, st, nullptr, nullptr);
  if (!rc) {
    const int nvec = ((need + 31) / 32) * 32;
#define TRDX_EXPORT(NX) hipLaunchKernelGGL((trdx_export_kernel<LX<NX>>), dim3(batch), dim3(NX), 0, st, ws, out_d, out_e, out_lam, out_res, nvec)
    TRDX_DISPATCH(n, TRDX_EXPORT)
  }
  hipError_t e = hipStreamSynchronize(st);
  (void)hipFree(ws);
  (void)hipFree(ib);
  if (rc) return rc;
  MUSED_CHECK_HIP(e);
  return MUSED_OK;
}

extern "C" int mused_debug_trdx_time(const double* G, int n, int need, int batch, int reps, double* out_ms, double* out_a_ms,
                                     int* out_done, long long* out_prof, void* stream) {
  MUSED_REQUIRE(G && batch >= 1 && reps >= 1 && out_ms && trdx_supports(n, need), "mused_debug_trdx_time: bad arguments");
  hipStream_t st = (hipStream_t)stream;
  int rc = trdx_prepare(n);
  if (rc) return rc;
  double *ws = nullptr, *work = nullptr;
  int* ib = nullptr;
  const size_t bytes = sizeof(double) * (size_t)batch * n * n;
  MUSED_CHECK_HIP(hipMalloc((void**)&ws, sizeof(double) * trdx_workspace_doubles(n, batch)));
  MUSED_CHECK_HIP(hipMalloc((void**)&work, bytes));
  MUSED_CHECK_HIP(hipMalloc((void**)&ib, sizeof(int) * (3 * (size_t)batch + 1)));
  MUSED_CHECK_HIP(hipMemset(ib + 3 * batch, 0, sizeof(int)));
  hipEvent_t e0, e1, ea;
  MUSED_CHECK_HIP(hipEventCreate(&e0));
  MUSED_CHECK_HIP(hipEventCreate(&e1));
  MUSED_CHECK_HIP(hipEventCreate(&ea));
  double total = 0.0, total_a = 0.0;
  for (int i = 0; i <= reps && !rc; ++i) {
    MUSED_CHECK_HIP(hipMemcpyAsync(work, G, bytes, hipMemcpyDeviceToDevice, st));
    MUSED_CHECK_HIP(hipEventRecord(e0, st));
    rc = trdx_solve(work, n, need, false, batch, nullptr, ib, ib + batch, ib + 2 * batch, ib + 3 * batch, ws, st, nullptr, ea, out_prof);
    MUSED_CHECK_HIP(hipEventRecord(e1, st));
    MUSED_CHECK_HIP(hipEventSynchronize(e1));
    float ms = 0.f, msa = 0.f;
    MUSED_CHECK_HIP(hipEventElapsedTime(&ms, e0, e1));
    MUSED_CHECK_HIP(hipEventElapsedTime(&msa, e0, ea));
    if (i > 0) { total += ms; total_a += msa; }
  }
  *out_ms = total / reps;
  if (out_a_ms) *out_a_ms = total_a / reps;
  if (out_done) MUSED_CHECK_HIP(hipMemcpy(out_done, ib, sizeof(int) * (size_t)batch, hipMemcpyDeviceToHost));
  (void)hipEventDestroy(e0);
  (void)hipEventDestroy(e1);
  (void)hipEventDestroy(ea);
  (void)hipFree(ws); (void)hipFree(work); (void)hipFree(ib);
  return rc;
}
```

Baseline: 552,600 rows/s.

## Compact active SWFD slots into a sorted list and trim per-matrix work

The rep kernel now runs as a single 1024-thread block that ranks active slots by their fill count and writes a compacted list, per-slot active K lengths, and per-matrix order offsets. The Gram GEMM, split-K reduce, trd eigensolver kernels and the queue prep then index through this list, so blocks map straight to live matrices instead of exiting early. The GEMM can also cut K to the active rows, and trd can solve smaller effective orders via offsets when n equals 256. This trades an O(S^2) rank computation in one block and extra indirection for fewer wasted blocks and less arithmetic on partly filled buffers.

```diff
diff --git a/mused_amd/csrc/eig.hip b/mused_amd/csrc/eig.hip
--- a/mused_amd/csrc/eig.hip
+++ b/mused_amd/csrc/eig.hip
@@ -54,6 +54,8 @@
   double* Gc = nullptr;
   double* lam = nullptr;
   const int* rep = nullptr;
+  const int* list = nullptr;
+  const int* offs = nullptr;
   const int* jrep = nullptr;
   int* err_out = nullptr;
   double* trace = nullptr;
@@ -770,8 +772,8 @@
 
 __global__ __launch_bounds__(1024) void osjq_prep_direct_kernel(OsjqCtl* __restrict__ ctl, unsigned* __restrict__ q, unsigned qcap,
                                                                int* __restrict__ qdone, int* __restrict__ qclean, int batch,
-                                                               int upr, const int* __restrict__ rep, const int* __restrict__ skip,
-                                                               const double* __restrict__ Gc, int ldn, int nflag,
+                                                               int upr, const int* __restrict__ rep, const int* __restrict__ list,
+                                                               const int* __restrict__ skip, const double* __restrict__ Gc, int ldn, int nflag,
                                                                double* __restrict__ trace, int* __restrict__ notconv) {
   __shared__ int s_dirty;
   const int t = threadIdx.x;
@@ -784,10 +786,15 @@
     ctl->head = 0; ctl->tail = 0; ctl->finished = 0; ctl->nmat = 0; ctl->all_done = 0; ctl->error = 0; ctl->dirty = 0;
   }
   __syncthreads();
-  for (int m = t; m < batch; m += 1024) {
-    qdone[m] = 0;
-    qclean[m] = 0;
-    if (rep && rep[m] != m) continue;
+  for (int i = t; i < batch; i += 1024) {
+    qdone[i] = 0;
+    qclean[i] = 0;
+  }
+  __syncthreads();
+  const int nrun = list ? list[0] : batch;
+  for (int i = t; i < nrun; i += 1024) {
+    const int m = list ? list[1 + i] : i;
+    if (!list && rep && rep[m] != m) continue;
     if (skip && skip[m]) continue;
     if (trace) {
       const double* M = Gc + (long)m * ldn * ldn;
@@ -811,7 +818,7 @@
   const bool behind_direct = p->c.direct == EigDirect::Trd;
   if (behind_direct) {
     hipLaunchKernelGGL(osjq_prep_direct_kernel, dim3(1), dim3(1024), 0, st, p->qctl, p->q, p->qcap, p->qdone, p->qclean, p->batch,
-                       upr, p->rep, p->trd_done, p->Gc, ldn, p->notconv ? p->sweeps * p->c.rps : 0, p->notconv ? p->trace : nullptr,
+                       upr, p->rep, p->list, p->trd_done, p->Gc, ldn, p->notconv ? p->sweeps * p->c.rps : 0, p->notconv ? p->trace : nullptr,
                        p->notconv);
   } else {
     hipLaunchKernelGGL(osjq_zero_kernel, dim3(cdiv(p->qcap, 1024)), dim3(1024), 0, st, p->q, p->qcap, p->qctl);
@@ -1063,7 +1070,7 @@
 }
 
 int eig_plan_create(int n, int batch, int sweeps, bool own_graph, EigPlan** out, const int* rep, int flags, int* err_out,
-                    int need) {
+                    int need, const int* list, const int* offs) {
   MUSED_REQUIRE(n >= 2 && n % 2 == 0 && n <= 1024 && batch >= 1 && sweeps >= 1,
                 "eig_plan_create: the order must be even and <= 1024 (n=%d)", n);
   CaptureLock resource_guard(capture_mutex());
@@ -1073,6 +1080,10 @@
   p->rep = p->jrep = rep;
   p->err_out = err_out;
   p->c = eig_choose(n, batch, sweeps, flags, need, env);
+  if (p->c.direct == EigDirect::Trd) {
+    p->list = list;
+    if (n == 256 && p->c.ldn == 256) p->offs = offs;
+  }
   const int rc = eig_plan_create_impl(p, env, own_graph);
   if (rc) {
     eig_plan_destroy(p);
@@ -1181,7 +1192,7 @@
   int rc;
   if (p->c.direct == EigDirect::Trd) {
     rc = trd_solve(p->Gc, p->n, p->c.ldn, p->c.need, p->c.cert_all, p->batch, p->rep, p->trd_done, p->trd_ws, st, nullptr, work,
-                   after_a, p->lam);
+                   after_a, p->lam, p->list, p->offs);
   } else {
     MUSED_CHECK_HIP(hipMemsetAsync(p->trdx_nrej, 0, sizeof(int), st));
     rc = trdx_solve(p->Gc, p->c.ldn, p->c.need, p->c.cert_all, p->batch, p->rep, p->trd_done, p->trdx_act, p->trdx_jrep,
diff --git a/mused_amd/csrc/gemm_f64.h b/mused_amd/csrc/gemm_f64.h
--- a/mused_amd/csrc/gemm_f64.h
+++ b/mused_amd/csrc/gemm_f64.h
@@ -24,6 +24,8 @@
   int bsplit;
   int tiles_m, tiles_n;
   const int* rep;
+  const int* list;
+  const int* kact;
   int sym;
 };
 
@@ -217,9 +219,14 @@
 __global__ __launch_bounds__(GEMM_THREADS, 2) void gemm_f64_kernel(GemmArgs g, Epi epi) {
   extern __shared__ __attribute__((aligned(16))) double smem[];
 
-  const int z = blockIdx.z;
-  const int zb = g.bsplit ? z / g.bsplit : z;
-  if (g.rep && g.rep[zb] != zb) return;
+  int z = blockIdx.z;
+  int zb = g.bsplit ? z / g.bsplit : z;
+  if (g.list) {
+    if (zb >= g.list[0]) return;
+    const int e = g.list[1 + zb];
+    z += (e - zb) * (g.bsplit ? g.bsplit : 1);
+    zb = e;
+  } else if (g.rep && g.rep[zb] != zb) return;
   int tm, tn;
   if (g.sym) {
     const int t = g.tiles_n, nwg = t * (t + 1) / 2;
@@ -256,6 +263,8 @@
     if (g.bsplit) {
       k_lo = (z - zb * g.bsplit) * g.kchunk;
       k_hi = min(g.K, k_lo + g.kchunk);
+    } else if (g.kact) {
+      k_hi = min(g.K, g.kact[zb]);
     }
   }
 
diff --git a/mused_amd/csrc/gemm_f64.hip b/mused_amd/csrc/gemm_f64.hip
--- a/mused_amd/csrc/gemm_f64.hip
+++ b/mused_amd/csrc/gemm_f64.hip
@@ -27,12 +27,12 @@
 
 int gemm_f64(bool a_kc, bool b_kc, const double* A, long lda, long strideA, const double* B, long ldb,
              long strideB, double* C, long ldc, long strideC, int M, int N, int K, int batch, double alpha,
-             hipStream_t stream, const int* rep) {
+             hipStream_t stream, const int* rep, const int* list, const int* kact) {
   GemmArgs g;
   memset(&g, 0, sizeof(g));
   g.A = A; g.B = B; g.lda = lda; g.ldb = ldb; g.strideA = strideA; g.strideB = strideB;
   g.M = M; g.N = N; g.K = K; g.splitk = 0; g.kchunk = 0;
-  g.rep = rep;
+  g.rep = rep; g.list = list; g.kact = kact;
   g.sym = (A == B && a_kc == b_kc && lda == ldb && strideA == strideB && M == N) ? 1 : 0;
   EpiStore epi{C, ldc, strideC, alpha};
   const bool vec = vec_ok<double>(A, lda, strideA) && vec_ok<double>(B, ldb, strideB);
@@ -69,14 +69,14 @@
 
 int gemm_f64_batched_splitk(bool a_kc, bool b_kc, const double* A, long lda, long strideA, const double* B, long ldb, long strideB,
                             double* partial, int M, int N, int K, int batch, int kchunk, int nsplit, hipStream_t stream,
-                            const int* rep) {
+                            const int* rep, const int* list) {
   MUSED_REQUIRE(kchunk > 0 && kchunk % GEMM_BK == 0 && nsplit >= 1 && (long)kchunk * nsplit >= K,
                 "gemm_f64_batched_splitk: bad kchunk %d x %d for K=%d", kchunk, nsplit, K);
   GemmArgs g;
   memset(&g, 0, sizeof(g));
   g.A = A; g.B = B; g.lda = lda; g.ldb = ldb; g.strideA = strideA; g.strideB = strideB;
   g.M = M; g.N = N; g.K = K; g.splitk = 0; g.kchunk = kchunk; g.bsplit = nsplit;
-  g.rep = rep;
+  g.rep = rep; g.list = list;
   g.sym = (A == B && a_kc == b_kc && lda == ldb && strideA == strideB && M == N) ? 1 : 0;
   EpiStore epi{partial, (long)N, (long)M * N, 1.0};
   const bool vec = vec_ok<double>(A, lda, strideA) && vec_ok<double>(B, ldb, strideB);
@@ -87,9 +87,12 @@
 }
 
 __global__ void batched_splitk_reduce_kernel(const double* __restrict__ partial, int nsplit, long count, double* __restrict__ out,
-                                             const int* __restrict__ rep) {
-  const int z = blockIdx.y;
-  if (rep && rep[z] != z) return;
+                                             const int* __restrict__ rep, const int* __restrict__ list) {
+  int z = blockIdx.y;
+  if (list) {
+    if (z >= list[0]) return;
+    z = list[1 + z];
+  } else if (rep && rep[z] != z) return;
   const long i = (long)blockIdx.x * blockDim.x + threadIdx.x;
   if (i >= count) return;
   const double* p = partial + (long)z * nsplit * count + i;
@@ -99,9 +102,9 @@
 }
 
 int gemm_batched_splitk_reduce(const double* partial, int nsplit, long count, double* out, int batch, const int* rep,
-                               hipStream_t stream) {
+                               hipStream_t stream, const int* list) {
   hipLaunchKernelGGL(batched_splitk_reduce_kernel, dim3(cdiv(count, 256), batch), dim3(256), 0, stream, partial, nsplit, count, out,
-                     rep);
+                     rep, list);
   MUSED_LAUNCH_CHECK();
   return MUSED_OK;
 }
@@ -147,6 +150,13 @@
                          alpha, (hipStream_t)stream, rep);
 }
 
+int mused_debug_gemm_f64_batched_active(int a_kc, int b_kc, const double* A, long lda, long strideA, const double* B, long ldb,
+                                        long strideB, double* C, long ldc, long strideC, int M, int N, int K, int batch,
+                                        double alpha, const int* list, const int* kact, void* stream) {
+  return mused::gemm_f64(a_kc != 0, b_kc != 0, A, lda, strideA, B, ldb, strideB, C, ldc, strideC, M, N, K, batch,
+                         alpha, (hipStream_t)stream, nullptr, list, kact);
+}
+
 int mused_gemm_f64_splitk(int a_kc, int b_kc, const double* A, long lda, const double* B, long ldb, double* partial,
                           double* C, int M, int N, int K, int kchunk, int nsplit, void* stream) {
   MUSED_REQUIRE(A && B && partial && C && M >= 0 && N >= 0 && K >= 0, "mused_gemm_f64_splitk: bad arguments");
diff --git a/mused_amd/csrc/internal.h b/mused_amd/csrc/internal.h
--- a/mused_amd/csrc/internal.h
+++ b/mused_amd/csrc/internal.h
@@ -21,13 +21,13 @@
 
 int gemm_f64(bool a_kc, bool b_kc, const double* A, long lda, long strideA, const double* B, long ldb,
              long strideB, double* C, long ldc, long strideC, int M, int N, int K, int batch, double alpha,
-             hipStream_t stream, const int* rep = nullptr);
+             hipStream_t stream, const int* rep = nullptr, const int* list = nullptr, const int* kact = nullptr);
 
 int gemm_f64_batched_splitk(bool a_kc, bool b_kc, const double* A, long lda, long strideA, const double* B, long ldb, long strideB,
                             double* partial, int M, int N, int K, int batch, int kchunk, int nsplit, hipStream_t stream,
-                            const int* rep = nullptr);
+                            const int* rep = nullptr, const int* list = nullptr);
 int gemm_batched_splitk_reduce(const double* partial, int nsplit, long count, double* out, int batch, const int* rep,
-                               hipStream_t stream);
+                               hipStream_t stream, const int* list = nullptr);
 int gemm_f64_prepare_all();
 
 int gemm_f64_splitk(bool a_kc, bool b_kc, const double* A, long lda, const double* B, long ldb, double* partial,
@@ -52,7 +52,7 @@
 constexpr int EIG_PLAN_TOP_NEED = 8;
 constexpr int EIG_PLAN_TOP_FD = 16;
 int eig_plan_create(int n, int batch, int sweeps, bool own_graph, EigPlan** out, const int* rep = nullptr, int flags = 0,
-                    int* err_out = nullptr, int need = 0);
+                    int* err_out = nullptr, int need = 0, const int* list = nullptr, const int* offs = nullptr);
 void eig_plan_destroy(EigPlan* p);
 double* eig_plan_input(EigPlan* p);
 int eig_plan_run_inplace(EigPlan* p, double* evals, double* V, hipStream_t stream, bool allow_graph);
@@ -77,7 +77,9 @@
 int trd_tail_launch(const double* G, const int* rep, double* ws, int batch, hipStream_t st);
 int trd_solve(double* Gc, int n, int ldn, int need, bool cert_all, int batch, const int* rep, int* done, double* ws,
               hipStream_t st, long long* dbg_clk = nullptr, unsigned long long* work = nullptr, hipEvent_t after_a = nullptr,
-              double* lam_out = nullptr);
+              double* lam_out = nullptr,
+              const int* list = nullptr,
+              const int* offs = nullptr);
 
 bool trdx_supports(int ldn, int need);
 size_t trdx_workspace_doubles(int ldn, int batch);
diff --git a/mused_amd/csrc/swfd.hip b/mused_amd/csrc/swfd.hip
--- a/mused_amd/csrc/swfd.hip
+++ b/mused_amd/csrc/swfd.hip
@@ -19,6 +19,11 @@
   long long* qt;
   int* meta;
   int* rep;
+  int* list;
+  int* offs;
+  int oround;
+  int* kact;
+  long long* ostat;
   long long* dropped;
   double* theta;
   double *T, *Wc;
@@ -85,31 +90,63 @@
 
 __global__ void swfd_set_now_kernel(long long* now, long long v) { *now = v; }
 
-__global__ void swfd_rep_kernel(const int* __restrict__ meta, int L, int nchains, int* __restrict__ rep, int twin,
-                                const long long* __restrict__ dropped, long long epoch_start, int skip_dead,
-                                long long* __restrict__ now_dev, long long now) {
-  const int c = blockIdx.x * blockDim.x + threadIdx.x;
-  if (c == 0) *now_dev = now;
-  if (c >= nchains) return;
-  const int base = ((twin && (c & 1)) ? c - 1 : c) * L;
-  if (twin && (c & 1)) {
+constexpr int SWFD_OFFS_ROUND = 16;
+__global__ __launch_bounds__(1024) void swfd_rep_kernel(const int* __restrict__ meta, int L, int nchains, int* __restrict__ rep,
+                                                        int twin, const long long* __restrict__ dropped, long long epoch_start,
+                                                        int skip_dead, long long* __restrict__ now_dev, long long now, int pend,
+                                                        int ell, int n2, int* __restrict__ list, int* __restrict__ offs,
+                                                        int* __restrict__ kact, long long* __restrict__ ostat, int oround) {
+  extern __shared__ int s_key[];
+  __shared__ int s_hist[17];
+  const int t = threadIdx.x, S = nchains * L;
+  if (t == 0) *now_dev = now;
+  if (t < 17) s_hist[t] = 0;
+  auto put = [&](int s, int r) {
+    rep[s] = r;
+    const int na = meta[s * 4 + 0] + pend;
+    s_key[s] = (r == s) ? (na < n2 ? na : n2) : -1;
+  };
+  for (int c = t; c < nchains; c += 1024) {
+    const int base = ((twin && (c & 1)) ? c - 1 : c) * L;
+    if (twin && (c & 1)) {
+      int r = base + L - 1;
+      put(c * L + L - 1, r);
+      for (int j = L - 2; j >= 0; --j) {
+        if (meta[(base + j) * 4 + 3] != 0) r = base + j;
+        put(c * L + j, r);
+      }
+      continue;
+    }
+    const bool dead_ok = skip_dead && !twin && (c & 1) == 0;
     int r = base + L - 1;
-    rep[c * L + L - 1] = r;
+    put(r, r);
     for (int j = L - 2; j >= 0; --j) {
       if (meta[(base + j) * 4 + 3] != 0) r = base + j;
-      rep[c * L + j] = r;
-    }
-    return;
-  }
-  int r = base + L - 1;
-  rep[r] = r;
-  for (int j = L - 2; j >= 0; --j) {
-    if (meta[(base + j) * 4 + 3] != 0) r = base + j;
-    rep[base + j] = r;
-  }
-  if (skip_dead && !twin && (c & 1) == 0)
-    for (int j = 0; j < L - 1; ++j)
-      if (dropped[base + j] > epoch_start) rep[base + j] = -1;
+      put(base + j, (dead_ok && dropped[base + j] > epoch_start) ? -1 : r);
+    }
+  }
+  __syncthreads();
+  if (!list) return;
+  for (int s = t; s < S; s += 1024) {
+    const int key = s_key[s];
+    if (key < 0) continue;
+    int rank = 0;
+    for (int j = 0; j < S; ++j) {
+      const int kj = s_key[j];
+      rank += (kj > key) || (kj == key && j < s);
+    }
+    list[1 + rank] = s;
+    const int n = offs ? n2 - ((n2 - (key > ell ? key : ell)) & ~(oround - 1)) : n2;
+    if (offs) offs[s] = n2 - n;
+    if (kact) kact[s] = min(n2, (key + 15) & ~15);
+    atomicAdd(&s_hist[16], 1);
+    atomicAdd(&s_hist[(n - 1) >> 4 < 16 ? (n - 1) >> 4 : 15], 1);
+  }
+  __syncthreads();
+  if (t == 0) list[0] = s_hist[16];
+  if (t == 0) ostat[0] += 1;
+  if (t == 1) ostat[1] += s_hist[16];
+  if (t < 16) ostat[2 + t] += s_hist[t];
 }
 
 __global__ __launch_bounds__(1024) void swfd_decide_kernel(const double* __restrict__ evals,
@@ -258,26 +295,27 @@
   const int S = h->S, n2 = h->n2, d = h->d, ell = h->ell;
   int rc;
   if (h->rep)
-    hipLaunchKernelGGL(swfd_rep_kernel, dim3(cdiv(2 * h->lanes, 64)), dim3(64), 0, st, h->meta, h->L, 2 * h->lanes, h->rep,
+    hipLaunchKernelGGL(swfd_rep_kernel, dim3(1), dim3(1024), sizeof(int) * (size_t)S, st, h->meta, h->L, 2 * h->lanes, h->rep,
                        h->twin ? 1 : 0, h->dropped, (long long)(((h->i - 1) / h->N) * h->N), h->skip_dead, h->now_dev,
-                       (long long)h->i);
+                       (long long)h->i, h->pend, ell, n2, h->list, h->offs, h->kact, h->ostat, h->oround);
   else
     hipLaunchKernelGGL(swfd_set_now_kernel, dim3(1), dim3(1), 0, st, h->now_dev, (long long)h->i);
   if (h->gram_split > 1) {
     const int kchunk = ((d + h->gram_split - 1) / h->gram_split + 15) / 16 * 16;
     if ((rc = gemm_f64_batched_splitk(true, true, h->buf, d, (long)n2 * d, h->buf, d, (long)n2 * d, h->gpart, n2, n2, d, S, kchunk,
-                                      h->gram_split, st, h->rep)))
+                                      h->gram_split, st, h->rep, h->list)))
       return rc;
-    if ((rc = gemm_batched_splitk_reduce(h->gpart, h->gram_split, (long)n2 * n2, eig_plan_input(h->eig), S, h->rep, st))) return rc;
+    if ((rc = gemm_batched_splitk_reduce(h->gpart, h->gram_split, (long)n2 * n2, eig_plan_input(h->eig), S, h->rep, st, h->list)))
+      return rc;
   } else if ((rc = gemm_f64(true, true, h->buf, d, (long)n2 * d, h->buf, d, (long)n2 * d, eig_plan_input(h->eig), n2,
-                            (long)n2 * n2, n2, n2, d, S, 1.0, st, h->rep)))
+                            (long)n2 * n2, n2, n2, d, S, 1.0, st, h->rep, h->list)))
     return rc;
   if ((rc = eig_plan_run_inplace(h->eig, nullptr, nullptr, st, true))) return rc;
   const EigColumns e = eig_plan_columns(h->eig);
   hipLaunchKernelGGL(swfd_decide_kernel, dim3(S), dim3(1024), 0, st, e.lam, e.cols, e.ld, n2, ell, h->cap, h->N, h->now_dev,
                      h->theta, h->meta, h->qt, h->dropped, h->plan, h->keep_src, h->Wc, h->rep);
   if ((rc = gemm_f64(true, false, h->Wc, n2, (long)ell * n2, h->buf, d, (long)n2 * d, h->T, d, (long)ell * d, ell, d,
-                     n2, S, 1.0, st, h->rep)))
+                     n2, S, 1.0, st, h->rep, h->list, h->kact)))
     return rc;
   hipLaunchKernelGGL(swfd_scatter_kernel, dim3(n2, S), dim3(256), 0, st, h->T, h->plan, h->keep_src, h->meta, h->buf,
                      h->queue, n2, ell, h->cap, d, h->rep);
@@ -596,6 +634,7 @@
   h->L = lg + 1;
   h->lanes = lanes;
   h->S = 2 * h->L * lanes;
+  MUSED_REQUIRE(h->S <= 8192, "mused_swfd_create: %d sketches (lanes x 2 levels), at most 8192", h->S);
   h->cap = 2 * ell;
   h->n2 = 2 * ell;
   h->n4 = 4 * ell;
@@ -613,6 +652,16 @@
   {
     const char* dd = getenv("MUSED_SWFD_DEDUPE");
     if (!(dd && dd[0] == '0')) ALLOC(h->rep, 4 * S);
+    auto off = [](const char* name) { const char* v = getenv(name); return v && v[0] == '0'; };
+    if (h->rep && !off("MUSED_SWFD_LIST")) {
+      ZALLOC(h->list, 4 * (S + 1));
+      ZALLOC(h->ostat, 8 * 18);
+      if (!off("MUSED_SWFD_ORDERS")) ZALLOC(h->offs, 4 * S);
+      const char* orr = getenv("MUSED_SWFD_ORDERS");
+      const int rv = orr ? atoi(orr) : 0;
+      h->oround = (rv == 1 || rv == 16 || rv == 32) ? rv : SWFD_OFFS_ROUND;
+      if (!off("MUSED_SWFD_KACT")) ZALLOC(h->kact, 4 * S);
+    }
     const char* sd = getenv("MUSED_SWFD_SKIP_DEAD");
     h->skip_dead = (sd && sd[0] == '0') ? 0 : 1;
   }
@@ -641,7 +690,8 @@
   MUSED_CHECK_HIP(hipMemcpy(h->theta, th.data(), 8 * S, hipMemcpyHostToDevice));
   int rc;
   if ((rc = gemm_f64_prepare_all())) return rc;
-  if ((rc = eig_plan_create(h->n2, h->S, h->sweeps, true, &h->eig, h->rep, EIG_PLAN_TOP_HALF, h->status))) return rc;
+  if ((rc = eig_plan_create(h->n2, h->S, h->sweeps, true, &h->eig, h->rep, EIG_PLAN_TOP_HALF, h->status, 0, h->list, h->offs)))
+    return rc;
   if ((rc = eig_plan_create(h->n4, lanes, h->sweeps + 2, true, &h->eigq, nullptr, EIG_PLAN_TOP_FD, h->status, ell))) return rc;
   if (h->n3 < h->n4 &&
       (rc = eig_plan_create(h->n3, lanes, h->sweeps + 2, true, &h->eigq3, nullptr, EIG_PLAN_TOP_FD, h->status, ell)))
@@ -677,7 +727,7 @@
   if (h->eigp) eig_plan_destroy(h->eigp);
   void* bufs[] = {h->buf, h->queue, h->qt, h->meta, h->dropped, h->theta, h->T, h->Wc, h->plan,
                   h->keep_src, h->now_dev, h->stack, h->Wq, h->Bout, h->sig_out, h->qinfo, h->qsel,
-                  h->rep, h->pre_in, h->pre_out, h->pre_gram, h->status, h->gpart};
+                  h->rep, h->pre_in, h->pre_out, h->pre_gram, h->status, h->gpart, h->list, h->offs, h->kact, h->ostat};
   for (void* b : bufs) (void)hipFree(b);
   if (h->status_host) (void)hipHostFree(h->status_host);
   delete h;
@@ -741,6 +791,15 @@
   if (h->rep && rep_out) MUSED_CHECK_HIP(hipMemcpy(rep_out, h->rep, 4 * (size_t)h->S, hipMemcpyDeviceToHost));
   if (meta_out) MUSED_CHECK_HIP(hipMemcpy(meta_out, h->meta, 16 * (size_t)h->S, hipMemcpyDeviceToHost));
   return h->rep ? 1 : 0;
+}
+
+int mused_swfd_debug_orders(void* handle, long long* out) {
+  Swfd* h = (Swfd*)handle;
+  if (!h || !out) return MUSED_ERR_ARG;
+  if (!h->ostat) return 0;
+  MUSED_CHECK_HIP(hipDeviceSynchronize());
+  MUSED_CHECK_HIP(hipMemcpy(out, h->ostat, 8 * 18, hipMemcpyDeviceToHost));
+  return 1;
 }
 
 int mused_swfd_query(void* handle, double* out_sketch, double* out_sigma, double* out_info, void* stream) {
@@ -837,6 +896,7 @@
   const size_t bytes = sizeof(double) * (size_t)2 * ell * d;
   hipError_t e = hipMemcpyAsync(h->buf, buf, bytes, hipMemcpyDeviceToDevice, st);
   h->i = 2 * ell;
+  h->pend = 2 * ell;
   if (e == hipSuccess) rc = mused::swfd_rotate_all(h, st);
   if (e == hipSuccess && !rc) e = hipMemcpyAsync(buf, h->buf, bytes, hipMemcpyDeviceToDevice, st);
   if (e == hipSuccess && !rc) {
diff --git a/mused_amd/csrc/trd.hip b/mused_amd/csrc/trd.hip
--- a/mused_amd/csrc/trd.hip
+++ b/mused_amd/csrc/trd.hip
@@ -209,21 +209,22 @@
 
 template <bool EMB>
 __global__ __launch_bounds__(TNT, 1) void trd_a_kernel(const double* __restrict__ Gc, const int* __restrict__ rep,
+                                                       const int* __restrict__ list, const int* __restrict__ offs,
                                                        double* __restrict__ ws, TrdDebug dbg, const TrdShape sh) {
   extern __shared__ __attribute__((aligned(16))) double sm[];
-  const int bm = blockIdx.x;
-  if (rep && rep[bm] != bm) return;
+  const int bm = trd_pick(rep, list, blockIdx.x);
+  if (bm < 0) return;
   const int t = threadIdx.x, w = t >> 6, l = t & 63;
   const int wp = w >> 2, wq = w & 3, lp = l & 7, lq = l >> 3;
   const int p = wp * 8 + lp, q = wq * 8 + lq;
-  const int off = EMB ? sh.off : 0, ldn = EMB ? sh.ldn : TN;
+  const int off = EMB ? (offs ? offs[bm] : sh.off) : 0, ldn = EMB ? sh.ldn : TN;
   const double* G = Gc + (long)bm * ldn * ldn;
   double* wsm = ws + (long)bm * W_PER;
   double* Hs = wsm + W_HS;
   double* S = sm + L_S;
   double A[2][36];
   const double* Gsrc = G;
-  if constexpr (EMB) {
+  if (EMB && off > 0) {
     for (int e = t; e < TN * TN; e += TNT) {
       const int j = e >> 8, i = e & 255;
       Hs[e] = (j >= off && i >= off) ? G[(long)(j - off) * ldn + (i - off)] : 0.0;
@@ -272,12 +273,13 @@
   }
 }
 
-__global__ __launch_bounds__(64) void trd_t_kernel(const int* __restrict__ rep, double* __restrict__ ws, const TrdShape sh) {
+__global__ __launch_bounds__(64) void trd_t_kernel(const int* __restrict__ rep, const int* __restrict__ list,
+                                                   const int* __restrict__ offs, double* __restrict__ ws, const TrdShape sh) {
   __shared__ double Gs[16][17];
   __shared__ double Ts[16][17];
-  const int bm = blockIdx.x >> 4, kb = blockIdx.x & 15;
-  if (rep && rep[bm] != bm) return;
-  if (16 * kb + 15 < sh.off) return;
+  const int bm = trd_pick(rep, list, blockIdx.x >> 4), kb = blockIdx.x & 15;
+  if (bm < 0) return;
+  if (16 * kb + 15 < (offs ? offs[bm] : sh.off)) return;
   double* wsm = ws + (long)bm * W_PER;
   const double* Hs = wsm + W_HS;
   const int l = threadIdx.x, kq = l >> 4, li = l & 15;
@@ -323,17 +325,16 @@
 constexpr int DM_TM = DM_VB + 16 * 272;
 constexpr int DM_TOTAL = DM_TM + 256;
 __global__ __launch_bounds__(TNT, 1) void trd_d_kernel(double* __restrict__ Gc, const int* __restrict__ rep,
+                                                       const int* __restrict__ list, const int* __restrict__ offs,
                                                        int* __restrict__ done, double* __restrict__ ws, TrdDebug dbg,
                                                        const TrdShape sh, double* __restrict__ lam_out) {
   extern __shared__ __attribute__((aligned(16))) double sm[];
-  const int bm = blockIdx.x;
-  if (rep && rep[bm] != bm) {
-    if (threadIdx.x == 0) done[bm] = 1;
-    return;
-  }
+  if (rep && rep[blockIdx.x] != (int)blockIdx.x && threadIdx.x == 0) done[blockIdx.x] = 1;
+  const int bm = trd_pick(rep, list, blockIdx.x);
+  if (bm < 0) return;
   const int t = threadIdx.x, w = t >> 6, l = t & 63;
   const int kq = l >> 4, li = l & 15;
-  const int off = sh.off, ldn = sh.ldn, n = sh.n;
+  const int off = offs ? offs[bm] : sh.off, ldn = sh.ldn, n = offs ? TN - off : sh.n;
   double* G = Gc + (long)bm * ldn * ldn;
   double* wsm = ws + (long)bm * W_PER;
   const double* Hs = wsm + W_HS;
@@ -550,7 +551,8 @@
   TrdDebug dbg{nullptr, nullptr};
   TrdShape sh;
   sh.n = TN; sh.ldn = TN; sh.off = 0; sh.nvec = TM; sh.need = TM; sh.cert_all = 0;
-  hipLaunchKernelGGL(trd_a_kernel<false>, dim3(batch), dim3(TNT), sizeof(double) * L_A_TOTAL, st, G, rep, ws, dbg, sh);
+  hipLaunchKernelGGL(trd_a_kernel<false>, dim3(batch), dim3(TNT), sizeof(double) * L_A_TOTAL, st, G, rep, (const int*)nullptr,
+                     (const int*)nullptr, ws, dbg, sh);
   MUSED_LAUNCH_CHECK();
   return MUSED_OK;
 }
@@ -558,8 +560,10 @@
 bool trd_supports(int n, int ldn, int need) { return n >= 2 && n <= TN && ldn >= n && ldn <= TN && need >= 1 && need <= TM && need <= n; }
 
 int trd_solve(double* Gc, int n, int ldn, int need, bool cert_all, int batch, const int* rep, int* done, double* ws,
-              hipStream_t st, long long* dbg_clk, unsigned long long* work, hipEvent_t after_a, double* lam_out) {
+              hipStream_t st, long long* dbg_clk, unsigned long long* work, hipEvent_t after_a, double* lam_out,
+              const int* list, const int* offs) {
   MUSED_REQUIRE(trd_supports(n, ldn, need), "trd_solve: unsupported shape (n=%d, ld=%d, need=%d)", n, ldn, need);
+  MUSED_REQUIRE(!offs || (n == TN && ldn == TN), "trd_solve: per-matrix orders need n = ld = 256 (n=%d, ld=%d)", n, ldn);
   TrdDebug dbg{dbg_clk, work};
   TrdShape sh;
   sh.n = n; sh.ldn = ldn; sh.off = TN - n;
@@ -567,14 +571,17 @@
   sh.need = need;
   sh.cert_all = cert_all ? 1 : 0;
   const int nch = sh.nvec / 32;
-  if (n == TN && ldn == TN) hipLaunchKernelGGL(trd_a_kernel<false>, dim3(batch), dim3(TNT), sizeof(double) * L_A_TOTAL, st, Gc, rep, ws, dbg, sh);
-  else hipLaunchKernelGGL(trd_a_kernel<true>, dim3(batch), dim3(TNT), sizeof(double) * L_A_TOTAL, st, Gc, rep, ws, dbg, sh);
+  if (n == TN && ldn == TN && !offs)
+    hipLaunchKernelGGL(trd_a_kernel<false>, dim3(batch), dim3(TNT), sizeof(double) * L_A_TOTAL, st, Gc, rep, list, offs, ws, dbg, sh);
+  else
+    hipLaunchKernelGGL(trd_a_kernel<true>, dim3(batch), dim3(TNT), sizeof(double) * L_A_TOTAL, st, Gc, rep, list, offs, ws, dbg, sh);
   if (after_a) MUSED_CHECK_HIP(hipEventRecord(after_a, st));
-  if (batch <= 64) hipLaunchKernelGGL((trd_b_kernel<128, L256>), dim3(nch * batch), dim3(128), 0, st, rep, ws, sh);
-  else hipLaunchKernelGGL((trd_b_kernel<512, L256>), dim3(batch), dim3(512), 0, st, rep, ws, sh);
-  hipLaunchKernelGGL((trd_c_kernel<L256, 32>), dim3(nch * batch), dim3(128), sizeof(double) * C_LDS, st, rep, ws, sh);
-  hipLaunchKernelGGL(trd_t_kernel, dim3(16 * batch), dim3(64), 0, st, rep, ws, sh);
-  hipLaunchKernelGGL(trd_d_kernel, dim3(batch), dim3(TNT), sizeof(double) * L_DM_TOTAL, st, Gc, rep, done, ws, dbg, sh, lam_out);
+  if (batch <= 64) hipLaunchKernelGGL((trd_b_kernel<128, L256>), dim3(nch * batch), dim3(128), 0, st, rep, list, ws, sh);
+  else hipLaunchKernelGGL((trd_b_kernel<512, L256>), dim3(batch), dim3(512), 0, st, rep, list, ws, sh);
+  hipLaunchKernelGGL((trd_c_kernel<L256, 32>), dim3(nch * batch), dim3(128), sizeof(double) * C_LDS, st, rep, list, ws, sh);
+  hipLaunchKernelGGL(trd_t_kernel, dim3(16 * batch), dim3(64), 0, st, rep, list, offs, ws, sh);
+  hipLaunchKernelGGL(trd_d_kernel, dim3(batch), dim3(TNT), sizeof(double) * L_DM_TOTAL, st, Gc, rep, list, offs, done, ws, dbg, sh,
+                     lam_out);
   MUSED_LAUNCH_CHECK();
   return MUSED_OK;
 }
@@ -607,6 +614,35 @@
   if (!rc) hipLaunchKernelGGL(trd_export_kernel, dim3(batch), dim3(TN), 0, st, ws, out_d, out_e, out_lam, out_res);
   hipError_t e = hipStreamSynchronize(st);
   (void)hipFree(ws);
+  if (rc) return rc;
+  MUSED_CHECK_HIP(e);
+  return MUSED_OK;
+}
+
+extern "C" int mused_debug_trd_offs(double* G, int need, int cert_all, int batch, double* out_d, double* out_e, double* out_lam,
+                                    double* out_res, int* out_done, const int* offs, const int* list, int nlist, const int* rep,
+                                    void* stream) {
+  MUSED_REQUIRE(G && batch >= 1 && out_done && nlist >= 0 && nlist <= batch, "mused_debug_trd_offs: bad arguments");
+  int rc = trd_prepare();
+  if (rc) return rc;
+  hipStream_t st = (hipStream_t)stream;
+  double* ws = nullptr;
+  int* lst = nullptr;
+  MUSED_CHECK_HIP(hipMalloc((void**)&ws, sizeof(double) * trd_workspace_doubles(batch)));
+  hipError_t e = hipSuccess;
+  if (list) {
+    e = hipMalloc((void**)&lst, sizeof(int) * (size_t)(batch + 1));
+    if (e == hipSuccess) e = hipMemcpyAsync(lst, &nlist, sizeof(int), hipMemcpyHostToDevice, st);
+    if (e == hipSuccess && nlist > 0) e = hipMemcpyAsync(lst + 1, list, sizeof(int) * (size_t)nlist, hipMemcpyDeviceToDevice, st);
+    if (e == hipSuccess) e = hipStreamSynchronize(st);
+  }
+  if (e == hipSuccess) {
+    rc = trd_solve(G, TN, TN, need, cert_all != 0, batch, rep, out_done, ws, st, nullptr, nullptr, nullptr, nullptr, lst, offs);
+    if (!rc) hipLaunchKernelGGL(trd_export_kernel, dim3(batch), dim3(TN), 0, st, ws, out_d, out_e, out_lam, out_res);
+    e = hipStreamSynchronize(st);
+  }
+  (void)hipFree(ws);
+  if (lst) (void)hipFree(lst);
   if (rc) return rc;
   MUSED_CHECK_HIP(e);
   return MUSED_OK;
diff --git a/mused_amd/csrc/trd_common.h b/mused_amd/csrc/trd_common.h
--- a/mused_amd/csrc/trd_common.h
+++ b/mused_amd/csrc/trd_common.h
@@ -27,6 +27,11 @@
   int need;
   int cert_all;
 };
+
+__device__ __forceinline__ int trd_pick(const int* __restrict__ rep, const int* __restrict__ list, int b) {
+  if (list) return b < list[0] ? list[1 + b] : -1;
+  return (rep && rep[b] != b) ? -1 : b;
+}
 
 __device__ __forceinline__ bool trd_significant(double lc, int c, double lam0, double lamcut, const TrdShape& sh) {
   if (c >= sh.need || !(lc > 0.0)) return false;
@@ -89,7 +94,8 @@
 }
 
 template <int NTB, typename LY>
-__global__ __launch_bounds__(NTB) void trd_b_kernel(const int* __restrict__ rep, double* __restrict__ ws, const TrdShape sh) {
+__global__ __launch_bounds__(NTB) void trd_b_kernel(const int* __restrict__ rep, const int* __restrict__ list,
+                                                    double* __restrict__ ws, const TrdShape sh) {
   constexpr int TNX = LY::TNX, NWV = NTB / 64;
   const int NCH = NTB == 512 ? 1 : sh.nvec / (NTB / 4);
   constexpr int PASSES = 19, NPT = 512;
@@ -97,8 +103,8 @@
   __shared__ double part[3 * NWV];
   __shared__ double scal[4];
   __shared__ int cnts[NPT];
-  const int bm = blockIdx.x / NCH, cq = blockIdx.x % NCH;
-  if (rep && rep[bm] != bm) return;
+  const int bm = trd_pick(rep, list, blockIdx.x / NCH), cq = blockIdx.x % NCH;
+  if (bm < 0) return;
   const int t = threadIdx.x, w = t >> 6, l = t & 63;
   double* wsm = ws + (long)bm * LY::W_PER;
   const double* dg = wsm + LY::W_TG;
@@ -173,7 +179,8 @@
 constexpr int trd_c_lds_doubles() { return 2 * LY::TNX + LY::TNX + 4 * VPW + 2 * LY::TNX * VPW; }
 
 template <typename LY, int VPW>
-__global__ __launch_bounds__(128) void trd_c_kernel(const int* __restrict__ rep, double* __restrict__ ws, const TrdShape sh) {
+__global__ __launch_bounds__(128) void trd_c_kernel(const int* __restrict__ rep, const int* __restrict__ list,
+                                                    double* __restrict__ ws, const TrdShape sh) {
   constexpr int TNX = LY::TNX, TMX = LY::TMX;
   static_assert(TNX % 32 == 0 && (VPW == 8 || VPW == 16 || VPW == 32), "trd_c_kernel: unsupported shape");
   extern __shared__ __attribute__((aligned(16))) double smc[];
@@ -183,8 +190,9 @@
   double* qp = xch + 4 * VPW;
   double* qm = qp + TNX * VPW;
   const int nch = sh.nvec / VPW;
-  const int bm = blockIdx.x / nch, cq = blockIdx.x - bm * nch;
-  if (rep && rep[bm] != bm) return;
+  const int bq = blockIdx.x / nch, cq = blockIdx.x - bq * nch;
+  const int bm = trd_pick(rep, list, bq);
+  if (bm < 0) return;
   const int t = threadIdx.x, role = t >> 6, l = t & 63;
   double* wsm = ws + (long)bm * LY::W_PER;
   double* Zg = wsm + LY::W_ZG;
diff --git a/mused_amd/csrc/trdx.hip b/mused_amd/csrc/trdx.hip
--- a/mused_amd/csrc/trdx.hip
+++ b/mused_amd/csrc/trdx.hip
@@ -794,9 +794,9 @@
   }
   hipLaunchKernelGGL(trdx_tail_merge_kernel<NX>, dim3(XTAIL, batch), dim3(256), 0, st, rep, ws, wst, trd_tail_ws_per(), trd_tail_off_hs(),
                      trd_tail_off_tg());
-  hipLaunchKernelGGL((trd_b_kernel<128, LY>), dim3(nch32 * batch), dim3(128), 0, st, rep, ws, sh);
+  hipLaunchKernelGGL((trd_b_kernel<128, LY>), dim3(nch32 * batch), dim3(128), 0, st, rep, (const int*)nullptr, ws, sh);
   constexpr size_t c_lds = sizeof(double) * trd_c_lds_doubles<LY, VPW>();
-  hipLaunchKernelGGL((trd_c_kernel<LY, VPW>), dim3(nchc * batch), dim3(128), c_lds, st, rep, ws, sh);
+  hipLaunchKernelGGL((trd_c_kernel<LY, VPW>), dim3(nchc * batch), dim3(128), c_lds, st, rep, (const int*)nullptr, ws, sh);
   hipLaunchKernelGGL(trdx_cert_kernel<LY>, dim3(batch), dim3(256), 0, st, rep, ws, done, act, jrep, nrej, work, sh);
   MUSED_LAUNCH_CHECK();
   hipLaunchKernelGGL(trdx_tfac_kernel<NX>, dim3(LY::NBLK, batch), dim3(256), sizeof(double) * TF_LDS_DOUBLES, st, act, ws);
```

Result: faster. 602,900 rows/s (median of 6 runs) (+9.1%).
